# KevinMathewT/multimodal-propaganda-meme-classification

Measured on AMD Instinct MI355X. Metric: memes/sec (fine-tune step) ViT-B/16+BERT-base bs=32, 1/2/4/8 MI355X, higher is better.
Workload: dtype fp16

## Files before the change

### include/memehip.h

```cpp
#ifndef MEMEHIP_H
#define MEMEHIP_H

#include <stdint.h>

#ifdef __cplusplus
extern "C" {
#endif

typedef enum MhStatus {
    MH_OK = 0,
    MH_EINVAL = 1,
    MH_ESHAPE = 2,
    MH_ELAUNCH = 3
} MhStatus;

typedef void* mh_stream_t;

const char* mh_version(void);
const char* mh_status_str(int status);

#define MH_GEMM_MAX_GROUP 8
#define MH_GEMM_GELU 1
#define MH_GEMM_OUT_F32 2
#define MH_GEMM_ACCUM 4
#define MH_GEMM_QUICK_GELU 8
#define MH_GEMM_DERIV_AUX 16

typedef struct MhGemmProblem {
    const void* A;
    const void* B;
    void* C;
    const float* bias;
    const void* residual;
    void* aux;
    const void* mul;
    float* rowsum;
    int32_t M, N, K;
    int32_t lda, ldb, ldc;
    int32_t flags;
    float alpha;
    const uint32_t* drop_rng;
    float drop_p;
    uint32_t drop_stream;
    const int32_t* rows_dev;
    const int32_t* drop_rows;
    int32_t ksplit;
    int32_t reserved_;
} MhGemmProblem;

int mh_gemm_bf16_grouped(const MhGemmProblem* problems , int n_problems, int a_kmajor,
                         int b_kmajor, mh_stream_t stream);
int mh_gemm_ksplit_for(int K, int want);
int mh_gemm_set_trace(void* device_buffer);

int mh_layernorm_fwd(const void* x , const float* gamma, const float* beta, void* y ,
                     float* y_f32 , float* mean, float* rstd,
                     int rows, int D, float eps, mh_stream_t stream);
int mh_layernorm_bwd(const void* dy , const void* x , const float* gamma,
                     const float* mean, const float* rstd, const void* dx_add ,
                     void* dx , float* part , int n_part, int rows, int D,
                     void* dx_drop ,
                     const uint32_t* rng, float drop_p, uint32_t drop_stream, mh_stream_t stream);
#define MH_LN_MAX_JOBS 4
typedef struct MhLnFwdJob {
    const void* x; const float* gamma; const float* beta; void* y; float* y_f32; float* mean; float* rstd;
    int32_t rows; float eps;
    const int32_t* rows_dev;
} MhLnFwdJob;
typedef struct MhLnBwdJob {
    const void* dy; const void* x; const float* gamma; const float* mean; const float* rstd;
    const void* dx_add; void* dx; float* part; void* dx_drop; const uint32_t* rng;
    int32_t n_part; int32_t rows; float drop_p; uint32_t drop_stream;
    const int32_t* rows_dev;
    const int32_t* drop_rows;
} MhLnBwdJob;
int mh_layernorm_fwd_grouped(const MhLnFwdJob* jobs, int n_jobs, int D, mh_stream_t stream);
int mh_layernorm_bwd_grouped(const MhLnBwdJob* jobs, int n_jobs, int D, mh_stream_t stream);
#define MH_COLSUM_MAX_JOBS 64
typedef struct MhColsumJob {
    const float* part;
    float* out0;
    float* out1;
} MhColsumJob;
int mh_colsum_partials_f32(const MhColsumJob* jobs , int n_jobs, int n_part, int D,
                           float scale, mh_stream_t stream);

int mh_attn_fwd(const void* qkv, const int64_t* key_mask, void* out, float* lse, int B, int S, int H,
                const uint32_t* rng, float drop_p, uint32_t drop_stream, mh_stream_t stream);
int mh_attn_bwd(const void* qkv, const int64_t* key_mask, const void* out, const void* dout,
                const float* lse, float* delta, void* dqkv, int B, int S, int H, const uint32_t* rng,
                float drop_p, uint32_t drop_stream, mh_stream_t stream);
int mh_attn_fwd_packed(const void* qkv, const int64_t* key_mask, void* out, float* lse, const int32_t* cu,
                       const int32_t* row_map, int B, int S, int H, const uint32_t* rng, float drop_p,
                       uint32_t drop_stream, mh_stream_t stream);
int mh_attn_bwd_packed(const void* qkv, const int64_t* key_mask, const void* out, const void* dout,
                       const float* lse, float* delta, void* dqkv, const int32_t* cu, const int32_t* row_map, int B,
                       int S, int H, const uint32_t* rng, float drop_p, uint32_t drop_stream, mh_stream_t stream);

#define MH_ATTN_MAX_GROUP 2
typedef struct MhAttnProblem {
    const void* qkv; const int64_t* key_mask; void* out; float* lse;
    const void* dout; float* delta; void* dqkv;
    const int32_t* cu; const int32_t* row_map;
    const uint32_t* rng; float drop_p; uint32_t drop_stream;
    int32_t B, S, H; int32_t reserved;
} MhAttnProblem;
int mh_attn_fwd_grouped(const MhAttnProblem* problems , int n, mh_stream_t stream);
int mh_attn_bwd_grouped(const MhAttnProblem* problems , int n, mh_stream_t stream);
int mh_attn_set_onepass(int on);

int mh_pack_plan(const int64_t* mask , int B, int S, int pool_index, int32_t* cu, int32_t* row_map,
                 int32_t* inv_map, int64_t* pmask, int32_t* pool_rows, int32_t* n_rows, mh_stream_t stream);
int mh_pack_rows(const void* src , const int32_t* row_map, const int32_t* n_rows, void* dst,
                 int max_rows, int D, mh_stream_t stream);
int mh_unpack_rows(const void* src , const int32_t* inv_map, void* dst ,
                   int max_rows, int D, mh_stream_t stream);

#define MH_ROWS_MAX_JOBS 8
typedef struct {
    const void* src;
    void* dst;
    const int32_t* idx;
    const int32_t* rows_dev;
    int32_t n, rows, D, stride, offset; int32_t reserved_;
} MhRowsJob;
int mh_rows_gather(const MhRowsJob* jobs , int n_jobs, mh_stream_t stream);
int mh_rows_scatter_zero(const MhRowsJob* jobs , int n_jobs, mh_stream_t stream);

int mh_bert_embed_fwd(const int64_t* ids, const float* word, const float* pos, const float* type0,
                      const float* gamma, const float* beta, void* pre ,
                      void* y , float* mean, float* rstd, int B, int S, int D, int vocab,
                      float eps, const uint32_t* rng, float drop_p, uint32_t drop_stream ,
                      mh_stream_t stream);
int mh_bert_embed_bwd(const int64_t* ids, const void* d_pre , float* dword ,
                      float* dpos , float* dtype0 , int B, int S, int D,
                      int vocab, int64_t pad_id, float scale,
                      uint8_t* row_live ,
                      int32_t* first_pos , int32_t* id_count
                      ,
                      mh_stream_t stream);
int mh_position_ids_from_input_ids(const int64_t* ids , int32_t* pos_ids, int32_t* pos_inv, int B, int S, int pad_id,
                                   int max_position, mh_stream_t stream);
int mh_bert_embed_fwd_pos(const int64_t* ids, const float* word, const float* pos , const float* type0,
                          const float* gamma, const float* beta, void* pre, void* y, float* mean, float* rstd, int B, int S,
                          int D, int vocab, float eps, const uint32_t* rng, float drop_p, uint32_t drop_stream,
                          const int32_t* pos_ids , int max_position, mh_stream_t stream);
int mh_embed_pos_bwd(const void* d_pre , const int32_t* pos_inv ,
                     float* dpos , float* dtype0 , float* scratch ,
                     int B, int S, int D, int max_position, float scale, mh_stream_t stream);
int mh_image_normalize_u8(const uint8_t* src, float* dst, int B, int H, int W, const float* mean3 ,
                          const float* std3 , mh_stream_t stream);
int mh_image_resample_u8(const uint8_t* arena, const int64_t* src_off, const int32_t* hw, const int32_t* xbounds,
                         const int32_t* xcoef, int KX, const int32_t* ybounds, const int32_t* ycoef, int KY, const uint8_t* flip,
                         const uint8_t* vfirst, uint8_t* tmp, uint8_t* out, int B, int max_h, int max_w, int OH, int OW,
                         mh_stream_t stream);
int mh_image_luma_sum_u8(const uint8_t* img, unsigned long long* sums, int B, int HW, mh_stream_t stream);
int mh_image_jitter_rotate_u8(const uint8_t* in, uint8_t* scratch, uint8_t* out, const void* params, unsigned long long* lsum,
                              int B, int H, int W, mh_stream_t stream);
int mh_dropout_apply(void* x, int64_t n, const uint32_t* rng, float p, uint32_t stream_id, mh_stream_t stream);
int mh_dropout_mask_u8(uint8_t* out, int64_t n, const uint32_t* rng, float p, uint32_t stream_id,
                       mh_stream_t stream);
int mh_zero_rows_f32(const int64_t* ids, float* table, int n_ids, int D, int vocab, mh_stream_t stream);

int mh_patchify(const float* image, void* patches, int B, int C, int H, int W, int P, mh_stream_t stream);
int mh_patchify_ld(const float* image, void* patches , int B, int C, int H, int W, int P, int ld,
                   mh_stream_t stream);
int mh_copy2d_u32(const void* src, int ld_src, void* dst, int ld_dst, int rows, int cols, int pad_to, mh_stream_t stream);
int mh_vit_assemble_fwd(const void* proj , const float* cls, const float* pos,
                        void* x , int B, int Np, int D, mh_stream_t stream);
int mh_vit_assemble_bwd(const void* dx , void* dproj ,
                        float* dcls, float* dpos, int B, int Np, int D, float scale, mh_stream_t stream);

typedef struct MhHeadParams {
    const float *Wt, *bt;
    const float *Wi, *bi;
    const float *Wf, *bf_;
    const float *Wo, *bo;
} MhHeadParams;
typedef struct MhHeadGrads {
    float *Wt, *bt, *Wi, *bi, *Wf, *bf_, *Wo, *bo;
} MhHeadGrads;

int mh_head_fwd(const MhHeadParams* p , const float* text_hidden ,
                const float* image_hidden , int text_pool_index, float* pooled
                , float* feat , float* fused ,
                float* logits , int B, int S, int Nt, int Dt, int Di, int P, int C,
                const uint32_t* rng, float drop_p, uint32_t drop_stream ,
                const int32_t* text_rows , mh_stream_t stream);
int mh_head_bwd(const MhHeadParams* p , const MhHeadGrads* g , const float* dlogits,
                const float* pooled, const float* feat, const float* fused, float* dfeat ,
                float* dfused , void* d_text_hidden ,
                void* d_image_hidden , int text_pool_index, int B, int S, int Nt,
                int Dt, int Di, int P, int C, float out_scale, const uint32_t* rng, float drop_p,
                uint32_t drop_stream, const int32_t* text_rows , mh_stream_t stream);
int mh_pool_fwd(const float* text_hidden, const float* image_hidden, int text_pool_index, float* pooled, int B, int S,
                int Nt, int Dt, int Di, const int32_t* text_rows, mh_stream_t stream);
int mh_pool_bwd(const float* d_pooled, void* d_text_hidden, void* d_image_hidden, int text_pool_index, int B, int S,
                int Nt, int Dt, int Di, float out_scale, const int32_t* text_rows, mh_stream_t stream);
#define MH_BN_RELU 1
#define MH_BN_FROZEN_STATS 2
int mh_bn1d_fwd(const float* x, int ldx, const float* gamma, const float* beta, float* running_mean, float* running_var,
                float* y, int ldy, float* save_mean, float* save_rstd, int B, int F, float eps, float momentum,
                int training, int relu, mh_stream_t stream);
int mh_bn1d_bwd(const float* dy, int lddy, const float* x, int ldx, const float* y, int ldy, const float* gamma,
                const float* save_mean, const float* save_rstd, float* dx, int lddx, float* dgamma, float* dbeta, int B,
                int F, int relu, mh_stream_t stream);
int mh_ce_fwd_bwd(const float* logits, const int64_t* labels, float* loss, float* dlogits,
                  int32_t* n_correct, int B, int C, float grad_scale,
                  const float* grad_scale_dev ,
                  mh_stream_t stream);
int mh_focal_fwd_bwd(const float* logits, int ld, const float* targets , float* loss,
                     float* dlogits, int32_t* n_correct, int B, float alpha, float gamma, float grad_scale,
                     const float* grad_scale_dev , mh_stream_t stream);

#define MH_F32_ACCUM 1
#define MH_F32_TANH 2
#define MH_F32_RELU 4
#define MH_F32_BN 8
typedef struct MhGemmF32 {
    const float* A; const float* B; float* C; const float* bias ;
    int32_t M, N, K, lda, ldb, ldc, flags;
    const float* bn_gamma; const float* bn_beta; float* bn_running_mean; float* bn_running_var;
    float* bn_save_mean; float* bn_save_rstd; float* bn_z ;
    int32_t bn_ldz; float bn_eps; float bn_momentum; int32_t bn_training;
} MhGemmF32;
int mh_gemm_f32(const MhGemmF32* p , int a_kmajor, int b_kmajor, mh_stream_t stream);
int mh_colsum_f32(const float* x, int ld, float* out, int rows, int D, float scale, mh_stream_t stream);
int mh_pool_max_fwd(const float* h, float* out, int32_t* arg, int B, int S, int D, mh_stream_t stream);
int mh_pool_max_bwd(const float* dout, const int32_t* arg, float* dh, int B, int S, int D, mh_stream_t stream);
int mh_pool_mean_fwd(const float* h, const int64_t* mask, float* out, int B, int S, int D, mh_stream_t stream);
int mh_pool_mean_bwd(const float* dout, const int64_t* mask, float* dh, int B, int S, int D, mh_stream_t stream);
int mh_pool_attn_fwd(const float* h, const float* u, const float* w2, const float* b2, const int64_t* mask, float* p,
                     float* out, int B, int S, int D, int A, mh_stream_t stream);
int mh_pool_attn_bwd(const float* h, const float* u, const float* w2, const float* p, const float* dout, float* du, float* dh,
                     float* dw2_part, float* db2_part, int B, int S, int D, int A, mh_stream_t stream);
int mh_pad_seq_f32(const float* h, float* hp, int B, int S, int D, int pad, int Sp, mh_stream_t stream);
int mh_relu_max_fwd(const float* z, float* out, int32_t* arg, int B, int S, int Sp, int D, mh_stream_t stream);
int mh_relu_max_bwd(const float* dout, const int32_t* arg, float* dz, int rows, int Sp, int D, mh_stream_t stream);
int mh_conv_fold_f32(const float* da, float* dh, int B, int S, int D, int taps, int pad, int Sp, int rows, mh_stream_t stream);
int mh_softmax_gate_fwd(const float* g, const float* c, float* y, int B, int F, mh_stream_t stream);
int mh_softmax_gate_bwd(const float* g, const float* c, const float* dy, float* dg, float* dc, int B, int F, mh_stream_t stream);

int mh_mca3_fwd(const float* pa, const float* pc, const float* pi, const float* Vw, const float* bv, const float* text,
                const float* caption, float* w, float* ctx, int B, int U, mh_stream_t stream);
int mh_mca3_bwd(const float* pa, const float* pc, const float* pi, const float* Vw, const float* text, const float* caption,
                const float* w, const float* dctx, float* de_ws, float* dpa, float* dpi, float* dtext, float* dcaption,
                float* dV_part, float* dbv_part, int B, int U, mh_stream_t stream);

int mh_nchw_to_nhwc(const float* x, void* y, int B, int C, int H, int W, int Cp, mh_stream_t stream);
int mh_im2col_nhwc(const void* x, void* col, int B, int H, int W, int C, int KH, int KW, int stride, int pad, int ldc,
                   mh_stream_t stream);
int mh_col2im_nhwc(const void* dcol, void* dx, int B, int H, int W, int C, int KH, int KW, int stride, int pad, int ldc,
                   mh_stream_t stream);
int mh_conv_weight_pack(const float* w , void* out , int Cout, int Cin, int KH, int KW,
                        int Cp, int ldk, mh_stream_t stream);
int mh_conv_weight_unpack(const float* gk , float* g , int Cout, int Cin, int KH, int KW, int Cp,
                          int ldk, float scale, mh_stream_t stream);
#define MH_CONV_MAX_JOBS 64
typedef struct MhConvPackJob {
    const float* w;
    void* out;
    int32_t Cout, Cin, KH, KW, Cp, ldk;
// ... 124 lines not shown
```

### multimodal_propaganda_meme_classification_amd/_lib.py

```python
from __future__ import annotations

import ctypes as C
import os

_HERE = os.path.dirname(os.path.abspath(__file__))
LIB_PATH = os.path.join(_HERE, "libmemehip.so")
LIB_PATH_F16 = os.path.join(_HERE, "libmemehip_f16.so")
LIB_PATHS = {"bf16": LIB_PATH, "fp16": LIB_PATH_F16}

MH_GEMM_MAX_GROUP = 8
MH_GEMM_GELU = 1
MH_GEMM_OUT_F32 = 2
MH_GEMM_ACCUM = 4
MH_GEMM_QUICK_GELU = 8
MH_GEMM_DERIV_AUX = 16
MH_COLSUM_MAX_JOBS = 64
MH_LN_MAX_JOBS = 4
MH_ATTN_MAX_GROUP = 2

c_void_p, c_int, c_int64, c_float = C.c_void_p, C.c_int, C.c_int64, C.c_float


class MhGemmProblem(C.Structure):
    _fields_ = [("A", c_void_p), ("B", c_void_p), ("C", c_void_p), ("bias", c_void_p),
                ("residual", c_void_p), ("aux", c_void_p), ("mul", c_void_p), ("rowsum", c_void_p),
                ("M", C.c_int32), ("N", C.c_int32), ("K", C.c_int32),
                ("lda", C.c_int32), ("ldb", C.c_int32), ("ldc", C.c_int32),
                ("flags", C.c_int32), ("alpha", C.c_float),
                ("drop_rng", c_void_p), ("drop_p", C.c_float), ("drop_stream", C.c_uint32),
                ("rows_dev", c_void_p), ("drop_rows", c_void_p), ("ksplit", C.c_int32), ("reserved_", C.c_int32)]


class MhColsumJob(C.Structure):
    _fields_ = [("part", c_void_p), ("out0", c_void_p), ("out1", c_void_p)]


class MhConvPackJob(C.Structure):
    _fields_ = [("w", c_void_p), ("out", c_void_p)] + [(n, C.c_int32) for n in ("Cout", "Cin", "KH", "KW", "Cp", "ldk", "block_start", "reserved_")]


class MhConvWgradJob(C.Structure):
    _fields_ = [("slabs", c_void_p), ("g", c_void_p)] + [(n, C.c_int32) for n in ("Cout", "Cin", "KH", "KW", "Cp", "ldk", "nsplit", "accumulate")] + \
               [("scale", C.c_float), ("block_start", C.c_int32)]


class MhConvGeom(C.Structure):
    _fields_ = [(n, C.c_int32) for n in ("B", "H", "W", "C", "KH", "KW", "stride", "pad", "Cout", "ldk")]


class MhConvBnBwd(C.Structure):
    _fields_ = [(n, c_void_p) for n in ("z", "mean", "rstd", "gamma", "beta", "part")] + [("relu", C.c_int32), ("reserved_", C.c_int32),
                                                                                          ("addend", c_void_p), ("y_mask", c_void_p)]


class MhConvWgradProblem(C.Structure):
    _fields_ = [("dy", c_void_p), ("x", c_void_p), ("slabs", c_void_p), ("ksplit", C.c_int32), ("alpha", C.c_float), ("geom", MhConvGeom)]


MH_CONV_MAX_GROUP = 6
MH_CONV_MAX_JOBS = 64
MH_BN_RELU, MH_BN_ACCUM_PARAM_GRADS = 1, 2


MH_ADAM_MAX_GROUPS = 8


class MhAdamSkipGroups(C.Structure):
    _fields_ = [("hyper", c_void_p * MH_ADAM_MAX_GROUPS), ("beta1", C.c_double * MH_ADAM_MAX_GROUPS), ("beta2", C.c_double * MH_ADAM_MAX_GROUPS),
                ("n", C.c_int32), ("reserved_", C.c_int32)]


class MhLossScale(C.Structure):
    _fields_ = [("scale", c_void_p), ("growth", c_void_p), ("overflow", c_void_p), ("growth_factor", C.c_float), ("backoff_factor", C.c_float),
                ("min_scale", C.c_float), ("max_scale", C.c_float), ("growth_interval", C.c_int32), ("base_grad_scale", C.c_float)]


class MhLnFwdJob(C.Structure):
    _fields_ = [(n, c_void_p) for n in ("x", "gamma", "beta", "y", "y_f32", "mean", "rstd")] + \
               [("rows", C.c_int32), ("eps", C.c_float), ("rows_dev", c_void_p)]


class MhLnBwdJob(C.Structure):
    _fields_ = [(n, c_void_p) for n in ("dy", "x", "gamma", "mean", "rstd", "dx_add", "dx", "part", "dx_drop", "rng")] + \
               [("n_part", C.c_int32), ("rows", C.c_int32), ("drop_p", C.c_float), ("drop_stream", C.c_uint32),
                ("rows_dev", c_void_p), ("drop_rows", c_void_p)]


class MhAttnProblem(C.Structure):
    _fields_ = [(n, c_void_p) for n in ("qkv", "key_mask", "out", "lse", "dout", "delta", "dqkv", "cu", "row_map", "rng")] + \
               [("drop_p", C.c_float), ("drop_stream", C.c_uint32), ("B", C.c_int32), ("S", C.c_int32), ("H", C.c_int32),
                ("reserved", C.c_int32)]


MH_ROWS_MAX_JOBS = 8


class MhRowsJob(C.Structure):
    _fields_ = [(n, c_void_p) for n in ("src", "dst", "idx", "rows_dev")] + \
               [(n, C.c_int32) for n in ("n", "rows", "D", "stride", "offset", "reserved_")]


class MhGemmF32(C.Structure):
    _fields_ = [("A", c_void_p), ("B", c_void_p), ("C", c_void_p), ("bias", c_void_p)] + \
               [(n, C.c_int32) for n in ("M", "N", "K", "lda", "ldb", "ldc", "flags")] + \
               [(n, c_void_p) for n in ("bn_gamma", "bn_beta", "bn_running_mean", "bn_running_var", "bn_save_mean",
                                        "bn_save_rstd", "bn_z")] + \
               [("bn_ldz", C.c_int32), ("bn_eps", C.c_float), ("bn_momentum", C.c_float), ("bn_training", C.c_int32)]


MH_F32_ACCUM, MH_F32_TANH, MH_F32_RELU, MH_F32_BN = 1, 2, 4, 8


class MhHeadParams(C.Structure):
    _fields_ = [(n, c_void_p) for n in ("Wt", "bt", "Wi", "bi", "Wf", "bf_", "Wo", "bo")]


class MhHeadGrads(C.Structure):
    _fields_ = [(n, c_void_p) for n in ("Wt", "bt", "Wi", "bi", "Wf", "bf_", "Wo", "bo")]


_PROTOS = {
    "mh_gemm_bf16_grouped": [C.POINTER(MhGemmProblem), c_int, c_int, c_int, c_void_p],
    "mh_gemm_set_trace": [c_void_p],
    "mh_gemm_ksplit_for": [c_int, c_int],
    "mh_layernorm_fwd": [c_void_p] * 7 + [c_int, c_int, c_float, c_void_p],
    "mh_layernorm_bwd": [c_void_p] * 8 + [c_int, c_int, c_int, c_void_p, c_void_p, c_float, C.c_uint32, c_void_p],
    "mh_layernorm_fwd_grouped": [C.POINTER(MhLnFwdJob), c_int, c_int, c_void_p],
    "mh_layernorm_bwd_grouped": [C.POINTER(MhLnBwdJob), c_int, c_int, c_void_p],
    "mh_colsum_partials_f32": [C.POINTER(MhColsumJob), c_int, c_int, c_int, c_float, c_void_p],
    "mh_attn_fwd": [c_void_p] * 4 + [c_int, c_int, c_int, c_void_p, c_float, C.c_uint32, c_void_p],
    "mh_attn_bwd": [c_void_p] * 7 + [c_int, c_int, c_int, c_void_p, c_float, C.c_uint32, c_void_p],
    "mh_attn_fwd_grouped": [C.POINTER(MhAttnProblem), c_int, c_void_p],
    "mh_attn_bwd_grouped": [C.POINTER(MhAttnProblem), c_int, c_void_p],
    "mh_attn_set_onepass": [c_int],
    "mh_attn_fwd_packed": [c_void_p] * 6 + [c_int, c_int, c_int, c_void_p, c_float, C.c_uint32, c_void_p],
    "mh_attn_bwd_packed": [c_void_p] * 9 + [c_int, c_int, c_int, c_void_p, c_float, C.c_uint32, c_void_p],
    "mh_pack_plan": [c_void_p, c_int, c_int, c_int] + [c_void_p] * 6 + [c_void_p],
    "mh_pack_rows": [c_void_p] * 4 + [c_int, c_int, c_void_p],
    "mh_unpack_rows": [c_void_p] * 3 + [c_int, c_int, c_void_p],
    "mh_rows_gather": [C.POINTER(MhRowsJob), c_int, c_void_p],
    "mh_rows_scatter_zero": [C.POINTER(MhRowsJob), c_int, c_void_p],
    "mh_bert_embed_fwd": [c_void_p] * 10 + [c_int, c_int, c_int, c_int, c_float, c_void_p, c_float, C.c_uint32, c_void_p],
    "mh_image_normalize_u8": [c_void_p, c_void_p, c_int, c_int, c_int, C.POINTER(c_float), C.POINTER(c_float), c_void_p],
    "mh_image_resample_u8": [c_void_p] * 5 + [c_int] + [c_void_p] * 2 + [c_int] + [c_void_p] * 4 + [c_int] * 5 + [c_void_p],
    "mh_image_luma_sum_u8": [c_void_p, c_void_p, c_int, c_int, c_void_p],
    "mh_image_jitter_rotate_u8": [c_void_p] * 5 + [c_int] * 3 + [c_void_p],
    "mh_dropout_apply": [c_void_p, c_int64, c_void_p, c_float, C.c_uint32, c_void_p],
    "mh_dropout_mask_u8": [c_void_p, c_int64, c_void_p, c_float, C.c_uint32, c_void_p],
    "mh_bert_embed_bwd": [c_void_p] * 5 + [c_int, c_int, c_int, c_int, c_int64, c_float, c_void_p, c_void_p, c_void_p, c_void_p],
    "mh_position_ids_from_input_ids": [c_void_p] * 3 + [c_int] * 4 + [c_void_p],
    "mh_bert_embed_fwd_pos": [c_void_p] * 10 + [c_int, c_int, c_int, c_int, c_float, c_void_p, c_float, C.c_uint32, c_void_p, c_int,
                              c_void_p],
    "mh_embed_pos_bwd": [c_void_p] * 5 + [c_int] * 4 + [c_float, c_void_p],
    "mh_zero_rows_f32": [c_void_p, c_void_p, c_int, c_int, c_int, c_void_p],
    "mh_patchify": [c_void_p, c_void_p] + [c_int] * 5 + [c_void_p],
    "mh_patchify_ld": [c_void_p, c_void_p] + [c_int] * 6 + [c_void_p],
    "mh_copy2d_u32": [c_void_p, c_int, c_void_p, c_int, c_int, c_int, c_int, c_void_p],
    "mh_vit_assemble_fwd": [c_void_p] * 4 + [c_int] * 3 + [c_void_p],
    "mh_vit_assemble_bwd": [c_void_p] * 4 + [c_int] * 3 + [c_float, c_void_p],
    "mh_head_fwd": [C.POINTER(MhHeadParams), c_void_p, c_void_p, c_int] + [c_void_p] * 4 + [c_int] * 7 + [c_void_p, c_float, C.c_uint32, c_void_p, c_void_p],
    "mh_head_bwd": [C.POINTER(MhHeadParams), C.POINTER(MhHeadGrads)] + [c_void_p] * 8 + [c_int] * 8 + [c_float, c_void_p, c_float, C.c_uint32, c_void_p, c_void_p],
    "mh_pool_fwd": [c_void_p, c_void_p, c_int, c_void_p] + [c_int] * 5 + [c_void_p, c_void_p],
    "mh_pool_bwd": [c_void_p, c_void_p, c_void_p, c_int] + [c_int] * 5 + [c_float, c_void_p, c_void_p],
    "mh_bn1d_fwd": [c_void_p, c_int, c_void_p, c_void_p, c_void_p, c_void_p, c_void_p, c_int, c_void_p, c_void_p, c_int, c_int,
                    c_float, c_float, c_int, c_int, c_void_p],
    "mh_bn1d_bwd": [c_void_p, c_int, c_void_p, c_int, c_void_p, c_int, c_void_p, c_void_p, c_void_p, c_void_p, c_int, c_void_p,
                    c_void_p, c_int, c_int, c_int, c_void_p],
    "mh_gemm_f32": [C.POINTER(MhGemmF32), c_int, c_int, c_void_p],
    "mh_colsum_f32": [c_void_p, c_int, c_void_p, c_int, c_int, c_float, c_void_p],
    "mh_pool_max_fwd": [c_void_p, c_void_p, c_void_p, c_int, c_int, c_int, c_void_p],
    "mh_pool_max_bwd": [c_void_p, c_void_p, c_void_p, c_int, c_int, c_int, c_void_p],
    "mh_pool_mean_fwd": [c_void_p, c_void_p, c_void_p, c_int, c_int, c_int, c_void_p],
    "mh_pool_mean_bwd": [c_void_p, c_void_p, c_void_p, c_int, c_int, c_int, c_void_p],
    "mh_pool_attn_fwd": [c_void_p] * 7 + [c_int] * 4 + [c_void_p],
    "mh_pool_attn_bwd": [c_void_p] * 9 + [c_int] * 4 + [c_void_p],
    "mh_pad_seq_f32": [c_void_p, c_void_p] + [c_int] * 5 + [c_void_p],
    "mh_relu_max_fwd": [c_void_p, c_void_p, c_void_p] + [c_int] * 4 + [c_void_p],
    "mh_relu_max_bwd": [c_void_p, c_void_p, c_void_p] + [c_int] * 3 + [c_void_p],
    "mh_conv_fold_f32": [c_void_p, c_void_p] + [c_int] * 7 + [c_void_p],
    "mh_mca3_fwd": [c_void_p] * 9 + [c_int, c_int, c_void_p],
    "mh_mca3_bwd": [c_void_p] * 15 + [c_int, c_int, c_void_p],
    "mh_softmax_gate_fwd": [c_void_p, c_void_p, c_void_p, c_int, c_int, c_void_p],
    "mh_softmax_gate_bwd": [c_void_p] * 5 + [c_int, c_int, c_void_p],
    "mh_nchw_to_nhwc": [c_void_p, c_void_p] + [c_int] * 5 + [c_void_p],
    "mh_im2col_nhwc": [c_void_p, c_void_p] + [c_int] * 9 + [c_void_p],
    "mh_col2im_nhwc": [c_void_p, c_void_p] + [c_int] * 9 + [c_void_p],
    "mh_conv_weight_pack": [c_void_p, c_void_p] + [c_int] * 6 + [c_void_p],
    "mh_conv_weight_unpack": [c_void_p, c_void_p] + [c_int] * 6 + [c_float, c_void_p],
    "mh_conv_weight_pack_batched": [C.POINTER(MhConvPackJob), c_int, c_void_p],
    "mh_conv_wgrad_finish_batched": [C.POINTER(MhConvWgradJob), c_int, c_void_p],
    "mh_conv_splitk": [C.POINTER(MhConvGeom), c_int],
    "mh_conv_fwd": [c_void_p, c_void_p, c_void_p, c_void_p, c_void_p, C.POINTER(MhConvGeom), c_void_p],
    "mh_conv_dgrad": [c_void_p, c_void_p, c_void_p, c_void_p, C.POINTER(MhConvGeom), C.POINTER(MhConvBnBwd), c_void_p],
    "mh_conv_dgrad_pair": [c_void_p, c_void_p, c_void_p, c_void_p, c_int, c_int, c_void_p, C.POINTER(MhConvGeom), C.POINTER(MhConvBnBwd), c_void_p],
    "mh_bn2d_bwd_parts": [c_void_p, c_void_p, c_void_p, c_int] + [c_void_p] * 7 + [c_int, c_int, c_int, c_float, c_void_p],
    "mh_conv_wgrad": [c_void_p, c_void_p, c_void_p, c_int, c_float, C.POINTER(MhConvGeom), c_void_p],
    "mh_conv_wgrad_grouped": [C.POINTER(MhConvWgradProblem), c_int, c_void_p],
    "mh_bn2d_fwd_parts": [c_void_p, c_void_p, c_int] + [c_void_p] * 8 + [c_int, c_int, c_float, c_float, c_int, c_void_p],
    "mh_bn2d_workspace_elems": [c_int, c_int],
    "mh_bn2d_fwd": [c_void_p] * 10 + [c_int, c_int, c_float, c_float, c_int, c_int, c_void_p],
    "mh_bn2d_apply": [c_void_p] * 7 + [c_int, c_int, c_int, c_void_p],
    "mh_bn2d_bwd": [c_void_p] * 12 + [c_int, c_int, c_int, c_float, c_void_p],
    "mh_maxpool_fwd": [c_void_p, c_void_p, c_void_p] + [c_int] * 7 + [c_void_p],
    "mh_maxpool_bwd": [c_void_p, c_void_p, c_void_p] + [c_int] * 7 + [c_void_p],
    "mh_avgpool_fwd": [c_void_p, c_void_p, c_int, c_int, c_int, c_void_p],
    "mh_avgpool_bwd": [c_void_p, c_void_p, c_int, c_int, c_int, c_float, c_void_p],
    "mh_add_h16": [c_void_p, c_void_p, c_void_p, c_int64, c_void_p],
    "mh_dwconv_weight_pack": [c_void_p, c_void_p, c_int, c_int, c_void_p],
    "mh_dwconv_nhwc": [c_void_p, c_void_p, c_void_p, c_void_p] + [c_int] * 5 + [c_void_p],
    "mh_dwconv_nhwc_dgrad": [c_void_p, c_void_p, c_void_p, c_void_p] + [c_int] * 5 + [c_void_p],
    "mh_dwconv_wgrad_workspace_elems": [c_int] * 5,
    "mh_dwconv_nhwc_wgrad": [c_void_p] * 5 + [c_int] * 5 + [c_float, c_int, c_void_p],
    "mh_layer_scale_bwd": [c_void_p] * 8 + [c_int, c_int, c_int, c_void_p],
    "mh_ce_fwd_bwd": [c_void_p] * 5 + [c_int, c_int, c_float, c_void_p, c_void_p],
    "mh_focal_fwd_bwd": [c_void_p, c_int, c_void_p, c_void_p, c_void_p, c_void_p, c_int, c_float, c_float, c_float, c_void_p, c_void_p],
    "mh_adam_skip_account": [C.POINTER(MhAdamSkipGroups), c_void_p, c_void_p, c_void_p, C.POINTER(MhLossScale), c_void_p],
    "mh_sumsq_f32": [c_void_p, c_int64, c_void_p, c_void_p, c_void_p],
    "mh_adam_step": [c_void_p] * 5 + [c_int64, c_int64, c_void_p, c_int, c_void_p, c_float, c_float, c_void_p, c_int, c_void_p],
    "mh_adam_step_rows": [c_void_p] * 6 + [c_int, c_int, c_void_p, c_int, c_void_p, c_float, c_float, c_void_p, c_int, c_void_p],
    "mh_cast_f32_bf16": [c_void_p, c_void_p, c_int64, c_void_p],
    "mh_cast_bf16_f32": [c_void_p, c_void_p, c_int64, c_void_p],
    "mh_sum_shards_16": [c_void_p, c_void_p, c_int, c_int64, c_void_p],
    "mh_attn_decode": [c_void_p, c_int, c_void_p, c_void_p, c_int64, c_int, c_void_p, c_int, c_void_p, c_int, c_void_p, c_int,
                       c_void_p, c_int, c_int, c_int, c_void_p],
    "mh_decode_embed": [c_void_p] * 7 + [c_int] * 4 + [c_float, c_void_p],
    "mh_greedy_step": [c_void_p, c_int, c_int, c_int, c_void_p, c_int, c_void_p, c_void_p, c_void_p, c_int, c_int64, c_int64, c_void_p],
    "mh_version": [],
    "mh_status_str": [c_int],
}
_RESTYPES = {"mh_version": C.c_char_p, "mh_status_str": C.c_char_p, "mh_bn2d_workspace_elems": c_int64,
             "mh_dwconv_wgrad_workspace_elems": c_int64}
_LAB_PROTOS = {"mh_gemm_set_variant": ([c_int], c_int), "mh_gemm_streamk_workspace_bytes": ([], c_int64),
               "mh_gemm_set_streamk": ([c_void_p, c_int], c_int)}

EXPORTED_SYMBOLS = tuple(_PROTOS)

_libs = {}


class MemehipError(RuntimeError):
    pass


def load(kind: str = "bf16") -> C.CDLL:
    if kind in _libs:
        return _libs[kind]
    if kind not in LIB_PATHS:
        raise ValueError(f"compute dtype must be 'bf16' or 'fp16', got {kind!r}")
    path = LIB_PATHS[kind]
    if kind == "bf16" and os.environ.get("MEMEHIP_LIB"):
        path = os.environ["MEMEHIP_LIB"]
    if kind == "fp16" and os.environ.get("MEMEHIP_LIB_F16"):
        path = os.environ["MEMEHIP_LIB_F16"]
    if not os.path.exists(path):
        raise MemehipError(
            f"{path} is missing: build the HIP extension first "
            "(python -c 'import __graft_entry__ as g; g.build()' or make -C "
            "multimodal_propaganda_meme_classification_amd/csrc). There is no CPU/PyTorch fallback.")
    lib = C.CDLL(path)
    for name, argtypes in _PROTOS.items():
        fn = getattr(lib, name)
        fn.argtypes = argtypes
        fn.restype = _RESTYPES.get(name, c_int)
    for name, (argtypes, restype) in _LAB_PROTOS.items():
        if hasattr(lib, name):
            fn = getattr(lib, name)
            fn.argtypes, fn.restype = argtypes, restype
    _libs[kind] = lib
    return lib


def check(status: int, what: str):
    if status != 0:
        msg = load().mh_status_str(status).decode()
        raise MemehipError(f"{what} failed: status {status} ({msg})")
```

### multimodal_propaganda_meme_classification_amd/csrc/attention.hip

```cpp
#include "common.h"
#include <stdlib.h>

namespace {

constexpr int HD = 64;
constexpr int TILE = 64;
constexpr int IMG = TILE * HD * 2;
constexpr float NEG_BIG = -1.0e30f;
constexpr float LOG2E = 1.4426950408889634f;
constexpr float LN2 = 0.6931471805599453f;

MH_DEV int row_img_off(int row, int chunk) { return row * 128 + ((chunk ^ ((row ^ (row >> 3)) & 7)) << 4); }
MH_DEV int tr_img_off(int row, int unit) { return row * 128 + ((unit ^ (((row >> 1) & 1) << 1)) << 5); }

template <int NT>
struct TileRegs {
    static constexpr int CH = (TILE * 8 + NT - 1) / NT;
    i32x4 v[CH];
};
template <int NT>
MH_DEV void tile_load(const h16* __restrict__ base, size_t pitch, int row0, int nrows, int tid, TileRegs<NT>& R) {
#pragma unroll
    for (int i = 0; i < TileRegs<NT>::CH; ++i) {
        const int q = tid + i * NT;
        const int r = q >> 3, c = q & 7;
        R.v[i] = i32x4{0, 0, 0, 0};
        if (q < TILE * 8 && row0 + r < nrows) R.v[i] = *(const i32x4*)(base + (size_t)(row0 + r) * pitch + c * 8);
    }
}
template <int NT>
MH_DEV void tile_store(const TileRegs<NT>& R, int tid, char* row_img, char* tr_img) {
#pragma unroll
    for (int i = 0; i < TileRegs<NT>::CH; ++i) {
        const int q = tid + i * NT;
        if (q >= TILE * 8) continue;
        const int r = q >> 3, c = q & 7;
        if (row_img) *(i32x4*)(row_img + row_img_off(r, c)) = R.v[i];
        if (tr_img) *(i32x4*)(tr_img + tr_img_off(r, c >> 1) + ((c & 1) << 4)) = R.v[i];
    }
}

template <int NW, int NTL>
MH_DEV void dma_resident(const h16* __restrict__ base, size_t pitch, int nrows, int ntiles, int wave_u, int lane, char* row_img,
                         char* tr_img) {
    const __amdgpu_buffer_rsrc_t rs = mh_rsrc(base, (uint32_t)(((size_t)(nrows - 1) * pitch + HD) * 2));
    const int npieces = ntiles * 8;
#pragma unroll
    for (int i = 0; i < (NTL * 8 + NW - 1) / NW; ++i) {
        const int p = wave_u + i * NW;
        if (p < npieces) {
            const int r = p * 8 + (lane >> 3), rl = r & (TILE - 1), cp = lane & 7;
            const uint32_t rowoff = (uint32_t)r * (uint32_t)pitch * 2u;
            if (row_img) {
                const int ck = cp ^ ((rl ^ (rl >> 3)) & 7);
                __builtin_amdgcn_raw_ptr_buffer_load_lds(rs, LDS_PTR(void, row_img + p * 1024), 16, rowoff + ck * 16, 0, 0, 0);
            }
            if (tr_img) {
                const int cv = ((((cp >> 1) ^ (((rl >> 1) & 1) << 1)) << 1) | (cp & 1));
                __builtin_amdgcn_raw_ptr_buffer_load_lds(rs, LDS_PTR(void, tr_img + p * 1024), 16, rowoff + cv * 16, 0, 0, 0);
            }
        }
    }
}

MH_DEV h16x8 frag_rows(const char* img, int rb, int s, int lane) {
    Pack8 u;
    u.v = *(const i32x4*)(img + row_img_off(rb + (lane & 31), 2 * s + (lane >> 5)));
    return u.h;
}
MH_DEV h16x8 frag_tr(const char* img, int rb, int s, int dbase, int lane) {
    const int i = lane & 15, q = i >> 2, p = i & 3;
    const int chalf = (lane >> 4) & 1, h = lane >> 5;
    const int unit = (dbase >> 4) + chalf;
    const int r0 = rb + 16 * s + 4 * h + q;
    const int r1 = r0 + 8;
    s16x4 lo = __builtin_amdgcn_ds_read_tr16_b64_v4i16(LDS_PTR(s16x4, img + tr_img_off(r0, unit) + 8 * p));
    s16x4 hi = __builtin_amdgcn_ds_read_tr16_b64_v4i16(LDS_PTR(s16x4, img + tr_img_off(r1, unit) + 8 * p));
    union {
        struct { s16x4 lo, hi; } s;
        h16x8 h8;
    } cv;
    cv.s.lo = lo;
    cv.s.hi = hi;
    return cv.h8;
}
MH_DEV h16x8 acc_frag(const f32x16& x, int s) {
    h16x8 f;
#pragma unroll
    for (int j = 0; j < 8; ++j) f[j] = (h16)x[8 * s + j];
    return f;
}
MH_DEV int acc_row(int g, int h) { return (g & 3) + 8 * (g >> 2) + 4 * h; }

MH_DEV void load_rows_frag(const h16* __restrict__ base, size_t pitch, int row0, int nrows, int lane,
                           h16x8 (&f)[4]) {
    const int r = row0 + (lane & 31);
#pragma unroll
    for (int s = 0; s < 4; ++s) {
        Pack8 u;
        u.v = i32x4{0, 0, 0, 0};
        if (r < nrows) u.v = *(const i32x4*)(base + (size_t)r * pitch + 16 * s + 8 * (lane >> 5));
        f[s] = u.h;
    }
}

MH_DEV void store_rows_from_T(h16* __restrict__ base, size_t pitch, int row0, int nrows, int lane,
                              const f32x16 (&acc)[2], float scale) {
    const int r = row0 + (lane & 31), h = lane >> 5;
    if (r >= nrows) return;
#pragma unroll
    for (int dt = 0; dt < 2; ++dt)
#pragma unroll
        for (int g4 = 0; g4 < 4; ++g4) {
            Pack4 u;
#pragma unroll
            for (int e = 0; e < 4; ++e) u.e[e] = (h16)(acc[dt][4 * g4 + e] * scale);
            *(i32x2*)(base + (size_t)r * pitch + dt * 32 + 8 * g4 + 4 * h) = u.v;
        }
}

struct AttnArgs {
    const h16* qkv;
    const int64_t* key_mask;
    h16* out;
    float* lse;
    const h16* dout;
    float* delta;
    h16* dqkv;
    int B, S, H;
    const uint32_t* rng;
    float drop_p;
    uint32_t drop_stream;
    const int32_t* cu;
    const int32_t* row_map;
};

template <int NW, int NT_RES, bool DROP>
MH_DEV void attn_fwd_body(const AttnArgs& A, const int bx, const int gx, const int bh, char* smem) {
    const h16* __restrict__ qkv = A.qkv;
    const int64_t* __restrict__ key_mask = A.key_mask;
    h16* __restrict__ out = A.out;
    float* __restrict__ lse = A.lse;
    const int S = A.S, H = A.H;
    const uint32_t* __restrict__ rng = A.rng;
    const float drop_p = A.drop_p;
    const uint32_t drop_stream = A.drop_stream;
    const int32_t* __restrict__ cu = A.cu;
    const int32_t* __restrict__ row_map = A.row_map;
    constexpr int NT = NW * 64;
    constexpr int NTL = NT_RES > 0 ? NT_RES : 1;
    const DropCtx drop = mh_drop_ctx(DROP ? rng : nullptr, drop_p, drop_stream);
    char* k_img = smem;
    char* v_img = smem + NTL * IMG;
    float* kbias = (float*)(smem + 2 * NTL * IMG);
    int* kany = (int*)(kbias + NTL * TILE);
    int* pos_t = kany + 16;

    const int b = bh / H, hh = bh % H;
    const int tid = threadIdx.x, lane = tid & 63, wave = tid >> 6, h = lane >> 5;
    const size_t pitch = (size_t)3 * H * HD;
    const size_t r0 = cu ? (size_t)cu[b] : (size_t)b * S;
    const int Sb = cu ? cu[b + 1] - cu[b] : S;
    auto pos = [&](int i) -> uint64_t { return (row_map && i < Sb) ? (uint64_t)(row_map[r0 + i] - b * S) : (uint64_t)i; };
    auto posl = [&](int i) -> uint64_t { return NT_RES > 0 ? (uint64_t)pos_t[i] : pos(i); };
    const h16* qb = qkv + r0 * pitch + hh * HD;
    const h16* kb = qb + (size_t)H * HD;
    const h16* vb = qb + (size_t)2 * H * HD;
    const float c = 0.125f * LOG2E;
    constexpr float LAZY_LOG2 = 6.0f;
    const int ntiles = (Sb + TILE - 1) / TILE;

    const int qt_first = bx * NW + wave;
    h16x8 qf[4];
    if (NT_RES > 0) {
        const int uw = __builtin_amdgcn_readfirstlane(wave);
        dma_resident<NW, NTL>(kb, pitch, Sb, ntiles, uw, lane, k_img, nullptr);
        dma_resident<NW, NTL>(vb, pitch, Sb, ntiles, uw, lane, nullptr, v_img);
        if (qt_first * 32 < Sb) load_rows_frag(qb, pitch, qt_first * 32, Sb, lane, qf);
        if (DROP)
            for (int i = tid; i < NTL * TILE; i += NT) pos_t[i] = (int)pos(i);
        if (tid < TILE) {
            int64_t km[NTL];
#pragma unroll
            for (int t = 0; t < NTL; ++t) km[t] = 1;
            if (key_mask && Sb > 0) {
#pragma unroll
                for (int t = 0; t < NTL; ++t) km[t] = key_mask[r0 + max(min(t * TILE + tid, Sb - 1), 0)];
            }
#pragma unroll
            for (int t = 0; t < NTL; ++t)
                if (t * TILE + tid >= Sb) km[t] = 0;
#pragma unroll
            for (int t = 0; t < NTL; ++t) {
                const float bias = km[t] != 0 ? 0.f : NEG_BIG;
                kbias[t * TILE + tid] = bias;
                const unsigned long long bal = __ballot(bias == 0.f);
                if (tid == 0) {
                    kany[t * 2] = (bal & 0xffffffffull) != 0;
                    kany[t * 2 + 1] = (bal >> 32) != 0;
                }
            }
        }
        __syncthreads();
    }

    for (int qt = qt_first; (NT_RES > 0) ? (qt * 32 < Sb) : (qt == bx * NW + wave); qt += NW * gx) {
        const int wq0 = qt * 32;
        const bool active = wq0 < Sb;
        if (NT_RES == 0 || qt != qt_first) load_rows_frag(qb, pitch, wq0, Sb, lane, qf);
        f32x16 o[2];
#pragma unroll
        for (int i = 0; i < 2; ++i)
#pragma unroll
            for (int g = 0; g < 16; ++g) o[i][g] = 0.f;
        float m = NEG_BIG, l = 0.f;
        TileRegs<NT> Rk, Rv;
        int64_t Rm = 0;
        auto pre_load = [&](int t) {
            tile_load<NT>(kb, pitch, t * TILE, Sb, tid, Rk);
            tile_load<NT>(vb, pitch, t * TILE, Sb, tid, Rv);
            if (tid < TILE) {
                const int key = t * TILE + tid;
                Rm = (key < Sb && (!key_mask || key_mask[r0 + key] != 0)) ? 1 : 0;
            }
        };
        auto pre_store = [&]() {
            tile_store<NT>(Rk, tid, k_img, nullptr);
            tile_store<NT>(Rv, tid, nullptr, v_img);
            if (tid < TILE) {
                const float bias = Rm ? 0.f : NEG_BIG;
                kbias[tid] = bias;
                const unsigned long long bal = __ballot(bias == 0.f);
                if (tid == 0) {
                    kany[0] = (bal & 0xffffffffull) != 0;
                    kany[1] = (bal >> 32) != 0;
                }
            }
        };
        if (NT_RES == 0 && ntiles > 0) pre_load(0);

        for (int t = 0; t < ntiles; ++t) {
            const int slot = NT_RES > 0 ? t : 0;
            if (NT_RES == 0) {
                __syncthreads();
                pre_store();
                __syncthreads();
                if (t + 1 < ntiles) pre_load(t + 1);
                if (!active) continue;
            }
            const char* ki = k_img + slot * IMG;
            const char* vi = v_img + slot * IMG;
            const float* kbt = kbias + slot * TILE;
#pragma unroll
            for (int sub = 0; sub < 2; ++sub) {
                if (!__builtin_amdgcn_readfirstlane(kany[slot * 2 + sub])) continue;
                f32x16 st;
#pragma unroll
                for (int g = 0; g < 16; ++g) st[g] = 0.f;
#pragma unroll
                for (int s = 0; s < 4; ++s)
                    st = MH_MFMA_32x32x16(frag_rows(ki, sub * 32, s, lane), qf[s], st, 0, 0, 0);
                float mx = NEG_BIG;
#pragma unroll
                for (int g4 = 0; g4 < 4; ++g4) {
                    const f32x4 kb4 = *(const f32x4*)(kbt + sub * 32 + 8 * g4 + 4 * h);
#pragma unroll
                    for (int e = 0; e < 4; ++e) {
                        const float v = st[4 * g4 + e] * c + kb4[e];
                        st[4 * g4 + e] = v;
                        mx = fmaxf(mx, v);
                    }
                }
                mx = fmaxf(mx, mh_xor_partner<32>(mx, (unsigned)lane));
                const bool move = mx > m + LAZY_LOG2;
                if (__ballot(move) != 0ull) {
                    const float mn = move ? mx : m;
                    const float alpha = __builtin_amdgcn_exp2f(m - mn);
                    m = mn;
                    l *= alpha;
#pragma unroll
                    for (int i = 0; i < 2; ++i)
#pragma unroll
                        for (int g = 0; g < 16; ++g) o[i][g] *= alpha;
                }
                float ps = 0.f;
#pragma unroll
                for (int g = 0; g < 16; ++g) {
                    const float p = __builtin_amdgcn_exp2f(st[g] - m);
                    st[g] = p;
                    ps += p;
                }
                l += ps;
                if (DROP && drop.on) {
                    const uint64_t rowbase = (((uint64_t)bh * S) + posl(wq0 + (lane & 31))) * (uint64_t)S;
#pragma unroll
                    for (int g = 0; g < 16; ++g)
                        st[g] *= mh_drop_mul(drop, rowbase + posl(t * TILE + sub * 32 + acc_row(g, h)));
                }
#pragma unroll
                for (int s = 0; s < 2; ++s) {
                    const h16x8 pf = acc_frag(st, s);
#pragma unroll
                    for (int dt = 0; dt < 2; ++dt)
                        o[dt] = MH_MFMA_32x32x16(frag_tr(vi, sub * 32, s, dt * 32, lane), pf, o[dt], 0, 0, 0);
                }
            }
        }
        if (!active) continue;
        l += mh_xor_partner<32>(l, (unsigned)lane);
        const float inv = l > 0.f ? 1.0f / l : 0.f;
        store_rows_from_T(out + r0 * H * HD + hh * HD, (size_t)H * HD, wq0, Sb, lane, o, inv);
        const int q = wq0 + (lane & 31);
        if (h == 0 && q < Sb) lse[((size_t)b * H + hh) * S + q] = (m + __builtin_amdgcn_logf(l)) * LN2;
    }
}

template <int NW, int NT_RES, bool DROP>
MH_DEV void attn_bwd_dq_body(const AttnArgs& A, const int bx, const int gx, const int bh, char* smem) {
    const h16* __restrict__ qkv = A.qkv;
    const int64_t* __restrict__ key_mask = A.key_mask;
    const h16* __restrict__ out = A.out;
    const h16* __restrict__ dout = A.dout;
    const float* __restrict__ lse = A.lse;
    float* __restrict__ delta = A.delta;
    h16* __restrict__ dqkv = A.dqkv;
    const int S = A.S, H = A.H;
    const uint32_t* __restrict__ rng = A.rng;
    const float drop_p = A.drop_p;
    const uint32_t drop_stream = A.drop_stream;
    const int32_t* __restrict__ cu = A.cu;
    const int32_t* __restrict__ row_map = A.row_map;
    constexpr int NT = NW * 64;
    constexpr int NTL = NT_RES > 0 ? NT_RES : 1;
    const DropCtx drop = mh_drop_ctx(DROP ? rng : nullptr, drop_p, drop_stream);
    char* k_img = smem;
    char* kt_img = smem + NTL * IMG;
    char* v_img = smem + 2 * NTL * IMG;
    float* kbias = (float*)(smem + 3 * NTL * IMG);
    int* kany = (int*)(kbias + NTL * TILE);
    int* pos_t = kany + 16;

    const int b = bh / H, hh = bh % H;
    const int tid = threadIdx.x, lane = tid & 63, wave = tid >> 6, h = lane >> 5;
    const size_t pitch = (size_t)3 * H * HD;
    const size_t r0 = cu ? (size_t)cu[b] : (size_t)b * S;
    const int Sb = cu ? cu[b + 1] - cu[b] : S;
    auto pos = [&](int i) -> uint64_t { return (row_map && i < Sb) ? (uint64_t)(row_map[r0 + i] - b * S) : (uint64_t)i; };
    auto posl = [&](int i) -> uint64_t { return NT_RES > 0 ? (uint64_t)pos_t[i] : pos(i); };
    const h16* qb = qkv + r0 * pitch + hh * HD;
    const h16* kb = qb + (size_t)H * HD;
    const h16* vb = qb + (size_t)2 * H * HD;
    const h16* dob = dout + r0 * H * HD + hh * HD;
    const float c = 0.125f * LOG2E;
    const int ntiles = (Sb + TILE - 1) / TILE;

    auto stage = [&](int t, int slot) {
        if (tid < TILE) {
            const int key = t * TILE + tid;
            float bias = NEG_BIG;
            if (key < Sb && (!key_mask || key_mask[r0 + key] != 0)) bias = 0.f;
            kbias[slot * TILE + tid] = bias;
            const unsigned long long bal = __ballot(bias == 0.f);
            if (tid == 0) {
                kany[slot * 2] = (bal & 0xffffffffull) != 0;
                kany[slot * 2 + 1] = (bal >> 32) != 0;
            }
        }
    };
    if (NT_RES > 0) {
        const int uw = __builtin_amdgcn_readfirstlane(wave);
        dma_resident<NW, NTL>(kb, pitch, Sb, ntiles, uw, lane, k_img, kt_img);
        dma_resident<NW, NTL>(vb, pitch, Sb, ntiles, uw, lane, v_img, nullptr);
        if (DROP)
            for (int i = tid; i < NTL * TILE; i += NT) pos_t[i] = (int)pos(i);
        for (int t = 0; t < ntiles; ++t) stage(t, t);
        __syncthreads();
    }

    for (int qt = bx * NW + wave; (NT_RES > 0) ? (qt * 32 < Sb) : (qt == bx * NW + wave); qt += NW * gx) {
        const int wq0 = qt * 32;
        const bool active = wq0 < Sb;
        const int q = wq0 + (lane & 31);
        h16x8 qf[4], dof[4];
        load_rows_frag(qb, pitch, wq0, Sb, lane, qf);
        load_rows_frag(dob, (size_t)H * HD, wq0, Sb, lane, dof);
        float dl = 0.f;
        {
            h16x8 of[4];
            load_rows_frag(out + r0 * H * HD + hh * HD, (size_t)H * HD, wq0, Sb, lane, of);
#pragma unroll
            for (int s4 = 0; s4 < 4; ++s4)
#pragma unroll
                for (int j = 0; j < 8; ++j) dl += (float)dof[s4][j] * (float)of[s4][j];
            dl += mh_xor_partner<32>(dl, (unsigned)lane);
        }
        float lse2 = 0.f;
        if (q < Sb) {
            lse2 = lse[((size_t)b * H + hh) * S + q] * LOG2E;
            if (h == 0) delta[((size_t)b * H + hh) * S + q] = dl;
        }
        f32x16 dq[2];
#pragma unroll
        for (int i = 0; i < 2; ++i)
#pragma unroll
            for (int g = 0; g < 16; ++g) dq[i][g] = 0.f;
        TileRegs<NT> Rk, Rv;
        int64_t Rm = 0;
        auto pre_load = [&](int t) {
            tile_load<NT>(kb, pitch, t * TILE, Sb, tid, Rk);
            tile_load<NT>(vb, pitch, t * TILE, Sb, tid, Rv);
            if (tid < TILE) {
                const int key = t * TILE + tid;
                Rm = (key < Sb && (!key_mask || key_mask[r0 + key] != 0)) ? 1 : 0;
            }
        };
        auto pre_store = [&]() {
            tile_store<NT>(Rk, tid, k_img, kt_img);
            tile_store<NT>(Rv, tid, v_img, nullptr);
            if (tid < TILE) {
                const float bias = Rm ? 0.f : NEG_BIG;
                kbias[tid] = bias;
                const unsigned long long bal = __ballot(bias == 0.f);
                if (tid == 0) {
                    kany[0] = (bal & 0xffffffffull) != 0;
                    kany[1] = (bal >> 32) != 0;
                }
            }
        };
        if (NT_RES == 0 && ntiles > 0) pre_load(0);

        for (int t = 0; t < ntiles; ++t) {
            const int slot = NT_RES > 0 ? t : 0;
            if (NT_RES == 0) {
                __syncthreads();
                pre_store();
                __syncthreads();
                if (t + 1 < ntiles) pre_load(t + 1);
                if (!active) continue;
            }
            const char* ki = k_img + slot * IMG;
            const char* kti = kt_img + slot * IMG;
            const char* vi = v_img + slot * IMG;
            const float* kbt = kbias + slot * TILE;
#pragma unroll
            for (int sub = 0; sub < 2; ++sub) {
                if (!__builtin_amdgcn_readfirstlane(kany[slot * 2 + sub])) continue;
                f32x16 st, dp;
#pragma unroll
                for (int g = 0; g < 16; ++g) { st[g] = 0.f; dp[g] = 0.f; }
#pragma unroll
                for (int s = 0; s < 4; ++s) {
                    st = MH_MFMA_32x32x16(frag_rows(ki, sub * 32, s, lane), qf[s], st, 0, 0, 0);
                    dp = MH_MFMA_32x32x16(frag_rows(vi, sub * 32, s, lane), dof[s], dp, 0, 0, 0);
                }
#pragma unroll
                for (int g4 = 0; g4 < 4; ++g4) {
                    const f32x4 kb4 = *(const f32x4*)(kbt + sub * 32 + 8 * g4 + 4 * h);
#pragma unroll
                    for (int e = 0; e < 4; ++e) {
                        const int g = 4 * g4 + e;
                        const float p = __builtin_amdgcn_exp2f(st[g] * c + kb4[e] - lse2);
                        float dpg = dp[g];
                        if (DROP && drop.on)
                            dpg *= mh_drop_mul(drop, ((uint64_t)bh * S + posl(q)) * (uint64_t)S +
                                                         posl(t * TILE + sub * 32 + acc_row(g, h)));
                        st[g] = p * (dpg - dl);
                    }
                }
#pragma unroll
                for (int s = 0; s < 2; ++s) {
                    const h16x8 df = acc_frag(st, s);
#pragma unroll
                    for (int dt = 0; dt < 2; ++dt)
                        dq[dt] = MH_MFMA_32x32x16(frag_tr(kti, sub * 32, s, dt * 32, lane), df, dq[dt], 0, 0, 0);
                }
            }
        }
        if (!active) continue;
        store_rows_from_T(dqkv + r0 * pitch + hh * HD, pitch, wq0, Sb, lane, dq, 0.125f);
    }
}

template <int NW, int NT_RES, bool DROP, bool OWN_DELTA = false>
MH_DEV void attn_bwd_dkv_body(const AttnArgs& A, const int bx, const int gx, const int bh, char* smem) {
    const h16* __restrict__ qkv = A.qkv;
    const int64_t* __restrict__ key_mask = A.key_mask;
    const h16* __restrict__ outp = A.out;
    const h16* __restrict__ dout = A.dout;
    const float* __restrict__ lse = A.lse;
    const float* __restrict__ delta = A.delta;
    h16* __restrict__ dqkv = A.dqkv;
    const int S = A.S, H = A.H;
    const uint32_t* __restrict__ rng = A.rng;
    const float drop_p = A.drop_p;
    const uint32_t drop_stream = A.drop_stream;
    const int32_t* __restrict__ cu = A.cu;
    const int32_t* __restrict__ row_map = A.row_map;
    constexpr int NT = NW * 64;
    constexpr int NTL = NT_RES > 0 ? NT_RES : 1;
    const DropCtx drop = mh_drop_ctx(DROP ? rng : nullptr, drop_p, drop_stream);
    char* q_img = smem;
    char* qt_img = smem + NTL * IMG;
    char* do_img = smem + 2 * NTL * IMG;
    char* dot_img = smem + 3 * NTL * IMG;
    float* lse_t = (float*)(smem + 4 * NTL * IMG);
    float* dl_t = lse_t + NTL * TILE;
    int* pos_t = (int*)(dl_t + NTL * TILE);

    const int b = bh / H, hh = bh % H;
    const int tid = threadIdx.x, lane = tid & 63, wave = tid >> 6, h = lane >> 5;
    const size_t pitch = (size_t)3 * H * HD;
    const size_t r0 = cu ? (size_t)cu[b] : (size_t)b * S;
    const int Sb = cu ? cu[b + 1] - cu[b] : S;
    auto pos = [&](int i) -> uint64_t { return (row_map && i < Sb) ? (uint64_t)(row_map[r0 + i] - b * S) : (uint64_t)i; };
    auto posl = [&](int i) -> uint64_t { return NT_RES > 0 ? (uint64_t)pos_t[i] : pos(i); };
    const h16* qb = qkv + r0 * pitch + hh * HD;
    const h16* kb = qb + (size_t)H * HD;
    const h16* vb = qb + (size_t)2 * H * HD;
    const h16* dob = dout + r0 * H * HD + hh * HD;
    const float c = 0.125f * LOG2E;
    const int ntiles = (Sb + TILE - 1) / TILE;

    auto stage = [&](int t, int slot) {
        for (int i = tid; i < TILE; i += NT) {
            const int qq = t * TILE + i;
            lse_t[slot * TILE + i] = qq < Sb ? lse[((size_t)b * H + hh) * S + qq] * LOG2E : 1.0e30f;
            if (!OWN_DELTA) dl_t[slot * TILE + i] = qq < Sb ? delta[((size_t)b * H + hh) * S + qq] : 0.f;
        }
        if (OWN_DELTA && tid < 2 * TILE) {
            const int i = tid >> 1, hf = tid & 1;
            const int qq = t * TILE + i;
            float dl = 0.f;
            if (qq < Sb) {
                const h16* dr = dob + (size_t)qq * H * HD + 8 * hf;
                const h16* orow = outp + (r0 + qq) * (size_t)H * HD + hh * HD + 8 * hf;
#pragma unroll
                for (int s4 = 0; s4 < 4; ++s4) {
                    Pack8 a, o;
                    a.v = *(const i32x4*)(dr + 16 * s4);
                    o.v = *(const i32x4*)(orow + 16 * s4);
#pragma unroll
                    for (int j = 0; j < 8; ++j) dl += (float)a.h[j] * (float)o.h[j];
                }
            }
            dl += mh_xor_partner<1>(dl, 0u);
            if (hf == 0) dl_t[slot * TILE + i] = dl;
        }
    };
    if (NT_RES > 0) {
        const int uw = __builtin_amdgcn_readfirstlane(wave);
        dma_resident<NW, NTL>(qb, pitch, Sb, ntiles, uw, lane, q_img, qt_img);
        dma_resident<NW, NTL>(dob, (size_t)H * HD, Sb, ntiles, uw, lane, do_img, dot_img);
        if (DROP)
            for (int i = tid; i < NTL * TILE; i += NT) pos_t[i] = (int)pos(i);
        for (int t = 0; t < ntiles; ++t) stage(t, t);
        __syncthreads();
    }

    for (int kt = bx * NW + wave; (NT_RES > 0) ? (kt * 32 < Sb) : (kt == bx * NW + wave); kt += NW * gx) {
        const int wk0 = kt * 32;
        const bool active = wk0 < Sb;
        const int key = wk0 + (lane & 31);
        h16x8 kf[4], vf[4];
        load_rows_frag(kb, pitch, wk0, Sb, lane, kf);
        load_rows_frag(vb, pitch, wk0, Sb, lane, vf);
        float kbias = NEG_BIG;
        if (key < Sb && (!key_mask || key_mask[r0 + key] != 0)) kbias = 0.f;
        f32x16 dk[2], dv[2];
#pragma unroll
        for (int i = 0; i < 2; ++i)
#pragma unroll
            for (int g = 0; g < 16; ++g) { dk[i][g] = 0.f; dv[i][g] = 0.f; }
        const bool any_key = __ballot(kbias == 0.f) != 0ull;
        TileRegs<NT> Rq, Rdo;
        float Rl = 0.f, Rd = 0.f;
        i32x4 Ra[4], Ro[4];
        auto pre_load = [&](int t) {
            tile_load<NT>(qb, pitch, t * TILE, Sb, tid, Rq);
            tile_load<NT>(dob, (size_t)H * HD, t * TILE, Sb, tid, Rdo);
            if (tid < TILE) {
                const int qq = t * TILE + tid;
                Rl = qq < Sb ? lse[((size_t)b * H + hh) * S + qq] * LOG2E : 1.0e30f;
                if (!OWN_DELTA) Rd = qq < Sb ? delta[((size_t)b * H + hh) * S + qq] : 0.f;
            }
            if (OWN_DELTA && tid < 2 * TILE) {
                const int i = tid >> 1, hf = tid & 1;
                const int qq = t * TILE + i;
#pragma unroll
                for (int s4 = 0; s4 < 4; ++s4) { Ra[s4] = i32x4{0, 0, 0, 0}; Ro[s4] = i32x4{0, 0, 0, 0}; }
                if (qq < Sb) {
                    const h16* dr = dob + (size_t)qq * H * HD + 8 * hf;
                    const h16* orow = outp + (r0 + qq) * (size_t)H * HD + hh * HD + 8 * hf;
#pragma unroll
                    for (int s4 = 0; s4 < 4; ++s4) {
                        Ra[s4] = *(const i32x4*)(dr + 16 * s4);
                        Ro[s4] = *(const i32x4*)(orow + 16 * s4);
                    }
                }
            }
        };
        auto pre_store = [&]() {
            tile_store<NT>(Rq, tid, q_img, qt_img);
            tile_store<NT>(Rdo, tid, do_img, dot_img);
            if (tid < TILE) {
                lse_t[tid] = Rl;
                if (!OWN_DELTA) dl_t[tid] = Rd;
            }
            if (OWN_DELTA && tid < 2 * TILE) {
                float dl = 0.f;
#pragma unroll
                for (int s4 = 0; s4 < 4; ++s4) {
                    Pack8 a, o;
                    a.v = Ra[s4];
                    o.v = Ro[s4];
#pragma unroll
                    for (int j = 0; j < 8; ++j) dl += (float)a.h[j] * (float)o.h[j];
                }
                dl += mh_xor_partner<1>(dl, 0u);
                if ((tid & 1) == 0) dl_t[tid >> 1] = dl;
            }
        };
        if (NT_RES == 0 && ntiles > 0) pre_load(0);

        for (int t = 0; t < ntiles; ++t) {
            const int slot = NT_RES > 0 ? t : 0;
            if (NT_RES == 0) {
                __syncthreads();
                pre_store();
                __syncthreads();
                if (t + 1 < ntiles) pre_load(t + 1);
                if (!active) continue;
            }
            if (!any_key) continue;
            const char* qi = q_img + slot * IMG;
            const char* qti = qt_img + slot * IMG;
            const char* doi = do_img + slot * IMG;
            const char* doti = dot_img + slot * IMG;
            const float* lt = lse_t + slot * TILE;
            const float* dt_ = dl_t + slot * TILE;
#pragma unroll
            for (int sub = 0; sub < 2; ++sub) {
                if (t * TILE + sub * 32 >= Sb) continue;
                f32x16 st, dp;
#pragma unroll
                for (int g = 0; g < 16; ++g) { st[g] = 0.f; dp[g] = 0.f; }
#pragma unroll
                for (int s = 0; s < 4; ++s) {
                    st = MH_MFMA_32x32x16(frag_rows(qi, sub * 32, s, lane), kf[s], st, 0, 0, 0);
                    dp = MH_MFMA_32x32x16(frag_rows(doi, sub * 32, s, lane), vf[s], dp, 0, 0, 0);
                }
                f32x16 pp;
#pragma unroll
                for (int g4 = 0; g4 < 4; ++g4) {
                    const f32x4 l4 = *(const f32x4*)(lt + sub * 32 + 8 * g4 + 4 * h);
                    const f32x4 d4 = *(const f32x4*)(dt_ + sub * 32 + 8 * g4 + 4 * h);
#pragma unroll
                    for (int e = 0; e < 4; ++e) {
                        const int g = 4 * g4 + e;
                        const float p = __builtin_amdgcn_exp2f(st[g] * c + kbias - l4[e]);
                        float mul = 1.f;
                        if (DROP && drop.on)
                            mul = mh_drop_mul(drop, ((uint64_t)bh * S + posl(t * TILE + sub * 32 + 8 * g4 + 4 * h + e)) *
                                                            (uint64_t)S + posl(key));
                        pp[g] = p * mul;
                        st[g] = p * (dp[g] * mul - d4[e]);
                    }
                }
#pragma unroll
                for (int s = 0; s < 2; ++s) {
                    const h16x8 pf = acc_frag(pp, s);
                    const h16x8 df = acc_frag(st, s);
#pragma unroll
                    for (int dt = 0; dt < 2; ++dt) {
                        dv[dt] = MH_MFMA_32x32x16(frag_tr(doti, sub * 32, s, dt * 32, lane), pf, dv[dt], 0, 0, 0);
                        dk[dt] = MH_MFMA_32x32x16(frag_tr(qti, sub * 32, s, dt * 32, lane), df, dk[dt], 0, 0, 0);
                    }
                }
            }
        }
        if (!active) continue;
        h16* dkb = dqkv + r0 * pitch + (size_t)H * HD + hh * HD;
        h16* dvb = dqkv + r0 * pitch + (size_t)2 * H * HD + hh * HD;
        store_rows_from_T(dkb, pitch, wk0, Sb, lane, dk, 0.125f);
        store_rows_from_T(dvb, pitch, wk0, Sb, lane, dv, 1.0f);
    }
}


template <int NW, int NT_RES, bool DROP>
__global__ __launch_bounds__(NW * 64) void attn_fwd_kernel(const AttnArgs A) {
    extern __shared__ __attribute__((aligned(16))) char smem[];
    attn_fwd_body<NW, NT_RES, DROP>(A, blockIdx.x, gridDim.x, blockIdx.y, smem);
}
template <int NW, int NT_RES, bool DROP>
__global__ __launch_bounds__(NW * 64) void attn_bwd_dq_kernel(const AttnArgs A) {
    extern __shared__ __attribute__((aligned(16))) char smem[];
    attn_bwd_dq_body<NW, NT_RES, DROP>(A, blockIdx.x, gridDim.x, blockIdx.y, smem);
}
template <int NW, int NT_RES, bool DROP>
__global__ __launch_bounds__(NW * 64) void attn_bwd_dkv_kernel(const AttnArgs A) {
    extern __shared__ __attribute__((aligned(16))) char smem[];
    attn_bwd_dkv_body<NW, NT_RES, DROP>(A, blockIdx.x, gridDim.x, blockIdx.y, smem);
}
template <int RES_A, bool DROP_B>
__global__ __launch_bounds__(448) void attn_fwd_dual_kernel(const AttnArgs A, const AttnArgs Bp, const int nA) {
    extern __shared__ __attribute__((aligned(16))) char smem[];
    if ((int)blockIdx.y < nA) {
        attn_fwd_body<7, RES_A, false>(A, 0, 1, blockIdx.y, smem);
    } else {
        if (threadIdx.x >= 256) return;
        attn_fwd_body<4, 2, DROP_B>(Bp, 0, 1, blockIdx.y - nA, smem);
    }
}

template <int RES_B, bool DROP_B>
__global__ __launch_bounds__(448) void attn_bwd_merged_dual_kernel(const AttnArgs A, const AttnArgs Bp, const int nA,
                                                                   const int nB) {
    extern __shared__ __attribute__((aligned(16))) char smem[];
    const int y = blockIdx.y;
    if (y < nA) {
        attn_bwd_dq_body<7, 0, false>(A, 0, 1, y, smem);
    } else if (y < 2 * nA) {
        attn_bwd_dkv_body<7, 0, false, true>(A, 0, 1, y - nA, smem);
    } else {
        if (threadIdx.x >= 256) return;
        if (y < 2 * nA + nB) attn_bwd_dq_body<4, RES_B, DROP_B>(Bp, 0, 1, y - 2 * nA, smem);
        else attn_bwd_dkv_body<4, RES_B, DROP_B, true>(Bp, 0, 1, y - 2 * nA - nB, smem);
    }
}


constexpr int OP_NB = 7, OP_ROWS = OP_NB * 32, OP_IMG = OP_ROWS * 128;
constexpr int OP_MB_PITCH = 72, OP_MB = 32 * OP_MB_PITCH;
constexpr int OP_LDS = 5 * OP_IMG + OP_NB * OP_MB + 2 * OP_ROWS * 4;

MH_DEV void attn_bwd_onepass_body(const AttnArgs& A, const int bh, char* smem) {
    const h16* __restrict__ qkv = A.qkv;
    const h16* __restrict__ outp = A.out;
    const h16* __restrict__ dout = A.dout;
    const float* __restrict__ lse = A.lse;
    float* __restrict__ delta = A.delta;
    h16* __restrict__ dqkv = A.dqkv;
    const int S = A.S, H = A.H;
    const int b = bh / H, hh = bh % H;
    const int tid = threadIdx.x, lane = tid & 63, wave = tid >> 6, h = lane >> 5;
    const size_t pitch = (size_t)3 * H * HD;
    const size_t r0 = (size_t)b * S;
    const int Sb = S;
    const h16* qb = qkv + r0 * pitch + hh * HD;
    const h16* kb = qb + (size_t)H * HD;
    const h16* vb = qb + (size_t)2 * H * HD;
    const h16* dob = dout + r0 * H * HD + hh * HD;
    const float c = 0.125f * LOG2E;

    char* q_img = smem;
    char* qt_img = smem + OP_IMG;
    char* do_img = smem + 2 * OP_IMG;
    char* dot_img = smem + 3 * OP_IMG;
    char* kt_img = smem + 4 * OP_IMG;
    char* mbox = smem + 5 * OP_IMG;
    float* lse_t = (float*)(mbox + OP_NB * OP_MB);
    float* dl_t = lse_t + OP_ROWS;

    {
        const uint32_t qk_bytes = (uint32_t)(((size_t)(Sb - 1) * pitch + HD) * 2);
        const uint32_t do_bytes = (uint32_t)(((size_t)(Sb - 1) * H * HD + HD) * 2);
        const __amdgpu_buffer_rsrc_t rq = mh_rsrc(qb, qk_bytes), rk = mh_rsrc(kb, qk_bytes), rd = mh_rsrc(dob, do_bytes);
        const int uw = __builtin_amdgcn_readfirstlane(wave);
#pragma unroll
        for (int i = 0; i < OP_ROWS / 8 / OP_NB; ++i) {
            const int p = uw + i * OP_NB;
            const int r = p * 8 + (lane >> 3), cp = lane & 7;
            const int c_row = cp ^ ((r ^ (r >> 3)) & 7);
            const int c_tr = ((((cp >> 1) ^ (((r >> 1) & 1) << 1)) << 1) | (cp & 1));
            const uint32_t oq = (uint32_t)r * (uint32_t)pitch * 2u, od = (uint32_t)r * (uint32_t)(H * HD) * 2u;
            char* dst = smem + p * 1024;
            __builtin_amdgcn_raw_ptr_buffer_load_lds(rq, LDS_PTR(void, dst), 16, oq + c_row * 16, 0, 0, 0);
            __builtin_amdgcn_raw_ptr_buffer_load_lds(rq, LDS_PTR(void, dst + OP_IMG), 16, oq + c_tr * 16, 0, 0, 0);
            __builtin_amdgcn_raw_ptr_buffer_load_lds(rd, LDS_PTR(void, dst + 2 * OP_IMG), 16, od + c_row * 16, 0, 0, 0);
            __builtin_amdgcn_raw_ptr_buffer_load_lds(rd, LDS_PTR(void, dst + 3 * OP_IMG), 16, od + c_tr * 16, 0, 0, 0);
            __builtin_amdgcn_raw_ptr_buffer_load_lds(rk, LDS_PTR(void, dst + 4 * OP_IMG), 16, oq + c_tr * 16, 0, 0, 0);
        }
    }
    const int wk0 = wave * 32;
    const bool mine = wk0 < Sb;
    h16x8 kf[4], vf[4];
    load_rows_frag(kb, pitch, wk0, Sb, lane, kf);
    load_rows_frag(vb, pitch, wk0, Sb, lane, vf);
    {
        const int i = tid >> 1, hf = tid & 1;
        float dl = 0.f;
        if (i < Sb) {
            const h16* dr = dob + (size_t)i * H * HD + 8 * hf;
            const h16* orow = outp + (r0 + i) * (size_t)H * HD + hh * HD + 8 * hf;
#pragma unroll
            for (int s4 = 0; s4 < 4; ++s4) {
                Pack8 a, o;
                a.v = *(const i32x4*)(dr + 16 * s4);
                o.v = *(const i32x4*)(orow + 16 * s4);
#pragma unroll
                for (int j = 0; j < 8; ++j) dl += (float)a.h[j] * (float)o.h[j];
            }
        }
        dl += mh_xor_partner<1>(dl, 0u);
        if (hf == 0) {
            dl_t[i] = dl;
            lse_t[i] = i < Sb ? lse[((size_t)b * H + hh) * S + i] * LOG2E : 1.0e30f;
            if (i < Sb) delta[((size_t)b * H + hh) * S + i] = dl;
        }
    }
    __syncthreads();

    const float kbias = (wk0 + (lane & 31)) < Sb ? 0.f : NEG_BIG;
    f32x16 dk[2], dv[2], dq[2];
#pragma unroll
    for (int i = 0; i < 2; ++i)
#pragma unroll
        for (int g = 0; g < 16; ++g) { dk[i][g] = 0.f; dv[i][g] = 0.f; dq[i][g] = 0.f; }

    for (int j = 0; j < OP_NB; ++j) {
        int qblk = wave + j;
        if (qblk >= OP_NB) qblk -= OP_NB;
        const int q0 = qblk * 32;
        if (mine && q0 < Sb) {
            f32x16 st, dp;
#pragma unroll
            for (int g = 0; g < 16; ++g) { st[g] = 0.f; dp[g] = 0.f; }
#pragma unroll
            for (int s = 0; s < 4; ++s) {
                st = MH_MFMA_32x32x16(frag_rows(q_img, q0, s, lane), kf[s], st, 0, 0, 0);
                dp = MH_MFMA_32x32x16(frag_rows(do_img, q0, s, lane), vf[s], dp, 0, 0, 0);
            }
            f32x16 pp;
#pragma unroll
            for (int g4 = 0; g4 < 4; ++g4) {
                const f32x4 l4 = *(const f32x4*)(lse_t + q0 + 8 * g4 + 4 * h);
                const f32x4 d4 = *(const f32x4*)(dl_t + q0 + 8 * g4 + 4 * h);
#pragma unroll
                for (int e = 0; e < 4; ++e) {
                    const int g = 4 * g4 + e;
                    const float pr = __builtin_amdgcn_exp2f(st[g] * c + kbias - l4[e]);
                    pp[g] = pr;
                    st[g] = pr * (dp[g] - d4[e]);
                }
            }
#pragma unroll
            for (int s = 0; s < 2; ++s) {
                const h16x8 pf = acc_frag(pp, s);
                const h16x8 df = acc_frag(st, s);
#pragma unroll
                for (int dt = 0; dt < 2; ++dt) {
                    dv[dt] = MH_MFMA_32x32x16(frag_tr(dot_img, q0, s, dt * 32, lane), pf, dv[dt], 0, 0, 0);
                    dk[dt] = MH_MFMA_32x32x16(frag_tr(qt_img, q0, s, dt * 32, lane), df, dk[dt], 0, 0, 0);
                }
            }
            char* mb = mbox + qblk * OP_MB + (lane & 31) * 2;
#pragma unroll
            for (int g4 = 0; g4 < 4; ++g4)
#pragma unroll
                for (int e = 0; e < 4; ++e) *(h16*)(mb + (8 * g4 + 4 * h + e) * OP_MB_PITCH) = (h16)st[4 * g4 + e];
        }
        __syncthreads();
        int src = wave - j;
        if (src < 0) src += OP_NB;
        if (mine && src * 32 < Sb) {
            const char* mb = mbox + wave * OP_MB + (lane & 31) * OP_MB_PITCH;
#pragma unroll
            for (int s = 0; s < 2; ++s) {
                union {
                    struct { i32x2 lo, hi; } v;
                    h16x8 f;
                } u;
                u.v.lo = *(const i32x2*)(mb + (16 * s + 4 * h) * 2);
                u.v.hi = *(const i32x2*)(mb + (16 * s + 8 + 4 * h) * 2);
#pragma unroll
                for (int dt = 0; dt < 2; ++dt)
                    dq[dt] = MH_MFMA_32x32x16(frag_tr(kt_img, src * 32, s, dt * 32, lane), u.f, dq[dt], 0, 0, 0);
            }
        }
        __syncthreads();
    }
    if (!mine) return;
    store_rows_from_T(dqkv + r0 * pitch + hh * HD, pitch, wk0, Sb, lane, dq, 0.125f);
    store_rows_from_T(dqkv + r0 * pitch + (size_t)H * HD + hh * HD, pitch, wk0, Sb, lane, dk, 0.125f);
    store_rows_from_T(dqkv + r0 * pitch + (size_t)2 * H * HD + hh * HD, pitch, wk0, Sb, lane, dv, 1.0f);
}

__global__ __launch_bounds__(448) void attn_bwd_onepass_kernel(const AttnArgs A) {
    extern __shared__ __attribute__((aligned(16))) char smem[];
    attn_bwd_onepass_body(A, blockIdx.x, smem);
}
template <int RES_B, bool DROP_B>
__global__ __launch_bounds__(448) void attn_bwd_onepass_dual_kernel(const AttnArgs A, const AttnArgs Bp, const int nA, const int nB) {
    extern __shared__ __attribute__((aligned(16))) char smem[];
    const int y = blockIdx.y;
    if (y < nA) {
        attn_bwd_onepass_body(A, y, smem);
    } else {
        if (threadIdx.x >= 256) return;
        if (y < nA + nB) attn_bwd_dq_body<4, RES_B, DROP_B>(Bp, 0, 1, y - nA, smem);
        else attn_bwd_dkv_body<4, RES_B, DROP_B, true>(Bp, 0, 1, y - nA - nB, smem);
    }
}
template <int RES_B, bool DROP_B>
__global__ __launch_bounds__(256) void attn_bwd_merged_single_kernel(const AttnArgs Bp, const int nB) {
    extern __shared__ __attribute__((aligned(16))) char smem[];
    const int y = blockIdx.y;
    if (y < nB) attn_bwd_dq_body<4, RES_B, DROP_B>(Bp, 0, 1, y, smem);
    else attn_bwd_dkv_body<4, RES_B, DROP_B, true>(Bp, 0, 1, y - nB, smem);
}

template <auto KERN, int THREADS, int LDS, typename... Args>
void launch(dim3 grid, hipStream_t s, const Args&... args) {
    static const hipError_t raised = hipFuncSetAttribute((const void*)KERN, hipFuncAttributeMaxDynamicSharedMemorySize, LDS);
    (void)raised;
    hipLaunchKernelGGL(KERN, grid, dim3(THREADS), LDS, s, args...);
}

int check_problem(const MhAttnProblem& p, bool bwd) {
    if (!p.qkv || !p.out || !p.lse) return MH_EINVAL;
    if (bwd && (!p.dout || !p.delta || !p.dqkv)) return MH_EINVAL;
    if (p.B < 1 || p.S < 1 || p.H < 1 || p.drop_p < 0.f || p.drop_p >= 1.f) return MH_ESHAPE;
    return MH_OK;
}
AttnArgs to_args(const MhAttnProblem& p) {
    AttnArgs a;
    a.qkv = (const h16*)p.qkv;
    a.key_mask = p.key_mask;
    a.out = (h16*)p.out;
    a.lse = p.lse;
    a.dout = (const h16*)p.dout;
    a.delta = p.delta;
    a.dqkv = (h16*)p.dqkv;
    a.B = p.B; a.S = p.S; a.H = p.H;
    a.rng = p.rng; a.drop_p = p.drop_p; a.drop_stream = p.drop_stream;
    a.cu = p.cu; a.row_map = p.row_map;
    return a;
}
bool has_drop(const MhAttnProblem& p) { return p.rng && p.drop_p > 0.f; }

constexpr int lds_fwd(int nt) { return 2 * (nt > 0 ? nt : 1) * IMG + 2 * (nt > 0 ? nt : 1) * TILE * 4 + 64; }
constexpr int lds_dq(int nt) { return 3 * (nt > 0 ? nt : 1) * IMG + 2 * (nt > 0 ? nt : 1) * TILE * 4 + 64; }
constexpr int lds_dkv(int nt) { return 4 * (nt > 0 ? nt : 1) * IMG + 3 * (nt > 0 ? nt : 1) * TILE * 4; }
constexpr int cmax(int a, int b) { return a > b ? a : b; }
constexpr int LDS_FWD_DUAL = cmax(lds_fwd(4), lds_fwd(2));
constexpr int LDS_BWD_TEXT = cmax(lds_dq(2), lds_dkv(2));
constexpr int LDS_BWD_DUAL = cmax(cmax(lds_dq(0), lds_dkv(0)), LDS_BWD_TEXT);

template <int NW, int NT_RES>
void fwd_one(bool dr, dim3 grid, hipStream_t s, const AttnArgs& a) {
    dr ? launch<attn_fwd_kernel<NW, NT_RES, true>, NW * 64, lds_fwd(NT_RES)>(grid, s, a)
       : launch<attn_fwd_kernel<NW, NT_RES, false>, NW * 64, lds_fwd(NT_RES)>(grid, s, a);
}
template <int NW, int NT_RES>
void bwd_sweeps(bool dr, dim3 grid, hipStream_t s, const AttnArgs& a) {
    dr ? launch<attn_bwd_dq_kernel<NW, NT_RES, true>, NW * 64, lds_dq(NT_RES)>(grid, s, a)
       : launch<attn_bwd_dq_kernel<NW, NT_RES, false>, NW * 64, lds_dq(NT_RES)>(grid, s, a);
    dr ? launch<attn_bwd_dkv_kernel<NW, NT_RES, true>, NW * 64, lds_dkv(NT_RES)>(grid, s, a)
       : launch<attn_bwd_dkv_kernel<NW, NT_RES, false>, NW * 64, lds_dkv(NT_RES)>(grid, s, a);
}

void launch_fwd(const MhAttnProblem& p, hipStream_t s) {
    const AttnArgs a = to_args(p);
    const bool dr = has_drop(p);
    const int S = p.S, BH = p.B * p.H;
    if (S <= 128) fwd_one<4, 2>(dr, dim3(1, BH), s, a);
    else if (S <= 224) fwd_one<7, 4>(dr, dim3(1, BH), s, a);
    else if (S <= 256) fwd_one<4, 4>(dr, dim3(2, BH), s, a);
    else fwd_one<4, 0>(dr, dim3((S + 127) / 128, BH), s, a);
}

int g_onepass = 2;
bool onepass_fits(const MhAttnProblem& p) {
    return g_onepass != 0 && p.S > 128 && p.S <= OP_ROWS && !p.key_mask && !p.cu && !has_drop(p);
}
void launch_onepass(const AttnArgs& a, int BH, hipStream_t s) { launch<attn_bwd_onepass_kernel, 448, OP_LDS>(dim3(BH), s, a); }

void launch_bwd(const MhAttnProblem& p, hipStream_t s) {
    const AttnArgs a = to_args(p);
    const bool dr = has_drop(p);
    const int S = p.S, BH = p.B * p.H;
    if (onepass_fits(p)) launch_onepass(a, BH, s);
    else if (S <= 128) bwd_sweeps<4, 2>(dr, dim3(1, BH), s, a);
    else if (S <= 224) bwd_sweeps<7, 0>(dr, dim3(1, BH), s, a);
    else bwd_sweeps<4, 0>(dr, dim3((S + 127) / 128, BH), s, a);
}

bool dual_pair(const MhAttnProblem* p, int n, int& ia, int& ib) {
    if (n != 2) return false;
    for (int k = 0; k < 2; ++k) {
        const MhAttnProblem &a = p[k], &b = p[1 - k];
        if (a.S > 128 && a.S <= 224 && !has_drop(a) && b.S <= 128) {
            ia = k;
            ib = 1 - k;
            return true;
        }
    }
    return false;
}

}

extern "C" int mh_attn_fwd_grouped(const MhAttnProblem* p, int n, mh_stream_t stream) {
    if (!p || n < 1 || n > MH_ATTN_MAX_GROUP) return MH_EINVAL;
    for (int i = 0; i < n; ++i)
        if (int st = check_problem(p[i], false)) return st;
    hipStream_t s = (hipStream_t)stream;
    int ia, ib;
    if (dual_pair(p, n, ia, ib)) {
        const AttnArgs A = to_args(p[ia]), Bp = to_args(p[ib]);
        const int nA = p[ia].B * p[ia].H, nB = p[ib].B * p[ib].H;
        const dim3 grid(1, nA + nB);
        has_drop(p[ib]) ? launch<attn_fwd_dual_kernel<4, true>, 448, LDS_FWD_DUAL>(grid, s, A, Bp, nA)
                        : launch<attn_fwd_dual_kernel<4, false>, 448, LDS_FWD_DUAL>(grid, s, A, Bp, nA);
    } else {
        for (int i = 0; i < n; ++i) launch_fwd(p[i], s);
    }
    return mh_launch_status();
}

extern "C" int mh_attn_bwd_grouped(const MhAttnProblem* p, int n, mh_stream_t stream) {
    if (!p || n < 1 || n > MH_ATTN_MAX_GROUP) return MH_EINVAL;
    for (int i = 0; i < n; ++i)
        if (int st = check_problem(p[i], true)) return st;
    hipStream_t s = (hipStream_t)stream;
    int ia, ib;
    if (dual_pair(p, n, ia, ib)) {
        const AttnArgs A = to_args(p[ia]), Bp = to_args(p[ib]);
        const int nA = p[ia].B * p[ia].H, nB = p[ib].B * p[ib].H;
        const bool dr = has_drop(p[ib]);
        if (!onepass_fits(p[ia])) {
            const dim3 grid(1, 2 * (nA + nB));
            dr ? launch<attn_bwd_merged_dual_kernel<2, true>, 448, LDS_BWD_DUAL>(grid, s, A, Bp, nA, nB)
               : launch<attn_bwd_merged_dual_kernel<2, false>, 448, LDS_BWD_DUAL>(grid, s, A, Bp, nA, nB);
        } else if (g_onepass == 2) {
            const dim3 grid(1, nA + 2 * nB);
            dr ? launch<attn_bwd_onepass_dual_kernel<2, true>, 448, OP_LDS>(grid, s, A, Bp, nA, nB)
               : launch<attn_bwd_onepass_dual_kernel<2, false>, 448, OP_LDS>(grid, s, A, Bp, nA, nB);
        } else {
            launch_onepass(A, nA, s);
            const dim3 grid(1, 2 * nB);
            dr ? launch<attn_bwd_merged_single_kernel<2, true>, 256, LDS_BWD_TEXT>(grid, s, Bp, nB)
               : launch<attn_bwd_merged_single_kernel<2, false>, 256, LDS_BWD_TEXT>(grid, s, Bp, nB);
        }
    } else {
        for (int i = 0; i < n; ++i) launch_bwd(p[i], s);
    }
    return mh_launch_status();
}

extern "C" int mh_attn_set_onepass(int on) {
    g_onepass = on < 0 ? 2 : on;
    return MH_OK;
}

static MhAttnProblem one_problem(const void* qkv, const int64_t* key_mask, const void* out, float* lse, const void* dout,
                                 float* delta, void* dqkv, const int32_t* cu, const int32_t* row_map, int B, int S, int H,
                                 const uint32_t* rng, float drop_p, uint32_t drop_stream) {
    MhAttnProblem p;
    p.qkv = qkv; p.key_mask = key_mask; p.out = (void*)out; p.lse = lse;
    p.dout = dout; p.delta = delta; p.dqkv = dqkv;
    p.cu = cu; p.row_map = row_map;
    p.rng = rng; p.drop_p = drop_p; p.drop_stream = drop_stream;
    p.B = B; p.S = S; p.H = H; p.reserved = 0;
    return p;
}

extern "C" int mh_attn_fwd(const void* qkv, const int64_t* key_mask, void* out, float* lse, int B, int S,
                           int H, const uint32_t* rng, float drop_p, uint32_t drop_stream, mh_stream_t stream) {
    const MhAttnProblem p = one_problem(qkv, key_mask, out, lse, nullptr, nullptr, nullptr, nullptr, nullptr, B, S, H, rng,
                                        drop_p, drop_stream);
    return mh_attn_fwd_grouped(&p, 1, stream);
}
extern "C" int mh_attn_fwd_packed(const void* qkv, const int64_t* key_mask, void* out, float* lse, const int32_t* cu,
                                  const int32_t* row_map, int B, int S, int H, const uint32_t* rng, float drop_p,
                                  uint32_t drop_stream, mh_stream_t stream) {
    if (!cu) return MH_EINVAL;
    const MhAttnProblem p = one_problem(qkv, key_mask, out, lse, nullptr, nullptr, nullptr, cu, row_map, B, S, H, rng,
                                        drop_p, drop_stream);
    return mh_attn_fwd_grouped(&p, 1, stream);
}
extern "C" int mh_attn_bwd(const void* qkv, const int64_t* key_mask, const void* out, const void* dout,
                           const float* lse, float* delta, void* dqkv, int B, int S, int H, const uint32_t* rng,
                           float drop_p, uint32_t drop_stream, mh_stream_t stream) {
    const MhAttnProblem p = one_problem(qkv, key_mask, out, (float*)lse, dout, delta, dqkv, nullptr, nullptr, B, S, H, rng,
                                        drop_p, drop_stream);
    return mh_attn_bwd_grouped(&p, 1, stream);
}
extern "C" int mh_attn_bwd_packed(const void* qkv, const int64_t* key_mask, const void* out, const void* dout,
                                  const float* lse, float* delta, void* dqkv, const int32_t* cu, const int32_t* row_map,
                                  int B, int S, int H, const uint32_t* rng, float drop_p, uint32_t drop_stream,
                                  mh_stream_t stream) {
    if (!cu) return MH_EINVAL;
    const MhAttnProblem p = one_problem(qkv, key_mask, out, (float*)lse, dout, delta, dqkv, cu, row_map, B, S, H, rng,
                                        drop_p, drop_stream);
    return mh_attn_bwd_grouped(&p, 1, stream);
}
```

### multimodal_propaganda_meme_classification_amd/engine.py

```python
from __future__ import annotations

import ctypes as C
from collections import namedtuple
from typing import Callable, Dict, List, NamedTuple, Optional, Tuple

import torch

from . import _lib
from ._lib import (MH_GEMM_DERIV_AUX, MH_GEMM_GELU, MH_GEMM_OUT_F32, MH_GEMM_QUICK_GELU, MhAttnProblem, MhColsumJob, MhGemmProblem, MhHeadGrads,
                   MhHeadParams, MhLnBwdJob, MhLnFwdJob, MhRowsJob)
from .config import Layout, ModelConfig, check_sequence_length

BF16, F32, I64 = torch.bfloat16, torch.float32, torch.int64
LN_PARTS = 512

LAUNCH, PY, WAIT = "launch", "py", "wait"


class Call(NamedTuple):
    fn: Optional[Callable]
    args: object
    name: str
    tag: str
    work: object
    lane: int
    kind: str = LAUNCH


class Segment:

    def __init__(self, name: str, lib=None):
        self.name = name
        self.lib = lib if lib is not None else _lib.load()
        self.calls: List[Call] = []

    def c(self, fn_name: str, *args, tag: Optional[str] = None, work: float = 0.0, lane: int = 0):
        self.calls.append(Call(getattr(self.lib, fn_name), args, fn_name, tag or fn_name, work, lane))

    def py(self, fn: Callable[[], None]):
        self.calls.append(Call(None, fn, PY, PY, 0.0, 0, PY))

    def wait(self, key: str):
        self.calls.append(Call(None, key, WAIT, WAIT, 0.0, 0, WAIT))

    def run(self, stream: int):
        for fn, args, name, _, _, _, kind in self.calls:
            if fn is None:
                if kind == PY:
                    args()
            else:
                st = fn(*args, stream)
                if st != 0:
                    _lib.check(st, name)

    def run2(self, main: "torch.cuda.Stream", side: Optional["torch.cuda.Stream"], events: Dict[str, "torch.cuda.Event"]):
        mp = main.cuda_stream
        sp = side.cuda_stream if side is not None else mp
        forked1 = False
        for fn, args, name, _, _, lane, kind in self.calls:
            if fn is None:
                if kind == PY:
                    args()
                elif kind == WAIT:
                    if args in events:
                        main.wait_event(events.pop(args))
                continue
            if lane == 1 and side is not None:
                if not forked1:
                    e = torch.cuda.Event()
                    e.record(main)
                    side.wait_event(e)
                    forked1 = True
                st = fn(*args, sp)
            else:
                st = fn(*args, mp)
            if st != 0:
                _lib.check(st, name)
        if forked1:
            d = torch.cuda.Event()
            d.record(side)
            events[self.name] = d

    def run_timed(self, stream: int, tag: str, out: list, dyn_scale: float = 1.0):
        for fn, args, name, t, work, _, kind in self.calls:
            if isinstance(work, tuple):
                work = work[0] + work[1] * dyn_scale
            if fn is None:
                if kind == PY:
                    args()
                continue
            if t == tag:
                e0, e1 = torch.cuda.Event(enable_timing=True), torch.cuda.Event(enable_timing=True)
                e0.record()
                st = fn(*args, stream)
                e1.record()
                out.append((e0, e1, work))
            else:
                st = fn(*args, stream)
            if st != 0:
                _lib.check(st, name)

    def __len__(self):
        return len(self.calls)


def _ptr(t: Optional[torch.Tensor]):
    return None if t is None else t.data_ptr()


class Plan:
    def __init__(self, B: int, S: int, lib=None):
        self.B, self.S = B, S
        self.lib = lib
        self.buf: Dict[str, torch.Tensor] = {}
        self.keep: list = []
        self.fwd = Segment("fwd", lib)
        self.loss = Segment("loss", lib)
        self.bwd: List[Segment] = []
        self.bucket_after: Dict[str, Tuple[int, int]] = {}
        self.n_launches = 0
        self.gemm_flops = 0.0
        self.gemm_flops_dyn = 0.0
        self.packed = False
        self.dropout_on = False
        self.features = False
        self.last_rows = "all"
        self.gather = None
        self._ln_jobs: Dict[int, list] = {}


class Engine:
    def __init__(self, cfg: ModelConfig, layout: Layout, P: torch.Tensor, G: torch.Tensor, SH: torch.Tensor):
        self.cfg, self.layout = cfg, layout
        self.P, self.G, self.SH = P, G, SH
        self.dev = P.device
        assert P.is_cuda and G.is_cuda and SH.is_cuda, "memehip needs HIP device buffers (no CPU fallback)"
        self.kind = cfg.compute_dtype
        self.T16 = torch.float16 if self.kind == "fp16" else torch.bfloat16
        assert SH.dtype == self.T16
        self.lib = _lib.load(self.kind)
        self.gscale = cfg.stream_scale
        self.pack_text = cfg.pack_text
        self.plans: Dict[Tuple[int, int], Plan] = {}
        self.word_row_live = torch.zeros(cfg.text.vocab_size, dtype=torch.uint8, device=self.dev)
        self.word_first = torch.full((cfg.text.vocab_size,), 0x7fffffff, dtype=torch.int32, device=self.dev)
        self.word_count = torch.zeros(cfg.text.vocab_size, dtype=torch.int32, device=self.dev)
        self.loss_scale = torch.ones(1, dtype=F32, device=self.dev)

    def _slice(self, flat: torch.Tensor, name: str, count: int = 1) -> torch.Tensor:
        s = self.layout.spec[name]
        return flat[s.offset:s.offset + s.numel * count]

    def p(self, name, count=1):
        return self._slice(self.P, name, count)

    def g(self, name, count=1):
        return self._slice(self.G, name, count)

    def w(self, name, count=1):
        s = self.layout.spec[name]
        assert s.offset + s.numel * count <= self.layout.n_shadow, name
        return self.SH[s.offset:s.offset + s.numel * count]

    def before_backward(self, plan: Plan):
        last = getattr(self, "_last_bwd_plan", None)
        if last is not None and last is not plan:
            gword = self.g("bert.embeddings.word_embeddings.weight")
            for key in ("prev_ids_all", "prev_ids"):
                prev = last.buf.get(key)
                if prev is not None:
                    st = self.lib.mh_zero_rows_f32(prev.data_ptr(), gword.data_ptr(), prev.numel(), self.cfg.text.hidden,
                                                   self.cfg.text.vocab_size, torch.cuda.current_stream().cuda_stream)
                    _lib.check(st, "mh_zero_rows_f32")
                    prev.zero_()
        self._last_bwd_plan = plan

    def plan(self, B: int, S: int, training: bool = True, gather_world: int = 0, features=False,
             last_rows: str = "pooled") -> Plan:
        if last_rows not in ("pooled", "all"):
            raise ValueError(f"last_rows must be 'pooled' or 'all', got {last_rows!r}")
        cfg = self.cfg
        has_drop = (cfg.text.hidden_dropout > 0 or cfg.text.attention_dropout > 0 or cfg.head_dropout > 0)
        features = features if features == "sequence" else bool(features)
        pack = self.pack_text and features != "sequence"
        key = (B, S, bool(training and has_drop), int(gather_world), pack, features) + (() if last_rows == "pooled" else (last_rows,))
        if key not in self.plans:
            self.plans[key] = self._build(B, S, key[2], key[3], key[4], key[5], last_rows=last_rows)
        return self.plans[key]

    def _build(self, B: int, S: int, dropout_on: bool = False, gather_world: int = 0, pack: bool = False,
               features=False, last_rows: str = "pooled") -> Plan:
        b = _PlanBuilder(self, B, S, dropout_on, gather_world, pack, features, last_rows)
        nl = max(b.text.L, b.image.L)
        b.text_embed()
        b.image_embed()
        b.last_layer_form()
        b.layer_buffers()
        for l in range(nl):
            b.fwd_layer(l)
        b.head_and_loss()
        b.bwd_head()
        for l in range(nl - 1, -1, -1):
            b.bwd_layer(l)
        b.bwd_embed()
        pl = b.pl
        pl.n_launches = sum(1 for sg in [pl.fwd, pl.loss] + pl.bwd for c in sg.calls if c[0] is not None)
        return pl



Site = namedtuple("Site", "rng p sid", defaults=(None, 0.0, 0))
NO_DROP = Site()

Gemm = namedtuple("Gemm", "A B C M N K lda ldb ldc bias residual aux mul rowsum gelu quick deriv_aux alpha drop rows_dev drop_rows",
                  defaults=(None, None, None, None, None, False, False, False, 1.0, NO_DROP, None, None))
LnFwd = namedtuple("LnFwd", "x gamma beta y mean rstd rows D eps y32 rows_dev", defaults=(None, None))
LnBwd = namedtuple("LnBwd", "dy x gamma mean rstd dx part rows D dx_add dx_drop drop rows_dev drop_rows",
                   defaults=(None, None, NO_DROP, None, None))
Attn = namedtuple("Attn", "qkv out lse B S H key_mask cu row_map drop dout delta dqkv", defaults=(None, None, None, NO_DROP, None, None, None))
RowsJob = namedtuple("RowsJob", "n rows D idx stride offset src dst rows_dev", defaults=(None, 0, 0, None, None, None))

TextActs = namedtuple("TextActs", "qkv ctx lse a y m1 r1 h g f m2 r2 pctx x rows")
ImageActs = namedtuple("ImageActs", "u m1 r1 qkv ctx lse xp w m2 r2 h g pctx x rows")

Roles = namedtuple("Roles", "attn_in proj_out ffn_in ffn_res ffn_out")

Grads = namedtuple("Grads", "d_out dh d_mid d_proj res dctx res_full dctx_full dqkv d_in df", defaults=(None,))


class Tower:

    def __init__(self, pre, c, T, S, attn, ln_mid, post_ln, quick=False, p_h=0.0, p_a=0.0):
        self.pre, self.T, self.S = pre, T, S
        self.D, self.I, self.H, self.L, self.eps = c.hidden, c.intermediate, c.heads, c.layers, c.ln_eps
        self.attn, self.ln_mid = attn, ln_mid
        self.post_ln, self.quick = post_ln, quick
        self.p_h, self.p_a = p_h, p_a
        self.rows_dev = self.row_map = self.key_mask = self.cu = None
        self.pool, self.compact = None, 0
        self.x, self.acts = [], []
        self.dX, self.d_last = [], None
        self.grads, self.delta = [], None

    def rows(self, l: int) -> int:
        return self.compact if (self.compact and l == self.L - 1) else self.T

    @property
    def out_rows(self) -> int:
        return self.compact or self.T

    def live(self, M: int, drop: bool = False) -> dict:
        if self.rows_dev is None or M != self.T:
            return {}
        return dict(rows_dev=self.rows_dev, drop_rows=self.row_map) if drop else dict(rows_dev=self.rows_dev)

    def name(self, l: int, stem: str) -> str:
        return f"{self.pre}encoder.layer.{l}.{stem}"

    def roles(self, l: int) -> Roles:
        a = self.acts[l]
        return Roles(self.x[l], a.a, a.y, a.y, a.f) if self.post_ln else Roles(a.u, a.xp, a.w, a.xp, self.x[l + 1])

    def d_x(self, l: int) -> torch.Tensor:
        return self.d_last if l == self.L - 1 else self.dX[(self.L - 1 - l) % 3]


def _fill_ln_fwd(e: MhLnFwdJob, j: LnFwd):
    assert j.x.numel() >= j.rows * j.D and j.y.numel() >= j.rows * j.D
    e.x, e.gamma, e.beta, e.y, e.y_f32 = _ptr(j.x), _ptr(j.gamma), _ptr(j.beta), _ptr(j.y), _ptr(j.y32)
    e.mean, e.rstd, e.rows, e.eps = _ptr(j.mean), _ptr(j.rstd), j.rows, j.eps
    e.rows_dev = _ptr(j.rows_dev)


def _fill_ln_bwd(e: MhLnBwdJob, j: LnBwd):
    n = j.rows * j.D
    assert j.dy.numel() >= n and j.x.numel() >= n and j.dx.numel() >= n
    assert j.dx_add is None or j.dx_add.numel() >= n
    e.dy, e.x, e.gamma, e.mean, e.rstd = _ptr(j.dy), _ptr(j.x), _ptr(j.gamma), _ptr(j.mean), _ptr(j.rstd)
    e.dx_add, e.dx, e.part, e.dx_drop, e.rng = _ptr(j.dx_add), _ptr(j.dx), _ptr(j.part), _ptr(j.dx_drop), j.drop.rng
    e.n_part, e.rows, e.drop_p, e.drop_stream = LN_PARTS, j.rows, j.drop.p, j.drop.sid
    e.rows_dev, e.drop_rows = _ptr(j.rows_dev), _ptr(j.drop_rows)


TXT, IMG = "bert.", "image_model."


class _PlanBuilder:

    def __init__(self, eng: Engine, B: int, S: int, dropout_on: bool, gather_world: int, pack: bool, features, last_rows: str):
        cfg, t, v = eng.cfg, eng.cfg.text, eng.cfg.image
        check_sequence_length(t, S)
        if B > 1024:
            raise ValueError("batch > 1024 not supported by the loss kernel")
        self.eng, self.cfg, self.B, self.S = eng, cfg, B, S
        self.T16 = eng.T16
        self.pl = pl = Plan(B, S, eng.lib)
        self.gather_world, self.last_rows = gather_world, last_rows
        pl.dropout_on, pl.packed, pl.features = dropout_on, pack, features
        self.rng = self.alloc("rng", (4,), torch.int32, zero=True)
        self.p_head = cfg.head_dropout if dropout_on else 0.0
        self.pool_index = 0 if cfg.pool == "cls" else S - 1
        self.text = Tower(TXT, t, B * S, S, "attention.self.", "attention.output.LayerNorm", post_ln=True,
                          p_h=t.hidden_dropout if dropout_on else 0.0, p_a=t.attention_dropout if dropout_on else 0.0)
        self.image = Tower(IMG, v, B * v.n_tokens, v.n_tokens, "attention.attention.", "layernorm_after", post_ln=False,
                           quick=v.act == "quick_gelu")
        self.towers = (self.text, self.image)

    def alloc(self, name, shape, dtype=None, zero=False):
        tns = (torch.zeros if zero else torch.empty)(shape, dtype=dtype or self.T16, device=self.eng.dev)
        self.pl.buf[name] = tns
        return tns

    def site(self, p_, sid) -> Site:
        return Site(self.rng.data_ptr(), float(p_), int(sid)) if p_ > 0 else NO_DROP

    def seg(self, name) -> Segment:
        s = Segment(name, self.eng.lib)
        self.pl.bwd.append(s)
        return s

    def _gemm(self, seg: Segment, probs: List[Gemm], a_k: bool, b_k: bool, lane: int = 0):
        n, pl, T16 = len(probs), self.pl, self.T16
        assert 1 <= n <= _lib.MH_GEMM_MAX_GROUP
        arr = (MhGemmProblem * n)()
        for e, d in zip(arr, probs):
            A, Bm, Cm, M, N, K, lda, ldb, ldc = d[:9]
            assert A.dtype == T16 and Bm.dtype == T16 and Cm.dtype in (T16, F32)
            a_need = (K - 1) * lda + M if a_k else (M - 1) * lda + K
            b_need = (K - 1) * ldb + N if b_k else (N - 1) * ldb + K
            assert A.numel() >= a_need and Bm.numel() >= b_need and Cm.numel() >= (M - 1) * ldc + N, (M, N, K)
            for key, t, dt, need in (("bias", d.bias, F32, N), ("residual", d.residual, T16, (M - 1) * ldc + N),
                                     ("aux", d.aux, T16, (M - 1) * ldc + N), ("mul", d.mul, T16, (M - 1) * ldc + N),
                                     ("rowsum", d.rowsum, F32, M)):
                assert t is None or (t.dtype == dt and t.numel() >= need), key
            e.A, e.B, e.C = _ptr(A), _ptr(Bm), _ptr(Cm)
            e.bias, e.residual, e.aux = _ptr(d.bias), _ptr(d.residual), _ptr(d.aux)
            e.mul, e.rowsum = _ptr(d.mul), _ptr(d.rowsum)
            e.M, e.N, e.K, e.lda, e.ldb, e.ldc = M, N, K, lda, ldb, ldc
            e.flags = (MH_GEMM_GELU if d.gelu else 0) | (MH_GEMM_OUT_F32 if Cm.dtype == F32 else 0) | \
                      (MH_GEMM_QUICK_GELU if d.quick else 0) | (MH_GEMM_DERIV_AUX if d.deriv_aux else 0)
            e.alpha = float(d.alpha)
            if d.drop.rng is not None:
                e.drop_rng, e.drop_p, e.drop_stream = d.drop
                e.drop_rows = _ptr(d.drop_rows)
            e.rows_dev = _ptr(d.rows_dev)
        pl.keep.append(arr)
        fl = [2.0 * d.M * d.N * d.K for d in probs]
        dyn = float(sum(x for x, d in zip(fl, probs) if d.rows_dev is not None))
        fixed = float(sum(fl)) - dyn
        pl.gemm_flops += fixed + dyn
        pl.gemm_flops_dyn += dyn
        seg.c("mh_gemm_bf16_grouped", arr, n, int(a_k), int(b_k), tag=f"gemm<{int(a_k)},{int(b_k)}>", work=(fixed, dyn),
              lane=lane)

    @staticmethod
    def _fwd_prob(x, w, out, T, N, K, **kw) -> Gemm:
        return Gemm(x, w, out, T, N, K, lda=K, ldb=K, ldc=N, **kw)

    @staticmethod
    def _dgrad_prob(dy, w, out, T, N_out, K_in, **kw) -> Gemm:
        return Gemm(dy, w, out, T, K_in, N_out, lda=N_out, ldb=K_in, ldc=K_in, **kw)

    def _wgrad_prob(self, dy, x, dw, db, T, N_out, K_in, **kw) -> Gemm:
        return Gemm(dy, x, dw, N_out, K_in, T, lda=N_out, ldb=K_in, ldc=K_in, rowsum=db, alpha=1.0 / self.eng.gscale, **kw)

    def _linear(self, tw: Tower, l, stem, x, out, M, N, K, count=1, **kw) -> Gemm:
        nm = tw.name(l, stem)
        return self._fwd_prob(x, self.eng.w(nm + ".weight", count), out, M, N, K, bias=self.eng.p(nm + ".bias", count), **kw)

    def _linear_dgrad(self, tw: Tower, l, stem, dy, out, M, N_out, K_in, count=1, **kw) -> Gemm:
        return self._dgrad_prob(dy, self.eng.w(tw.name(l, stem) + ".weight", count), out, M, N_out, K_in, **kw)

    def _linear_wgrad(self, tw: Tower, l, stem, dy, x, M, N_out, K_in, count=1, **kw) -> Gemm:
        nm = tw.name(l, stem)
        return self._wgrad_prob(dy, x, self.eng.g(nm + ".weight", count), self.eng.g(nm + ".bias", count), M, N_out, K_in, **kw)

    def _ln_fwd_job(self, x, name, y, mean, rstd, rows, D, eps, y32=None, rows_dev=None) -> LnFwd:
        return LnFwd(x, self.eng.p(name + ".weight"), self.eng.p(name + ".bias"), y, mean, rstd, rows, D, float(eps), y32, rows_dev)

    def _ln_bwd_job(self, dy, x, name, mean, rstd, dx, rows, D, dx_add=None, dx_drop=None, drop=NO_DROP, rows_dev=None,
                    drop_rows=None) -> LnBwd:
        part = self.alloc(f"lnpart.{name}.weight", (2, LN_PARTS, D), F32)
        self.pl._ln_jobs.setdefault(D, []).append((part, self.eng.g(name + ".weight"), self.eng.g(name + ".bias")))
        on = drop.rng is not None and dx_drop is not None
        return LnBwd(dy, x, self.eng.p(name + ".weight"), mean, rstd, dx, part, rows, D, dx_add, dx_drop if on else None,
                     drop if on else NO_DROP, rows_dev, drop_rows if on else None)

    def _ln(self, seg: Segment, jobs: list, fn_name: str, struct, fill):
        by_d: Dict[int, list] = {}
        for j in jobs:
            if j is not None:
                by_d.setdefault(j.D, []).append(j)
        for D, js in by_d.items():
            assert len(js) <= _lib.MH_LN_MAX_JOBS
            arr = (struct * len(js))()
            for e, j in zip(arr, js):
                fill(e, j)
            self.pl.keep.append(arr)
            seg.c(fn_name, arr, len(js), D)

    def _ln_fwd(self, seg: Segment, jobs: List[Optional[LnFwd]]):
        self._ln(seg, jobs, "mh_layernorm_fwd_grouped", MhLnFwdJob, _fill_ln_fwd)

    def _ln_bwd(self, seg: Segment, jobs: List[Optional[LnBwd]]):
        self._ln(seg, jobs, "mh_layernorm_bwd_grouped", MhLnBwdJob, _fill_ln_bwd)

    def _attn(self, seg: Segment, probs: List[Attn], backward: bool):
        arr = (MhAttnProblem * len(probs))()
        for e, d in zip(arr, probs):
            for k in ("qkv", "key_mask", "out", "lse", "dout", "delta", "dqkv", "cu", "row_map"):
                setattr(e, k, _ptr(getattr(d, k)))
            e.rng, e.drop_p, e.drop_stream = d.drop
            e.B, e.S, e.H = d.B, d.S, d.H
            n = d.B * d.S * d.H * 64
            assert d.qkv.numel() >= 3 * n and d.out.numel() >= n and d.lse.numel() >= d.B * d.H * d.S
            if backward:
                assert d.dout.numel() >= n and d.dqkv.numel() >= 3 * n and d.delta.numel() >= d.B * d.H * d.S
        self.pl.keep.append(arr)
        seg.c("mh_attn_bwd_grouped" if backward else "mh_attn_fwd_grouped", arr, len(probs))

    def _attn_prob(self, tw: Tower, l: int, **bw) -> Attn:
        a = tw.acts[l]
        return Attn(a.qkv, a.ctx, a.lse, self.B, tw.S, tw.H, tw.key_mask, tw.cu, tw.row_map,
                    self.site(tw.p_a, 16 * (l + 1) + 1), **bw)

    def _rows(self, seg: Segment, jobs: List[RowsJob], scatter: bool):
        if not jobs:
            return
        assert len(jobs) <= _lib.MH_ROWS_MAX_JOBS
        arr = (MhRowsJob * len(jobs))()
        for e, j in zip(arr, jobs):
            full, compact = (j.dst, j.src) if scatter else (j.src, j.dst)
            assert j.src.dtype == self.T16 and j.dst.dtype == self.T16 and full.numel() >= j.rows * j.D and compact.numel() >= j.n * j.D
            assert j.idx is None or (j.idx.dtype == torch.int32 and j.idx.numel() >= j.n)
            e.src, e.dst, e.idx, e.rows_dev = _ptr(j.src), _ptr(j.dst), _ptr(j.idx), _ptr(j.rows_dev if scatter else None)
            e.n, e.rows, e.D, e.stride, e.offset = j.n, j.rows, j.D, j.stride, j.offset
        self.pl.keep.append(arr)
        seg.c("mh_rows_scatter_zero" if scatter else "mh_rows_gather", arr, len(jobs))

    def text_embed(self):
        eng, f, tw, t, B, S, alloc = self.eng, self.pl.fwd, self.text, self.cfg.text, self.B, self.S, self.alloc
        Tt, Dt = tw.T, tw.D
        self.ids, self.mask = alloc("ids", (B, S), I64, zero=True), alloc("mask", (B, S), I64, zero=True)
        self.prev_ids = alloc("prev_ids", (B, S), I64, zero=True)
        self.pre0 = alloc("t.pre0", (Tt, Dt))
        x0d = alloc("t.x0", (Tt, Dt))
        self.m0, self.r0 = alloc("t.m0", (Tt,), F32), alloc("t.r0", (Tt,), F32)
        type0 = eng.p(TXT + "embeddings.token_type_embeddings.weight")[:Dt] if t.type_vocab > 0 else None
        embed = (_ptr(self.ids), _ptr(eng.p(TXT + "embeddings.word_embeddings.weight")),
                 _ptr(eng.p(TXT + "embeddings.position_embeddings.weight")), _ptr(type0),
                 _ptr(eng.p(TXT + "embeddings.LayerNorm.weight")), _ptr(eng.p(TXT + "embeddings.LayerNorm.bias")),
                 _ptr(self.pre0), _ptr(x0d), _ptr(self.m0), _ptr(self.r0), B, S, Dt, t.vocab_size, float(t.ln_eps), *self.site(tw.p_h, 1))
        if t.position_scheme == "roberta":
            pos_ids = alloc("t.pos_ids", (B, S), torch.int32, zero=True)
            self.pos_inv = alloc("t.pos_inv", (B, t.max_position), torch.int32, zero=True)
            f.c("mh_position_ids_from_input_ids", _ptr(self.ids), _ptr(pos_ids), _ptr(self.pos_inv), B, S, int(t.pad_token_id),
                t.max_position)
            f.c("mh_bert_embed_fwd_pos", *embed, _ptr(pos_ids), t.max_position)
        else:
            f.c("mh_bert_embed_fwd", *embed)
        if self.pl.packed:
            I32 = torch.int32
            cu, row_map = alloc("pk.cu", (B + 1,), I32, zero=True), alloc("pk.row_map", (Tt,), I32, zero=True)
            self.inv_map, pmask = alloc("pk.inv_map", (Tt,), I32, zero=True), alloc("pk.pmask", (Tt,), I64, zero=True)
            self.pool_rows, n_rows = alloc("pk.pool_rows", (B,), I32, zero=True), alloc("pk.n_rows", (1,), I32, zero=True)
            f.c("mh_pack_plan", _ptr(self.mask), B, S, self.pool_index, _ptr(cu), _ptr(row_map), _ptr(self.inv_map), _ptr(pmask),
                _ptr(self.pool_rows), _ptr(n_rows))
            tw.x.append(alloc("t.x0p", (Tt, Dt)))
            f.c("mh_pack_rows", _ptr(x0d), _ptr(row_map), _ptr(n_rows), _ptr(tw.x[0]), Tt, Dt)
            tw.rows_dev, tw.row_map, tw.key_mask, tw.cu = n_rows, row_map, pmask, cu
            tw.pool = RowsJob(B, Tt, Dt, idx=self.pool_rows)
        else:
            self.inv_map = self.pool_rows = None
            tw.x.append(x0d)
            tw.key_mask = self.mask
            tw.pool = RowsJob(B, Tt, Dt, stride=S, offset=self.pool_index)

    def image_embed(self):
        eng, f, tw, v, B, alloc = self.eng, self.pl.fwd, self.image, self.cfg.image, self.B, self.alloc
        Np, Ti, Di = v.n_patches, tw.T, tw.D
        Kp, Kpp = v.patch_dim, v.patch_dim_padded
        image = alloc("image", (B, v.channels, v.image_size, v.image_size), F32, zero=True)
        self.patches = alloc("i.patches", (B * Np, Kpp))
        proj = alloc("i.proj", (B * Np, Di))
        tw.x.append(alloc("i.x0", (Ti, Di)))
        tw.pool = RowsJob(B, Ti, Di, stride=tw.S, offset=0)
        wp = eng.w(IMG + "embeddings.patch_embeddings.projection.weight")
        if Kpp == Kp and v.patch % 8 == 0:
            f.c("mh_patchify", _ptr(image), _ptr(self.patches), B, v.channels, v.image_size, v.image_size, v.patch)
        else:
            f.c("mh_patchify_ld", _ptr(image), _ptr(self.patches), B, v.channels, v.image_size, v.image_size, v.patch, Kpp)
        if Kpp != Kp:
            wpad = alloc("i.wp_pad", (Di, Kpp))
            f.c("mh_copy2d_u32", _ptr(wp), Kp // 2, _ptr(wpad), Kpp // 2, Di, Kp // 2, Kpp // 2)
            wp = wpad
        pbias = eng.p(IMG + "embeddings.patch_embeddings.projection.bias") if v.patch_bias else None
        self._gemm(f, [self._fwd_prob(self.patches, wp, proj, B * Np, Di, Kpp, bias=pbias)], False, False)
        x0 = alloc("i.x0pre", (Ti, Di)) if v.pre_ln else tw.x[0]
        f.c("mh_vit_assemble_fwd", _ptr(proj), _ptr(eng.p(IMG + "embeddings.cls_token")),
            _ptr(eng.p(IMG + "embeddings.position_embeddings")), _ptr(x0), B, Np, Di)
        if v.pre_ln:
            self._ln_fwd(f, [self._ln_fwd_job(x0, IMG + "pre_layernorm", tw.x[0], alloc("i.mpre", (Ti,), F32),
                                              alloc("i.rpre", (Ti,), F32), Ti, Di, v.ln_eps)])

    def last_layer_form(self):
        pl, B, t, v = self.pl, self.B, self.text, self.image
        cmp = self.last_rows == "pooled" and pl.features != "sequence" and not pl.dropout_on and t.L >= 1 and v.L >= 1
        pl.last_rows = "pooled" if cmp else "all"
        self.head_rows = (1, 1, 0, None) if cmp else (t.S, v.S, self.pool_index, self.pool_rows)
        for tw, n in ((t, "t"), (v, "i")):
            tw.compact = B if cmp else 0
            tw.dX = [self.alloc(f"{n}.dX{i}", (tw.T, tw.D)) for i in range(3)]
            tw.d_last = self.alloc(f"{n}.dXrows", (B, tw.D)) if cmp else tw.dX[0]
        self.zero_fill = not cmp

    def layer_buffers(self):
        B, t, v, alloc = self.B, self.text, self.image, self.alloc
        self.xt_last32 = alloc("t.xlast32", (t.out_rows, t.D), F32)
        self.xf32 = alloc("i.xf32", (v.out_rows, v.D), F32)
        for l in range(t.L):
            R, n = t.rows(l), f"t{l}."
            ctx = alloc(n + "ctx", (t.T, t.D))
            t.acts.append(TextActs(
                qkv=alloc(n + "qkv", (t.T, 3 * t.D)), ctx=ctx, lse=alloc(n + "lse", (B, t.H, t.S), F32), a=alloc(n + "a", (R, t.D)),
                y=alloc(n + "y", (R, t.D)), m1=alloc(n + "m1", (R,), F32), r1=alloc(n + "r1", (R,), F32),
                h=alloc(n + "h", (R, t.I)), g=alloc(n + "g", (R, t.I)), f=alloc(n + "f", (R, t.D)),
                m2=alloc(n + "m2", (R,), F32), r2=alloc(n + "r2", (R,), F32),
                pctx=alloc(n + "pctx", (B, t.D)) if R != t.T else ctx, x=alloc(n + "xrows", (B, t.D)) if R != t.T else t.x[l], rows=R))
            t.x.append(alloc(f"t.x{l + 1}", (R, t.D)))
        for l in range(v.L):
            R, n = v.rows(l), f"i{l}."
            ctx = alloc(n + "ctx", (v.T, v.D))
            v.acts.append(ImageActs(
                u=alloc(n + "u", (v.T, v.D)), m1=alloc(n + "m1", (v.T,), F32), r1=alloc(n + "r1", (v.T,), F32),
                qkv=alloc(n + "qkv", (v.T, 3 * v.D)), ctx=ctx, lse=alloc(n + "lse", (B, v.H, v.S), F32),
                xp=alloc(n + "xp", (R, v.D)), w=alloc(n + "w", (R, v.D)), m2=alloc(n + "m2", (R,), F32), r2=alloc(n + "r2", (R,), F32),
                h=alloc(n + "h", (R, v.I)), g=alloc(n + "g", (R, v.I)),
                pctx=alloc(n + "pctx", (B, v.D)) if R != v.T else ctx, x=alloc(n + "xrows", (B, v.D)) if R != v.T else v.x[l], rows=R))
            v.x.append(alloc(f"i.x{l + 1}", (R, v.D)))
        self.xf = alloc("i.xf", (v.out_rows, v.D))
        self.mf, self.rf = alloc("i.mf", (v.out_rows,), F32), alloc("i.rf", (v.out_rows,), F32)
        self._ln_fwd(self.pl.fwd, [self._img_ln1(0)])

    def _img_ln1(self, l) -> Optional[LnFwd]:
        v = self.image
        if l < v.L:
            b = v.acts[l]
            return self._ln_fwd_job(v.x[l], v.name(l, "layernorm_before"), b.u, b.m1, b.r1, v.T, v.D, v.eps)
        if l == v.L:
            return self._ln_fwd_job(v.x[l], IMG + "layernorm", self.xf, self.mf, self.rf, v.out_rows, v.D, v.eps, y32=self.xf32)
        return None

    def fwd_layer(self, l):
        f, t, v = self.pl.fwd, self.text, self.image
        lay = [(tw, tw.acts[l], tw.roles(l), tw.rows(l)) for tw in self.towers if l < tw.L]
        a, b = (t.acts[l] if l < t.L else None), (v.acts[l] if l < v.L else None)
        self._gemm(f, [self._linear(tw, l, tw.attn + "query", r.attn_in, a_.qkv, tw.T, 3 * tw.D, tw.D, 3, **tw.live(tw.T))
                       for tw, a_, r, M in lay], False, False)
        self._attn(f, [self._attn_prob(tw, l) for tw, _, _, _ in reversed(lay)], backward=False)
        self._rows(f, [j for tw, a_, r, M in lay if M != tw.T
                       for j in (tw.pool._replace(src=a_.ctx, dst=a_.pctx), tw.pool._replace(src=tw.x[l], dst=a_.x))], scatter=False)
        self._gemm(f, [self._linear(tw, l, "attention.output.dense", a_.pctx, r.proj_out, M, tw.D, tw.D, residual=a_.x,
                                    drop=self.site(tw.p_h, 16 * (l + 1) + 2), **tw.live(M, drop=True)) for tw, a_, r, M in lay], False, False)
        self._ln_fwd(f, [
            self._ln_fwd_job(a.a, t.name(l, t.ln_mid), a.y, a.m1, a.r1, a.rows, t.D, t.eps, **t.live(a.rows)) if a else None,
            self._ln_fwd_job(b.xp, v.name(l, v.ln_mid), b.w, b.m2, b.r2, b.rows, v.D, v.eps) if b else None])
        self._gemm(f, [self._linear(tw, l, "intermediate.dense", r.ffn_in, a_.g, M, tw.I, tw.D, aux=a_.h, gelu=True, deriv_aux=True,
                                    quick=tw.quick, **tw.live(M)) for tw, a_, r, M in lay], False, False)
        self._gemm(f, [self._linear(tw, l, "output.dense", a_.g, r.ffn_out, M, tw.D, tw.I, residual=r.ffn_res,
                                    drop=self.site(tw.p_h, 16 * (l + 1) + 3), **tw.live(M, drop=True)) for tw, a_, r, M in lay], False, False)
        self._ln_fwd(f, [
            self._ln_fwd_job(a.f, t.name(l, "output.LayerNorm"), t.x[l + 1], a.m2, a.r2, a.rows, t.D, t.eps,
                             y32=self.xt_last32 if l == t.L - 1 else None, **t.live(a.rows)) if a else None,
            self._img_ln1(l + 1) if b else None])

    def head_and_loss(self):
        eng, pl, f, B, alloc, t, v = self.eng, self.pl, self.pl.fwd, self.B, self.alloc, self.text, self.image
        P_, Cn = self.cfg.proj, self.cfg.num_classes
        self.hp, self.hg = MhHeadParams(), MhHeadGrads()
        for fld, nm in (("Wt", "bert_fc.weight"), ("bt", "bert_fc.bias"), ("Wi", "image_fc.weight"),
                        ("bi", "image_fc.bias"), ("Wf", "fusion_fc.weight"), ("bf_", "fusion_fc.bias"),
                        ("Wo", "output_fc.weight"), ("bo", "output_fc.bias")):
            setattr(self.hp, fld, _ptr(eng.p(nm)))
            setattr(self.hg, fld, _ptr(eng.g(nm)))
        pl.keep += [self.hp, self.hg]
        self.pooled = alloc("h.pooled", (B, t.D + v.D), F32)
        self.feat, self.fused = alloc("h.feat", (B, 2 * P_), F32), alloc("h.fused", (B, P_), F32)
        logits = alloc("logits", (B, Cn), F32)
        S_h, Nt_h, pool_h, rows_h = self.head_rows
        if pl.features == "sequence":
            assert not pl.packed
            self.d_seq_t, self.d_seq_i = alloc("h.d_seq_t", (t.T, t.D), F32, zero=True), alloc("h.d_seq_i", (v.T, v.D), F32, zero=True)
        elif pl.features:
            self.d_pooled = alloc("h.d_pooled", (B, t.D + v.D), F32, zero=True)
            f.c("mh_pool_fwd", _ptr(self.xt_last32), _ptr(self.xf32), pool_h, _ptr(self.pooled), B, S_h, Nt_h, t.D, v.D, _ptr(rows_h))
        else:
            f.c("mh_head_fwd", C.byref(self.hp), _ptr(self.xt_last32), _ptr(self.xf32), pool_h, _ptr(self.pooled), _ptr(self.feat),
                _ptr(self.fused), _ptr(logits), B, S_h, Nt_h, t.D, v.D, P_, Cn, *self.site(self.p_head, 7), _ptr(rows_h))
        labels, loss = alloc("labels", (B,), I64, zero=True), alloc("loss", (1,), F32, zero=True)
        self.dlogits = alloc("dlogits", (B, Cn), F32, zero=True)
        ncorrect = alloc("ncorrect", (1,), torch.int32, zero=True)
        pl.loss.c("mh_ce_fwd_bwd", _ptr(logits), _ptr(labels), _ptr(loss), _ptr(self.dlogits), _ptr(ncorrect), B, Cn,
                  1.0, _ptr(eng.loss_scale))

    def bwd_head(self):
        eng, pl, B, alloc, t, v = self.eng, self.pl, self.B, self.alloc, self.text, self.image
        P_, Cn = self.cfg.proj, self.cfg.num_classes
        s = self.seg("bwd_head")
        dXf = alloc("i.dXf", (v.out_rows, v.D))
        dfeat, dfused = alloc("h.dfeat", (B, 2 * P_), F32), alloc("h.dfused", (B, P_), F32)
        S_h, Nt_h, pool_h, rows_h = self.head_rows
        if self.zero_fill:
            s.py(t.d_last.zero_)
            s.py(dXf.zero_)
        if pl.features:
            h0 = eng.layout.spec["bert_fc.weight"].offset
            h1 = eng.layout.spec["output_fc.bias"].offset + eng.layout.spec["output_fc.bias"].numel
            head_grads = eng.G[h0:h1]
            s.py(head_grads.zero_)
            if pl.features == "sequence":
                s.c("mh_cast_f32_bf16", _ptr(self.d_seq_t), _ptr(t.d_last), t.T * t.D)
                s.c("mh_cast_f32_bf16", _ptr(self.d_seq_i), _ptr(dXf), v.T * v.D)
            else:
                s.c("mh_pool_bwd", _ptr(self.d_pooled), _ptr(t.d_last), _ptr(dXf), pool_h, B, S_h, Nt_h, t.D, v.D, float(eng.gscale),
                    _ptr(rows_h))
        else:
            s.c("mh_head_bwd", C.byref(self.hp), C.byref(self.hg), _ptr(self.dlogits), _ptr(self.pooled), _ptr(self.feat),
                _ptr(self.fused), _ptr(dfeat), _ptr(dfused), _ptr(t.d_last), _ptr(dXf), pool_h, B, S_h, Nt_h, t.D, v.D, P_, Cn,
                float(eng.gscale), *self.site(self.p_head, 7), _ptr(rows_h))
        t.grads, v.grads = self._text_grads(), self._image_grads()
        self.t_dpre = alloc("t.dpre", (t.T, t.D))
        self._ln_bwd(s, [
            self._ln_bwd_job(dXf, v.x[v.L], IMG + "layernorm", self.mf, self.rf, v.d_last, v.out_rows, v.D),
            self._text_ln2_bwd(t.L - 1) if t.L >= v.L else None])

    def _text_grads(self) -> List[Grads]:
        t, B, alloc = self.text, self.B, self.alloc
        dh = [alloc(f"t.dh{i}", (t.T, t.I)) for i in range(2)]
        da = [alloc(f"t.da{i}", (t.T, t.D)) for i in range(2)]
        dqkv = [alloc(f"t.dqkv{i}", (t.T, 3 * t.D)) for i in range(2)]
        dam = [alloc(f"t.dam{i}", (t.T, t.D)) for i in range(2)] if t.p_h > 0 else da
        df = [alloc(f"t.df{i}", (t.T, t.D)) for i in range(3)]
        dfm = [alloc(f"t.dfm{i}", (t.T, t.D)) for i in range(3)] if t.p_h > 0 else df
        dy, dctx = alloc("t.dy", (t.T, t.D)), alloc("t.dctx", (t.T, t.D))
        t.delta = alloc("t.delta", (B, t.H, t.S), F32)
        out = [Grads(d_out=dfm[l % 3], dh=dh[l & 1], d_mid=dy, d_proj=dam[l & 1], res=da[l & 1], dctx=dctx, res_full=da[l & 1],
                     dctx_full=dctx, dqkv=dqkv[l & 1], d_in=t.d_x(l - 1), df=df[l % 3]) for l in range(t.L)]
        if t.compact:
            c_df, c_dh, c_dy = alloc("t.dfrows", (B, t.D)), alloc("t.dhrows", (B, t.I)), alloc("t.dyrows", (B, t.D))
            c_da, c_dctx = alloc("t.darows", (B, t.D)), alloc("t.dctxrows", (B, t.D))
            if t.rows(t.L - 1) != t.T:
                out[-1] = out[-1]._replace(d_out=c_df, dh=c_dh, d_mid=c_dy, d_proj=c_da, res=c_da, dctx=c_dctx, df=c_df)
        return out

    def _image_grads(self) -> List[Grads]:
        v, B, alloc = self.image, self.B, self.alloc
        dh = [alloc(f"i.dh{i}", (v.T, v.I)) for i in range(2)]
        dxp = [alloc(f"i.dxp{i}", (v.T, v.D)) for i in range(2)]
        dqkv = [alloc(f"i.dqkv{i}", (v.T, 3 * v.D)) for i in range(2)]
        dw, dctx, du = alloc("i.dw", (v.T, v.D)), alloc("i.dctx", (v.T, v.D)), alloc("i.du", (v.T, v.D))
        v.delta = alloc("i.delta", (B, v.H, v.S), F32)
        out = [Grads(d_out=v.d_x(l), dh=dh[l & 1], d_mid=dw, d_proj=dxp[l & 1], res=dxp[l & 1], dctx=dctx, res_full=dxp[l & 1],
                     dctx_full=dctx, dqkv=dqkv[l & 1], d_in=du) for l in range(v.L)]
        if v.compact:
            c_dh, c_dw = alloc("i.dhrows", (B, v.I)), alloc("i.dwrows", (B, v.D))
            c_dxp, c_dctx = alloc("i.dxprows", (B, v.D)), alloc("i.dctxrows", (B, v.D))
            if v.rows(v.L - 1) != v.T:
                out[-1] = out[-1]._replace(dh=c_dh, d_mid=c_dw, d_proj=c_dxp, res=c_dxp, dctx=c_dctx)
        return out

    def _text_ln2_bwd(self, l) -> Optional[LnBwd]:
        t = self.text
        if not (0 <= l < t.L):
            return None
        a, g = t.acts[l], t.grads[l]
        return self._ln_bwd_job(t.d_x(l), a.f, t.name(l, "output.LayerNorm"), a.m2, a.r2, g.df, a.rows, t.D, dx_drop=g.d_out,
                                drop=self.site(t.p_h, 16 * (l + 1) + 3), **t.live(a.rows, drop=True))

    def _text_embed_ln_bwd(self, s: Segment) -> LnBwd:
        t = self.text
        d_emb = t.d_x(-1)
        if self.pl.packed:
            d_emb = self.alloc("t.dX_dense", (t.T, t.D))
            s.c("mh_unpack_rows", _ptr(t.d_x(-1)), _ptr(self.inv_map), _ptr(d_emb), t.T, t.D)
        if t.p_h > 0:
            s.c("mh_dropout_apply", _ptr(d_emb), t.T * t.D, self.rng.data_ptr(), float(t.p_h), 1)
        return self._ln_bwd_job(d_emb, self.pre0, TXT + "embeddings.LayerNorm", self.m0, self.r0, self.t_dpre, t.T, t.D)

    def bwd_layer(self, l):
        t, v = self.text, self.image
        s = self.seg(f"bwd_layer_{l}")
        s.wait(f"bwd_layer_{l + 2}")
        lay = [(tw, tw.acts[l], tw.roles(l), tw.grads[l], tw.rows(l)) for tw in self.towers if l < tw.L]
        a, ga = (t.acts[l], t.grads[l]) if l < t.L else (None, None)
        b, gb = (v.acts[l], v.grads[l]) if l < v.L else (None, None)
        self._gemm(s, [self._linear_dgrad(tw, l, "output.dense", g.d_out, g.dh, M, tw.D, tw.I, mul=a_.h, deriv_aux=True, quick=tw.quick,
                                          **tw.live(M)) for tw, a_, r, g, M in lay], False, True)
        self._gemm(s, [self._linear_dgrad(tw, l, "intermediate.dense", g.dh, g.d_mid, M, tw.I, tw.D, residual=g.df, **tw.live(M))
                       for tw, a_, r, g, M in lay], False, True)
        self._ln_bwd(s, [
            self._ln_bwd_job(ga.d_mid, a.a, t.name(l, t.ln_mid), a.m1, a.r1, ga.res, a.rows, t.D, dx_drop=ga.d_proj,
                             drop=self.site(t.p_h, 16 * (l + 1) + 2), **t.live(a.rows, drop=True)) if a else None,
            self._ln_bwd_job(gb.d_mid, b.xp, v.name(l, v.ln_mid), b.m2, b.r2, gb.res, b.rows, v.D, dx_add=gb.d_out) if b else None])
        self._gemm(s, [self._linear_dgrad(tw, l, "attention.output.dense", g.d_proj, g.dctx, M, tw.D, tw.D, **tw.live(M))
                       for tw, a_, r, g, M in lay], False, True)
        self._rows(s, [j for tw, a_, r, g, M in lay if M != tw.T
                       for j in (tw.pool._replace(src=g.dctx, dst=g.dctx_full, rows_dev=tw.rows_dev),
                                 tw.pool._replace(src=g.res, dst=g.res_full, rows_dev=tw.rows_dev))], scatter=True)
        self._attn(s, [self._attn_prob(tw, l, dout=g.dctx_full, delta=tw.delta, dqkv=g.dqkv) for tw, a_, r, g, M in reversed(lay)],
                   backward=True)
        self._gemm(s, [self._linear_dgrad(tw, l, tw.attn + "query", g.dqkv, g.d_in, tw.T, 3 * tw.D, tw.D, 3,
                                          residual=g.res_full if tw.post_ln else None, **tw.live(tw.T)) for tw, a_, r, g, M in lay], False, True)
        t_job = self._text_ln2_bwd(l - 1) if l >= 1 else self._text_embed_ln_bwd(s)
        self._ln_bwd(s, [
            t_job,
            self._ln_bwd_job(gb.d_in, v.x[l], v.name(l, "layernorm_before"), b.m1, b.r1, v.d_x(l - 1), v.T, v.D,
                             dx_add=gb.res_full) if b else None])
        for tw, a_, r, g, M in lay:
            self._gemm(s, [
                self._linear_wgrad(tw, l, "output.dense", g.d_out, a_.g, M, tw.D, tw.I, **tw.live(M)),
                self._linear_wgrad(tw, l, "intermediate.dense", g.dh, r.ffn_in, M, tw.I, tw.D, **tw.live(M)),
                self._linear_wgrad(tw, l, "attention.output.dense", g.d_proj, a_.pctx, M, tw.D, tw.D, **tw.live(M)),
                self._linear_wgrad(tw, l, tw.attn + "query", g.dqkv, r.attn_in, tw.T, 3 * tw.D, tw.D, 3, **tw.live(tw.T))],
                True, True, lane=1)
        rng = [r for r in self.eng.layout.layer_ranges if r[0] == l][0]
        self.pl.bucket_after[s.name] = (rng[1], rng[2])

    def bwd_embed(self):
        eng, pl, B, alloc, v, tw = self.eng, self.pl, self.B, self.alloc, self.cfg.image, self.image
        Np, Ti, Di = v.n_patches, tw.T, tw.D
        s = self.seg("bwd_embed")
        i_dproj = alloc("i.dproj", (B * Np, Di))
        d_x0 = tw.d_x(-1)
        if v.pre_ln:
            d_x0 = alloc("i.dx0pre", (Ti, Di))
            self._ln_bwd(s, [self._ln_bwd_job(tw.d_x(-1), pl.buf["i.x0pre"], IMG + "pre_layernorm", pl.buf["i.mpre"], pl.buf["i.rpre"],
                                              d_x0, Ti, Di)])
        s.c("mh_vit_assemble_bwd", _ptr(d_x0), _ptr(i_dproj), _ptr(eng.g(IMG + "embeddings.cls_token")),
            _ptr(eng.g(IMG + "embeddings.position_embeddings")), B, Np, Di, 1.0 / eng.gscale)
        self._patch_wgrad(s, i_dproj)
        if self.gather_world <= 0:
            self._table_grads(s, self.ids, self.t_dpre, self.prev_ids, B)
        for D, jobs in pl._ln_jobs.items():
            for i0 in range(0, len(jobs), _lib.MH_COLSUM_MAX_JOBS):
                chunk = jobs[i0:i0 + _lib.MH_COLSUM_MAX_JOBS]
                arr = (MhColsumJob * len(chunk))()
                for j, (part, o0, o1) in enumerate(chunk):
                    arr[j].part, arr[j].out0, arr[j].out1 = _ptr(part), _ptr(o0), _ptr(o1)
                pl.keep.append(arr)
                s.c("mh_colsum_partials_f32", arr, len(chunk), LN_PARTS, D, 1.0 / eng.gscale)
        tail0 = eng.layout.layer_ranges[-1][2]
        if self.gather_world <= 0:
            pl.bucket_after[s.name] = (tail0, eng.layout.n_total)
        else:
            self._bwd_embed_tables(s, tail0)

    def _patch_wgrad(self, s: Segment, i_dproj):
        eng, pl, alloc, v, Di = self.eng, self.pl, self.alloc, self.cfg.image, self.image.D
        Kp, Kpp, Tp = v.patch_dim, v.patch_dim_padded, self.B * v.n_patches
        gw = gw_out = eng.g(IMG + "embeddings.patch_embeddings.projection.weight")
        gb = eng.g(IMG + "embeddings.patch_embeddings.projection.bias") if v.patch_bias else None
        if Kpp != Kp:
            gw = alloc("i.dwp_pad", (Di * Kpp,), F32)
        nsplit = min(_lib.MH_GEMM_MAX_GROUP, max(1, Tp // 512))
        if nsplit > 1:
            chunk = -(-Tp // nsplit)
            chunk = -(-chunk // 8) * 8
            part_w = alloc("i.dwp_part", (2, nsplit, Di * Kpp), F32)
            part_b = alloc("i.dbp_part", (2, nsplit, Di), F32)
            probs = []
            for i in range(nsplit):
                k0 = i * chunk
                kk = min(chunk, Tp - k0)
                if kk <= 0:
                    part_w[0, i].zero_(), part_b[0, i].zero_()
                    continue
                probs.append(self._wgrad_prob(i_dproj[k0:], self.patches[k0:], part_w[0, i], part_b[0, i], kk, Di, Kpp))
            self._gemm(s, probs, True, True)
            for part, out, D_ in ((part_w, gw, Di * Kpp), (part_b, gb, Di)):
                if out is None:
                    continue
                arr = (MhColsumJob * 1)()
                arr[0].part, arr[0].out0, arr[0].out1 = _ptr(part), _ptr(out), None
                pl.keep.append(arr)
                s.c("mh_colsum_partials_f32", arr, 1, nsplit, D_, 1.0)
        else:
            self._gemm(s, [self._wgrad_prob(i_dproj, self.patches, gw, gb, Tp, Di, Kpp)], True, True)
        if Kpp != Kp:
            s.c("mh_copy2d_u32", _ptr(gw), Kpp, _ptr(gw_out), Kp, Di, Kp, Kp)

    def _table_grads(self, sg: Segment, ids_, dpre_, prev_, nb):
        eng, t, S, Dt = self.eng, self.cfg.text, self.S, self.text.D
        gword = eng.g(TXT + "embeddings.word_embeddings.weight")
        gtype0 = eng.g(TXT + "embeddings.token_type_embeddings.weight")[:Dt] if t.type_vocab > 0 else None
        gpos = eng.g(TXT + "embeddings.position_embeddings.weight")
        sg.c("mh_zero_rows_f32", _ptr(prev_), _ptr(gword), nb * S, Dt, t.vocab_size)
        roberta = t.position_scheme == "roberta"
        dpos = self.alloc("t.dpos_by_s", (S, Dt), F32) if roberta else gpos
        sg.c("mh_bert_embed_bwd", _ptr(ids_), _ptr(dpre_), _ptr(gword), _ptr(dpos), _ptr(gtype0), nb, S, Dt, t.vocab_size,
             int(t.pad_token_id), 1.0 / eng.gscale, eng.word_row_live.data_ptr(), eng.word_first.data_ptr(),
             eng.word_count.data_ptr())
        if roberta:
            pos_inv = self.pos_inv
            if ids_ is not self.ids:
                pos_ids = self.alloc("t.pos_ids_all", (nb, S), torch.int32, zero=True)
                pos_inv = self.alloc("t.pos_inv_all", (nb, t.max_position), torch.int32, zero=True)
                sg.c("mh_position_ids_from_input_ids", _ptr(ids_), _ptr(pos_ids), _ptr(pos_inv), nb, S, int(t.pad_token_id),
                     t.max_position)
            sg.c("mh_embed_pos_bwd", _ptr(dpre_), _ptr(pos_inv), _ptr(gpos), None, None, nb, S, Dt, t.max_position,
                 1.0 / eng.gscale)
        sg.py(lambda: prev_.copy_(ids_))

    def _bwd_embed_tables(self, s: Segment, tail0: int):
        eng, pl, t, B, S, W, alloc = self.eng, self.pl, self.cfg.text, self.B, self.S, self.gather_world, self.alloc
        Tt, Dt = self.text.T, self.text.D
        first_tbl = TXT + ("embeddings.token_type_embeddings.weight" if t.type_vocab > 0
                           else "embeddings.position_embeddings.weight")
        tbl0 = eng.layout.spec[first_tbl].offset
        assert eng.layout.spec[TXT + "embeddings.word_embeddings.weight"].offset + t.vocab_size * Dt + 3 >= eng.layout.n_total - 3
        pl.bucket_after[s.name] = (tail0, tbl0)
        ids_all = alloc("ids_all", (W * B, S), I64, zero=True)
        prev_all = alloc("prev_ids_all", (W * B, S), I64, zero=True)
        dpre_all = alloc("t.dpre_all", (W * Tt, Dt))
        pl.gather = [(self.ids, ids_all), (self.t_dpre, dpre_all)]
        self._table_grads(self.seg("bwd_embed_tables"), ids_all, dpre_all, prev_all, W * B)
```

### multimodal_propaganda_meme_classification_amd/ops.py

```python
from __future__ import annotations

import ctypes as C
from typing import Optional, Sequence

import torch

from . import _lib
from ._lib import (MH_GEMM_ACCUM, MH_GEMM_DERIV_AUX, MH_GEMM_GELU, MH_GEMM_OUT_F32, MH_GEMM_QUICK_GELU, MhColsumJob, MhGemmProblem, MhHeadGrads,
                   MhHeadParams, check)

BF16, F16, F32, I64 = torch.bfloat16, torch.float16, torch.float32, torch.int64
H16 = (BF16, F16)


def _stream() -> int:
    return torch.cuda.current_stream().cuda_stream


def _p(t: Optional[torch.Tensor]) -> Optional[int]:
    return None if t is None else t.data_ptr()


def _kind(t: torch.Tensor) -> str:
    return "fp16" if t.dtype == F16 else "bf16"
# ... 187 lines not shown
    y = torch.empty_like(x) if y is None else _chk(y, BF16, "y")
    mean = torch.empty(rows, dtype=F32, device=x.device) if mean is None else mean
    rstd = torch.empty(rows, dtype=F32, device=x.device) if rstd is None else rstd
    if y_f32 is not None:
        _chk(y_f32, F32, "y_f32")
        assert y_f32.numel() >= rows * D
    check(_L(x).mh_layernorm_fwd(_p(x), _p(gamma), _p(beta), _p(y), _p(y_f32), _p(mean), _p(rstd), rows, D,
                                       float(eps), _stream()), "mh_layernorm_fwd")
    return y, mean, rstd


def layernorm_bwd(dy, x, gamma, mean, rstd, part, dx=None, dx_add=None, dx_drop=None, drop=None):
    _chk(dy, BF16, "dy"), _chk(x, BF16, "x"), _chk(gamma, F32, "gamma"), _chk(part, F32, "part")
    rows, D = x.shape
    n_part = part.shape[1]
    assert part.shape == (2, n_part, D) and mean.numel() >= rows and rstd.numel() >= rows
    dx = torch.empty_like(x) if dx is None else _chk(dx, BF16, "dx")
    r, p, sid = _drop(drop)
    check(_L(x).mh_layernorm_bwd(_p(dy), _p(x), _p(gamma), _p(mean), _p(rstd), _p(dx_add), _p(dx), _p(part),
                                 n_part, rows, D, _p(dx_drop), r, p, sid, _stream()), "mh_layernorm_bwd")
    return dx


def colsum_partials(jobs, n_part: int, D: int, scale: float = 1.0):
    for i in range(0, len(jobs), _lib.MH_COLSUM_MAX_JOBS):
        chunk = jobs[i:i + _lib.MH_COLSUM_MAX_JOBS]
        arr = (MhColsumJob * len(chunk))()
        for j, (part, o0, o1) in enumerate(chunk):
            _chk(part, F32, "part")
            assert part.numel() >= 2 * n_part * D
            for o in (o0, o1):
                if o is not None:
                    _chk(o, F32, "out", False)
                    assert o.numel() >= D
            arr[j].part, arr[j].out0, arr[j].out1 = _p(part), _p(o0), _p(o1)
        check(_lib.load().mh_colsum_partials_f32(arr, len(chunk), n_part, D, float(scale), _stream()), "mh_colsum_partials_f32")



def attn_fwd(qkv, key_mask, B, S, H, out=None, lse=None, drop=None):
    _chk(qkv, BF16, "qkv")
    assert qkv.numel() == B * S * 3 * H * 64
    if key_mask is not None:
        _chk(key_mask, I64, "key_mask")
        assert key_mask.numel() == B * S
    out = torch.empty((B * S, H * 64), dtype=qkv.dtype, device=qkv.device) if out is None else _chk(out, BF16, "out")
    lse = torch.empty((B, H, S), dtype=F32, device=qkv.device) if lse is None else _chk(lse, F32, "lse")
    assert out.numel() == B * S * H * 64 and lse.numel() == B * H * S
    r, p, sid = _drop(drop)
    check(_L(qkv).mh_attn_fwd(_p(qkv), _p(key_mask), _p(out), _p(lse), B, S, H, r, p, sid, _stream()), "mh_attn_fwd")
    return out, lse


def pack_plan(mask, pool_index: int):
    _chk(mask, I64, "mask")
    B, S = mask.shape
    dev = mask.device
    I32 = torch.int32
    out = dict(cu=torch.empty(B + 1, dtype=I32, device=dev), row_map=torch.empty(B * S, dtype=I32, device=dev),
               inv_map=torch.empty(B * S, dtype=I32, device=dev), pmask=torch.empty(B * S, dtype=I64, device=dev),
               pool_rows=torch.empty(B, dtype=I32, device=dev), n_rows=torch.empty(1, dtype=I32, device=dev))
    check(_lib.load().mh_pack_plan(_p(mask), B, S, int(pool_index), _p(out["cu"]), _p(out["row_map"]), _p(out["inv_map"]),
                                   _p(out["pmask"]), _p(out["pool_rows"]), _p(out["n_rows"]), _stream()), "mh_pack_plan")
    return out


def pack_rows(src, plan, D):
    _chk(src, BF16, "src")
    max_rows = plan["row_map"].numel()
    assert src.numel() == max_rows * D
    dst = torch.zeros_like(src)
    check(_L(src).mh_pack_rows(_p(src), _p(plan["row_map"]), _p(plan["n_rows"]), _p(dst), max_rows, D, _stream()),
          "mh_pack_rows")
    return dst


def unpack_rows(src, plan, D):
    _chk(src, BF16, "src")
    max_rows = plan["inv_map"].numel()
    assert src.numel() == max_rows * D
    dst = torch.empty_like(src)
    check(_L(src).mh_unpack_rows(_p(src), _p(plan["inv_map"]), _p(dst), max_rows, D, _stream()), "mh_unpack_rows")
    return dst


def _rows_jobs(jobs, scatter: bool):
    assert 1 <= len(jobs) <= _lib.MH_ROWS_MAX_JOBS
    arr = (_lib.MhRowsJob * len(jobs))()
    for e, j in zip(arr, jobs):
        src, dst, idx = _chk(j["src"], BF16, "src"), _chk(j["dst"], BF16, "dst"), j.get("idx")
        assert src.dim() == 2 and dst.dim() == 2 and src.dtype == dst.dtype and src.shape[1] == dst.shape[1]
        full, compact = (dst, src) if scatter else (src, dst)
        n, D = compact.shape
        if idx is not None:
            _chk(idx, torch.int32, "idx")
            assert idx.numel() == n
        e.src, e.dst, e.idx, e.rows_dev = _p(src), _p(dst), _p(idx), _p(j.get("rows_dev") if scatter else None)
        e.n, e.rows, e.D, e.stride, e.offset = n, full.shape[0], D, int(j.get("stride", 0)), int(j.get("offset", 0))
    return arr


def rows_gather(jobs):
    arr = _rows_jobs(jobs, False)
    check(_L(jobs[0]["src"]).mh_rows_gather(arr, len(jobs), _stream()), "mh_rows_gather")


def rows_scatter_zero(jobs):
    arr = _rows_jobs(jobs, True)
    check(_L(jobs[0]["src"]).mh_rows_scatter_zero(arr, len(jobs), _stream()), "mh_rows_scatter_zero")


def attn_fwd_packed(qkv, plan, B, S, H, drop=None):
    _chk(qkv, BF16, "qkv")
    assert qkv.numel() == B * S * 3 * H * 64
    out = torch.zeros((B * S, H * 64), dtype=qkv.dtype, device=qkv.device)
    lse = torch.zeros((B, H, S), dtype=F32, device=qkv.device)
    r, p, sid = _drop(drop)
    check(_L(qkv).mh_attn_fwd_packed(_p(qkv), _p(plan["pmask"]), _p(out), _p(lse), _p(plan["cu"]), _p(plan["row_map"]),
                                     B, S, H, r, p, sid, _stream()), "mh_attn_fwd_packed")
    return out, lse


def attn_bwd_packed(qkv, plan, out, dout, lse, B, S, H, drop=None):
    _chk(qkv, BF16, "qkv"), _chk(out, BF16, "out"), _chk(dout, BF16, "dout"), _chk(lse, F32, "lse")
    assert qkv.numel() == B * S * 3 * H * 64 and out.numel() == B * S * H * 64 == dout.numel()
    dqkv = torch.zeros_like(qkv)
    delta = torch.empty((B, H, S), dtype=F32, device=qkv.device)
    r, p, sid = _drop(drop)
    check(_L(qkv).mh_attn_bwd_packed(_p(qkv), _p(plan["pmask"]), _p(out), _p(dout), _p(lse), _p(delta), _p(dqkv),
                                     _p(plan["cu"]), _p(plan["row_map"]), B, S, H, r, p, sid, _stream()),
          "mh_attn_bwd_packed")
    return dqkv


def attn_grouped(problems, backward: bool = False):
    from ._lib import MhAttnProblem
    arr = (MhAttnProblem * len(problems))()
    for e, d in zip(arr, problems):
        _chk(d["qkv"], BF16, "qkv"), _chk(d["out"], BF16, "out"), _chk(d["lse"], F32, "lse")
        n = d["B"] * d["S"] * d["H"] * 64
        assert d["qkv"].numel() >= 3 * n and d["out"].numel() >= n and d["lse"].numel() >= d["B"] * d["H"] * d["S"]
        if backward:
            _chk(d["dout"], BF16, "dout"), _chk(d["dqkv"], BF16, "dqkv"), _chk(d["delta"], F32, "delta")
            assert d["dout"].numel() >= n and d["dqkv"].numel() >= 3 * n and d["delta"].numel() >= d["B"] * d["H"] * d["S"]
        for k in ("qkv", "key_mask", "out", "lse", "dout", "delta", "dqkv", "cu", "row_map"):
            setattr(e, k, _p(d.get(k)))
        e.rng, e.drop_p, e.drop_stream = _drop(d.get("drop"))
        e.B, e.S, e.H = d["B"], d["S"], d["H"]
    lib = _L(problems[0]["qkv"])
    fn = lib.mh_attn_bwd_grouped if backward else lib.mh_attn_fwd_grouped
    check(fn(arr, len(problems), _stream()), "mh_attn_bwd_grouped" if backward else "mh_attn_fwd_grouped")


def attn_bwd(qkv, key_mask, out, dout, lse, B, S, H, dqkv=None, delta=None, drop=None):
    _chk(qkv, BF16, "qkv"), _chk(out, BF16, "out"), _chk(dout, BF16, "dout"), _chk(lse, F32, "lse")
    assert qkv.numel() == B * S * 3 * H * 64 and out.numel() == B * S * H * 64 == dout.numel()
    assert lse.numel() == B * H * S
    dqkv = torch.empty_like(qkv) if dqkv is None else _chk(dqkv, BF16, "dqkv")
    delta = torch.empty((B, H, S), dtype=F32, device=qkv.device) if delta is None else _chk(delta, F32, "delta")
    assert dqkv.numel() == qkv.numel() and delta.numel() == B * H * S
    r, p, sid = _drop(drop)
    check(_L(qkv).mh_attn_bwd(_p(qkv), _p(key_mask), _p(out), _p(dout), _p(lse), _p(delta), _p(dqkv), B, S, H,
                              r, p, sid, _stream()), "mh_attn_bwd")
    return dqkv



def bert_embed_fwd(ids, word, pos, type0, gamma, beta, eps, pre, y, mean, rstd, drop=None):
    _chk(ids, I64, "ids"), _chk(word, F32, "word"), _chk(pos, F32, "pos")
    B, S = ids.shape
    V, D = word.shape
    assert pos.shape[0] >= S and pos.shape[1] == D
    assert pre.numel() >= B * S * D and y.numel() >= B * S * D and mean.numel() >= B * S and rstd.numel() >= B * S
    check(_L(pre).mh_bert_embed_fwd(_p(ids), _p(word), _p(pos), _p(type0), _p(gamma), _p(beta),
                                        _p(_chk(pre, BF16, "pre")), _p(_chk(y, BF16, "y")), _p(mean), _p(rstd), B, S,
                                        D, V, float(eps), *_drop(drop), _stream()), "mh_bert_embed_fwd")


def bert_embed_bwd(ids, d_pre, dword, dpos, dtype0, pad_id: int, scale: float = 1.0, row_live=None, index=None):
    _chk(ids, I64, "ids"), _chk(d_pre, BF16, "d_pre"), _chk(dword, F32, "dword"), _chk(dpos, F32, "dpos")
    B, S = ids.shape
    V, D = dword.shape
    assert d_pre.numel() >= B * S * D and dpos.shape[0] >= S
    check(_L(d_pre).mh_bert_embed_bwd(_p(ids), _p(d_pre), _p(dword), _p(dpos), _p(dtype0), B, S, D, V, int(pad_id),
                                      float(scale), _p(row_live), _p(index[0]) if index else None,
                                      _p(index[1]) if index else None, _stream()), "mh_bert_embed_bwd")


def position_ids_from_input_ids(ids, pad_id: int, max_position: int, pos_ids=None, pos_inv=None, kind: str = "bf16"):
    _chk(ids, I64, "ids")
    B, S = ids.shape
    I32 = torch.int32
    pos_ids = torch.empty((B, S), dtype=I32, device=ids.device) if pos_ids is None else _chk(pos_ids, I32, "pos_ids")
    pos_inv = torch.empty((B, max_position), dtype=I32, device=ids.device) if pos_inv is None else _chk(pos_inv, I32, "pos_inv")
    assert pos_ids.numel() >= B * S and pos_inv.numel() >= B * max_position
    check(_lib.load(kind).mh_position_ids_from_input_ids(_p(ids), _p(pos_ids), _p(pos_inv), B, S, int(pad_id), int(max_position),
                                                         _stream()), "mh_position_ids_from_input_ids")
    return pos_ids, pos_inv


def bert_embed_fwd_pos(ids, pos_ids, word, pos, type0, gamma, beta, eps, pre, y, mean, rstd, drop=None):
    _chk(ids, I64, "ids"), _chk(pos_ids, torch.int32, "pos_ids"), _chk(word, F32, "word"), _chk(pos, F32, "pos")
    B, S = ids.shape
    V, D = word.shape
    assert pos_ids.numel() >= B * S and pos.shape[1] == D
    assert pre.numel() >= B * S * D and y.numel() >= B * S * D and mean.numel() >= B * S and rstd.numel() >= B * S
    check(_L(pre).mh_bert_embed_fwd_pos(_p(ids), _p(word), _p(pos), _p(type0), _p(gamma), _p(beta), _p(_chk(pre, BF16, "pre")),
                                        _p(_chk(y, BF16, "y")), _p(mean), _p(rstd), B, S, D, V, float(eps), *_drop(drop),
                                        _p(pos_ids), pos.shape[0], _stream()), "mh_bert_embed_fwd_pos")


def embed_pos_bwd(d_pre, pos_inv, dpos, dtype0=None, scratch=None, scale: float = 1.0):
    _chk(d_pre, BF16, "d_pre"), _chk(pos_inv, torch.int32, "pos_inv"), _chk(dpos, F32, "dpos")
    B, P = pos_inv.shape
    D = dpos.shape[1]
    S = d_pre.numel() // (B * D)
    assert d_pre.numel() == B * S * D and dpos.shape[0] == P
    if dtype0 is not None:
        _chk(dtype0, F32, "dtype0"), _chk(scratch, F32, "scratch")
        assert dtype0.numel() >= D and scratch.numel() >= S * D
    check(_L(d_pre).mh_embed_pos_bwd(_p(d_pre), _p(pos_inv), _p(dpos), _p(dtype0), _p(scratch), B, S, D, P, float(scale),
                                     _stream()), "mh_embed_pos_bwd")


def zero_rows(ids, table):
    _chk(ids, I64, "ids"), _chk(table, F32, "table")
    V, D = table.shape
    check(_lib.load().mh_zero_rows_f32(_p(ids), _p(table), ids.numel(), D, V, _stream()), "mh_zero_rows_f32")


def image_normalize_u8(images_u8, mean, std, out=None):
    if not (images_u8.is_cuda and images_u8.dtype == torch.uint8 and images_u8.dim() == 4 and images_u8.shape[-1] == 3
            and images_u8.is_contiguous()):
        raise _lib.MemehipError("image_normalize_u8: expected a contiguous uint8 [B,H,W,3] tensor on the HIP device")
    B, H, W, _ = images_u8.shape
    out = torch.empty((B, 3, H, W), dtype=F32, device=images_u8.device) if out is None else _chk(out, F32, "out")
    m = (C.c_float * 3)(*[float(x) for x in mean])
    sd = (C.c_float * 3)(*[float(x) for x in std])
    check(_lib.load().mh_image_normalize_u8(_p(images_u8), _p(out), B, H, W, m, sd, _stream()), "mh_image_normalize_u8")
    return out


def patchify(image, patch: int, out=None, dtype=BF16, ld=None):
    _chk(image, F32, "image")
    B, Cc, H, W = image.shape
    rows, K = B * (H // patch) * (W // patch), Cc * patch * patch
    pitch = K if ld is None else int(ld)
    out = torch.empty((rows, pitch), dtype=dtype, device=image.device) if out is None else _chk(out, BF16, "patches")
    assert out.numel() >= rows * pitch
    if ld is None:
        check(_L(out).mh_patchify(_p(image), _p(out), B, Cc, H, W, patch, _stream()), "mh_patchify")
    else:
        check(_L(out).mh_patchify_ld(_p(image), _p(out), B, Cc, H, W, patch, pitch, _stream()), "mh_patchify_ld")
    return out


def copy2d_words(src, ld_src, dst, ld_dst, rows, cols, pad_to):
    for nm, t in (("src", src), ("dst", dst)):
        if not t.is_cuda:
            raise _lib.MemehipError(f"{nm}: memehip kernels need a HIP device tensor; no CPU fallback")
    assert src.element_size() == dst.element_size()
    wpe = 4 // src.element_size()
    assert src.numel() >= ((rows - 1) * ld_src + cols) * wpe and dst.numel() >= ((rows - 1) * ld_dst + pad_to) * wpe
    check(_lib.load().mh_copy2d_u32(_p(src), ld_src, _p(dst), ld_dst, rows, cols, pad_to, _stream()), "mh_copy2d_u32")
    return dst


def dwconv_dgrad(dy, wt, B, H, W, addend=None, dx=None, K: int = 7):
    _chk(dy, BF16, "dy"), _chk(wt, F32, "wt")
    C = dy.shape[-1]
    if dy.numel() != B * H * W * C or wt.numel() != K * K * C:
        raise ValueError("dwconv_dgrad: dy / wt do not have the sizes B, H, W, C, K imply")
    dx = torch.empty_like(dy) if dx is None else _chk(dx, BF16, "dx")
    if addend is not None:
        _chk(addend, BF16, "addend")
    if dx.numel() != dy.numel() or dx.dtype != dy.dtype or (addend is not None and (addend.numel() != dy.numel() or addend.dtype != dy.dtype)):
        raise ValueError("dwconv_dgrad: dx / addend must match dy")
    check(_L(dy).mh_dwconv_nhwc_dgrad(_p(dy), _p(wt), _p(addend), _p(dx), B, H, W, C, K, _stream()), "mh_dwconv_nhwc_dgrad")
    return dx


def dwconv_wgrad_workspace_elems(B, H, W, C, K: int = 7) -> int:
    return int(_lib.load().mh_dwconv_wgrad_workspace_elems(B, H, W, C, K))


def dwconv_wgrad(x, dy, dw, dbias, B, H, W, scale: float = 1.0, accum: bool = False, workspace=None, K: int = 7):
    _chk(x, BF16, "x"), _chk(dy, BF16, "dy"), _chk(dw, F32, "dw")
    C = x.shape[-1]
    if x.dtype != dy.dtype or x.numel() != B * H * W * C or dy.numel() != x.numel() or dw.numel() != C * K * K:
        raise ValueError("dwconv_wgrad: x / dy / dw do not have the sizes B, H, W, C, K imply")
    if dbias is not None and (_chk(dbias, F32, "dbias").numel() != C):
        raise ValueError("dwconv_wgrad: dbias must hold C elements")
    need = dwconv_wgrad_workspace_elems(B, H, W, C, K)
    if need <= 0:
        raise _lib.MemehipError(f"mh_dwconv_nhwc_wgrad: unsupported shape B={B} H={H} W={W} C={C} K={K}")
    if workspace is None:
        workspace = torch.empty(need, dtype=F32, device=x.device)
    elif _chk(workspace, F32, "workspace").numel() < need:
        raise ValueError(f"dwconv_wgrad: workspace holds {workspace.numel()} elements, {need} needed")
    check(_L(x).mh_dwconv_nhwc_wgrad(_p(x), _p(dy), _p(dw), _p(dbias), _p(workspace), B, H, W, C, K, float(scale), int(accum), _stream()),
          "mh_dwconv_nhwc_wgrad")
    return dw


def layer_scale_bwd(W, b, gamma, dWp, dbp, dgamma, dW=None, db=None, accum: bool = False):
    dW, db = dWp if dW is None else dW, dbp if db is None else db
# ... 206 lines not shown
```

Baseline: 3371.

## Compute attention only for pooled query rows in final layers

Adds row-restricted attention kernels (forward and backward) that compute attention for only one query row per sequence, such as the CLS or pooled token, while keeping K/V over the full sequence. The engine now gathers just those query rows, projects Q only for them, and skips the full-sequence dQ/dKV work and the context scatter in layers where only pooled rows remain live. This removes most of the attention and Q-projection cost in the last layers, at the price of new specialised kernels and more complex plumbing.

```diff
diff --git a/include/memehip.h b/include/memehip.h
--- a/include/memehip.h
+++ b/include/memehip.h
@@ -108,6 +108,15 @@
 int mh_attn_fwd_grouped(const MhAttnProblem* problems , int n, mh_stream_t stream);
 int mh_attn_bwd_grouped(const MhAttnProblem* problems , int n, mh_stream_t stream);
 int mh_attn_set_onepass(int on);
+
+typedef struct MhAttnRowsProblem {
+    MhAttnProblem base;
+    const void* q;
+    const int32_t* idx;
+    int32_t stride, offset;
+} MhAttnRowsProblem;
+int mh_attn_fwd_rows_grouped(const MhAttnRowsProblem* problems , int n, mh_stream_t stream);
+int mh_attn_bwd_rows_grouped(const MhAttnRowsProblem* problems , int n, mh_stream_t stream);
 
 int mh_pack_plan(const int64_t* mask , int B, int S, int pool_index, int32_t* cu, int32_t* row_map,
                  int32_t* inv_map, int64_t* pmask, int32_t* pool_rows, int32_t* n_rows, mh_stream_t stream);
diff --git a/multimodal_propaganda_meme_classification_amd/_lib.py b/multimodal_propaganda_meme_classification_amd/_lib.py
--- a/multimodal_propaganda_meme_classification_amd/_lib.py
+++ b/multimodal_propaganda_meme_classification_amd/_lib.py
@@ -90,6 +90,10 @@
     _fields_ = [(n, c_void_p) for n in ("qkv", "key_mask", "out", "lse", "dout", "delta", "dqkv", "cu", "row_map", "rng")] + \
                [("drop_p", C.c_float), ("drop_stream", C.c_uint32), ("B", C.c_int32), ("S", C.c_int32), ("H", C.c_int32),
                 ("reserved", C.c_int32)]
+
+
+class MhAttnRowsProblem(C.Structure):
+    _fields_ = [("base", MhAttnProblem), ("q", c_void_p), ("idx", c_void_p), ("stride", C.c_int32), ("offset", C.c_int32)]
 
 
 MH_ROWS_MAX_JOBS = 8
@@ -132,6 +136,8 @@
     "mh_attn_bwd": [c_void_p] * 7 + [c_int, c_int, c_int, c_void_p, c_float, C.c_uint32, c_void_p],
     "mh_attn_fwd_grouped": [C.POINTER(MhAttnProblem), c_int, c_void_p],
     "mh_attn_bwd_grouped": [C.POINTER(MhAttnProblem), c_int, c_void_p],
+    "mh_attn_fwd_rows_grouped": [C.POINTER(MhAttnRowsProblem), c_int, c_void_p],
+    "mh_attn_bwd_rows_grouped": [C.POINTER(MhAttnRowsProblem), c_int, c_void_p],
     "mh_attn_set_onepass": [c_int],
     "mh_attn_fwd_packed": [c_void_p] * 6 + [c_int, c_int, c_int, c_void_p, c_float, C.c_uint32, c_void_p],
     "mh_attn_bwd_packed": [c_void_p] * 9 + [c_int, c_int, c_int, c_void_p, c_float, C.c_uint32, c_void_p],
diff --git a/multimodal_propaganda_meme_classification_amd/csrc/attention.hip b/multimodal_propaganda_meme_classification_amd/csrc/attention.hip
--- a/multimodal_propaganda_meme_classification_amd/csrc/attention.hip
+++ b/multimodal_propaganda_meme_classification_amd/csrc/attention.hip
@@ -118,6 +118,17 @@
             *(i32x2*)(base + (size_t)r * pitch + dt * 32 + 8 * g4 + 4 * h) = u.v;
         }
 }
+MH_DEV void store_row_from_T(h16* __restrict__ row, int h, const f32x16 (&acc)[2], float scale) {
+#pragma unroll
+    for (int dt = 0; dt < 2; ++dt)
+#pragma unroll
+        for (int g4 = 0; g4 < 4; ++g4) {
+            Pack4 u;
+#pragma unroll
+            for (int e = 0; e < 4; ++e) u.e[e] = (h16)(acc[dt][4 * g4 + e] * scale);
+            *(i32x2*)(row + dt * 32 + 8 * g4 + 4 * h) = u.v;
+        }
+}
 
 struct AttnArgs {
     const h16* qkv;
@@ -135,8 +146,55 @@
     const int32_t* row_map;
 };
 
-template <int NW, int NT_RES, bool DROP>
-MH_DEV void attn_fwd_body(const AttnArgs& A, const int bx, const int gx, const int bh, char* smem) {
+struct RowsArgs {
+    const h16* q;
+    const int32_t* idx;
+    int stride, offset;
+};
+MH_DEV int rows_query_row(const RowsArgs& R, int b) { return R.idx ? R.idx[b] : b * R.stride + R.offset; }
+MH_DEV int rows_query_pos(int row, size_t r0, int Sb) {
+    const long long p = (long long)row - (long long)r0;
+    return (p >= 0 && p < Sb) ? (int)p : -1;
+}
+MH_DEV void load_one_row_frag(const h16* __restrict__ row, bool mine, int lane, h16x8 (&f)[4]) {
+#pragma unroll
+    for (int s = 0; s < 4; ++s) {
+        Pack8 u;
+        u.v = *(const i32x4*)(row + 16 * s + 8 * (lane >> 5));
+        if (!mine) u.v = i32x4{0, 0, 0, 0};
+        f[s] = u.h;
+    }
+}
+template <int NT>
+MH_DEV void stage_one_row(const h16* __restrict__ qrow, const h16* __restrict__ drow, int live, int nrows, int tid, char* q_img,
+                          char* qt_img, char* do_img, char* dot_img) {
+    for (int i = tid; i < nrows * 8; i += NT) {
+        const int r = i >> 3, c = i & 7;
+        i32x4 vq = *(const i32x4*)(qrow + c * 8), vd = *(const i32x4*)(drow + c * 8);
+        if (r != live) vq = vd = i32x4{0, 0, 0, 0};
+        *(i32x4*)(q_img + row_img_off(r, c)) = vq;
+        *(i32x4*)(qt_img + tr_img_off(r, c >> 1) + ((c & 1) << 4)) = vq;
+        *(i32x4*)(do_img + row_img_off(r, c)) = vd;
+        *(i32x4*)(dot_img + tr_img_off(r, c >> 1) + ((c & 1) << 4)) = vd;
+    }
+}
+MH_DEV float row_delta_pair(const h16* __restrict__ drow, const h16* __restrict__ orow, bool live, int hf) {
+    float dl = 0.f;
+#pragma unroll
+    for (int s4 = 0; s4 < 4; ++s4) {
+        Pack8 a, o;
+        a.v = *(const i32x4*)(drow + 8 * hf + 16 * s4);
+        o.v = *(const i32x4*)(orow + 8 * hf + 16 * s4);
+#pragma unroll
+        for (int j = 0; j < 8; ++j) dl += (float)a.h[j] * (float)o.h[j];
+    }
+    if (!live) dl = 0.f;
+    return dl + mh_xor_partner<1>(dl, 0u);
+}
+
+template <int NW, int NT_RES, bool DROP, bool ROWS = false>
+MH_DEV void attn_fwd_body(const AttnArgs& A, const int bx, const int gx, const int bh, char* smem, const RowsArgs* R = nullptr) {
+    static_assert(!ROWS || (NT_RES > 0 && !DROP), "the restricted form: resident K / V, no dropout");
     const h16* __restrict__ qkv = A.qkv;
     const int64_t* __restrict__ key_mask = A.key_mask;
     h16* __restrict__ out = A.out;
@@ -159,6 +217,7 @@
     const int b = bh / H, hh = bh % H;
     const int tid = threadIdx.x, lane = tid & 63, wave = tid >> 6, h = lane >> 5;
     const size_t pitch = (size_t)3 * H * HD;
+    const int qrow = ROWS ? rows_query_row(*R, b) : 0;
     const size_t r0 = cu ? (size_t)cu[b] : (size_t)b * S;
     const int Sb = cu ? cu[b + 1] - cu[b] : S;
     auto pos = [&](int i) -> uint64_t { return (row_map && i < Sb) ? (uint64_t)(row_map[r0 + i] - b * S) : (uint64_t)i; };
@@ -170,13 +229,16 @@
     constexpr float LAZY_LOG2 = 6.0f;
     const int ntiles = (Sb + TILE - 1) / TILE;
 
-    const int qt_first = bx * NW + wave;
+    const int pq = ROWS ? rows_query_pos(qrow, r0, Sb) : 0;
+    const size_t prow = ROWS ? (size_t)b * H * HD + hh * HD : 0;
+    const int qt_first = ROWS ? max(pq, 0) >> 5 : bx * NW + wave;
     h16x8 qf[4];
     if (NT_RES > 0) {
         const int uw = __builtin_amdgcn_readfirstlane(wave);
         dma_resident<NW, NTL>(kb, pitch, Sb, ntiles, uw, lane, k_img, nullptr);
         dma_resident<NW, NTL>(vb, pitch, Sb, ntiles, uw, lane, nullptr, v_img);
-        if (qt_first * 32 < Sb) load_rows_frag(qb, pitch, qt_first * 32, Sb, lane, qf);
+        if constexpr (ROWS) load_one_row_frag(R->q + prow, pq >= 0 && (lane & 31) == (pq & 31), lane, qf);
+        else if (qt_first * 32 < Sb) load_rows_frag(qb, pitch, qt_first * 32, Sb, lane, qf);
         if (DROP)
             for (int i = tid; i < NTL * TILE; i += NT) pos_t[i] = (int)pos(i);
         if (tid < TILE) {
@@ -202,6 +264,10 @@
             }
         }
         __syncthreads();
+    }
+    if constexpr (ROWS) if (wave != 0 || pq < 0) {
+        if (pq < 0 && tid < 8) *(i32x4*)(out + prow + tid * 8) = i32x4{0, 0, 0, 0};
+        return;
     }
 
     for (int qt = qt_first; (NT_RES > 0) ? (qt * 32 < Sb) : (qt == bx * NW + wave); qt += NW * gx) {
@@ -309,14 +375,22 @@
         if (!active) continue;
         l += mh_xor_partner<32>(l, (unsigned)lane);
         const float inv = l > 0.f ? 1.0f / l : 0.f;
+        const int q = wq0 + (lane & 31);
+        if constexpr (ROWS) {
+            if (q == pq) {
+                store_row_from_T(out + prow, h, o, inv);
+                if (h == 0) lse[((size_t)b * H + hh) * S + q] = (m + __builtin_amdgcn_logf(l)) * LN2;
+            }
+            return;
+        }
         store_rows_from_T(out + r0 * H * HD + hh * HD, (size_t)H * HD, wq0, Sb, lane, o, inv);
-        const int q = wq0 + (lane & 31);
         if (h == 0 && q < Sb) lse[((size_t)b * H + hh) * S + q] = (m + __builtin_amdgcn_logf(l)) * LN2;
     }
 }
 
-template <int NW, int NT_RES, bool DROP>
-MH_DEV void attn_bwd_dq_body(const AttnArgs& A, const int bx, const int gx, const int bh, char* smem) {
+template <int NW, int NT_RES, bool DROP, bool ROWS = false>
+MH_DEV void attn_bwd_dq_body(const AttnArgs& A, const int bx, const int gx, const int bh, char* smem, const RowsArgs* R = nullptr) {
+    static_assert(!ROWS || (NT_RES > 0 && !DROP), "the restricted form: resident K / V, no dropout");
     const h16* __restrict__ qkv = A.qkv;
     const int64_t* __restrict__ key_mask = A.key_mask;
     const h16* __restrict__ out = A.out;
@@ -343,6 +417,7 @@
     const int b = bh / H, hh = bh % H;
     const int tid = threadIdx.x, lane = tid & 63, wave = tid >> 6, h = lane >> 5;
     const size_t pitch = (size_t)3 * H * HD;
+    const int qrow = ROWS ? rows_query_row(*R, b) : 0;
     const size_t r0 = cu ? (size_t)cu[b] : (size_t)b * S;
     const int Sb = cu ? cu[b + 1] - cu[b] : S;
     auto pos = [&](int i) -> uint64_t { return (row_map && i < Sb) ? (uint64_t)(row_map[r0 + i] - b * S) : (uint64_t)i; };
@@ -353,6 +428,8 @@
     const h16* dob = dout + r0 * H * HD + hh * HD;
     const float c = 0.125f * LOG2E;
     const int ntiles = (Sb + TILE - 1) / TILE;
+    const int pq = ROWS ? rows_query_pos(qrow, r0, Sb) : 0;
+    const size_t prow = ROWS ? (size_t)b * H * HD + hh * HD : 0;
 
     auto stage = [&](int t, int slot) {
         if (tid < TILE) {
@@ -381,13 +458,21 @@
         const int wq0 = qt * 32;
         const bool active = wq0 < Sb;
         const int q = wq0 + (lane & 31);
+        const bool skip = ROWS && !(pq >= 0 && qt == (pq >> 5));
+        const bool row_lane = ROWS && q == pq;
         h16x8 qf[4], dof[4];
-        load_rows_frag(qb, pitch, wq0, Sb, lane, qf);
-        load_rows_frag(dob, (size_t)H * HD, wq0, Sb, lane, dof);
+        if constexpr (ROWS) {
+            load_one_row_frag(R->q + prow, row_lane, lane, qf);
+            load_one_row_frag(dout + prow, row_lane, lane, dof);
+        } else {
+            load_rows_frag(qb, pitch, wq0, Sb, lane, qf);
+            load_rows_frag(dob, (size_t)H * HD, wq0, Sb, lane, dof);
+        }
         float dl = 0.f;
         {
             h16x8 of[4];
-            load_rows_frag(out + r0 * H * HD + hh * HD, (size_t)H * HD, wq0, Sb, lane, of);
+            if constexpr (ROWS) load_one_row_frag(out + prow, row_lane, lane, of);
+            else load_rows_frag(out + r0 * H * HD + hh * HD, (size_t)H * HD, wq0, Sb, lane, of);
 #pragma unroll
             for (int s4 = 0; s4 < 4; ++s4)
 #pragma unroll
@@ -395,7 +480,13 @@
             dl += mh_xor_partner<32>(dl, (unsigned)lane);
         }
         float lse2 = 0.f;
-        if (q < Sb) {
+        if constexpr (ROWS) {
+            const float lv = lse[((size_t)b * H + hh) * S + max(pq, 0)] * LOG2E;
+            if (row_lane) {
+                lse2 = lv;
+                if (h == 0) delta[((size_t)b * H + hh) * S + q] = dl;
+            }
+        } else if (q < Sb) {
             lse2 = lse[((size_t)b * H + hh) * S + q] * LOG2E;
             if (h == 0) delta[((size_t)b * H + hh) * S + q] = dl;
         }
@@ -429,7 +520,9 @@
         };
         if (NT_RES == 0 && ntiles > 0) pre_load(0);
 
-        for (int t = 0; t < ntiles; ++t) {
+        int t_end = ntiles;
+        if constexpr (ROWS) t_end = skip ? 0 : ntiles;
+        for (int t = 0; t < t_end; ++t) {
             const int slot = NT_RES > 0 ? t : 0;
             if (NT_RES == 0) {
                 __syncthreads();
@@ -481,8 +574,9 @@
     }
 }
 
-template <int NW, int NT_RES, bool DROP, bool OWN_DELTA = false>
-MH_DEV void attn_bwd_dkv_body(const AttnArgs& A, const int bx, const int gx, const int bh, char* smem) {
+template <int NW, int NT_RES, bool DROP, bool OWN_DELTA = false, bool ROWS = false>
+MH_DEV void attn_bwd_dkv_body(const AttnArgs& A, const int bx, const int gx, const int bh, char* smem, const RowsArgs* R = nullptr) {
+    static_assert(!ROWS || (NT_RES == 1 && !DROP && OWN_DELTA), "the restricted form: one staged tile, no dropout, its own delta");
     const h16* __restrict__ qkv = A.qkv;
     const int64_t* __restrict__ key_mask = A.key_mask;
     const h16* __restrict__ outp = A.out;
@@ -510,6 +604,7 @@
     const int b = bh / H, hh = bh % H;
     const int tid = threadIdx.x, lane = tid & 63, wave = tid >> 6, h = lane >> 5;
     const size_t pitch = (size_t)3 * H * HD;
+    const int qrow = ROWS ? rows_query_row(*R, b) : 0;
     const size_t r0 = cu ? (size_t)cu[b] : (size_t)b * S;
     const int Sb = cu ? cu[b + 1] - cu[b] : S;
     auto pos = [&](int i) -> uint64_t { return (row_map && i < Sb) ? (uint64_t)(row_map[r0 + i] - b * S) : (uint64_t)i; };
@@ -520,6 +615,8 @@
     const h16* dob = dout + r0 * H * HD + hh * HD;
     const float c = 0.125f * LOG2E;
     const int ntiles = (Sb + TILE - 1) / TILE;
+    const int pq = ROWS ? rows_query_pos(qrow, r0, Sb) : 0;
+    const size_t prow = ROWS ? (size_t)b * H * HD + hh * HD : 0;
 
     auto stage = [&](int t, int slot) {
         for (int i = tid; i < TILE; i += NT) {
@@ -547,7 +644,17 @@
             if (hf == 0) dl_t[slot * TILE + i] = dl;
         }
     };
-    if (NT_RES > 0) {
+    if constexpr (ROWS) {
+        const int live = pq >= 0 ? (pq & (TILE - 1)) : -1;
+        stage_one_row<NT>(R->q + prow, dout + prow, live, TILE, tid, q_img, qt_img, do_img, dot_img);
+        const float lv = lse[((size_t)b * H + hh) * S + max(pq, 0)] * LOG2E;
+        for (int i = tid; i < TILE; i += NT) lse_t[i] = i == live ? lv : 1.0e30f;
+        if (tid < 2 * TILE) {
+            const float dl = row_delta_pair(dout + prow, outp + prow, (tid >> 1) == live, tid & 1);
+            if ((tid & 1) == 0) dl_t[tid >> 1] = dl;
+        }
+        __syncthreads();
+    } else if (NT_RES > 0) {
         const int uw = __builtin_amdgcn_readfirstlane(wave);
         dma_resident<NW, NTL>(qb, pitch, Sb, ntiles, uw, lane, q_img, qt_img);
         dma_resident<NW, NTL>(dob, (size_t)H * HD, Sb, ntiles, uw, lane, do_img, dot_img);
@@ -622,8 +729,10 @@
         };
         if (NT_RES == 0 && ntiles > 0) pre_load(0);
 
-        for (int t = 0; t < ntiles; ++t) {
-            const int slot = NT_RES > 0 ? t : 0;
+        int t_first = 0, t_end = ntiles;
+        if constexpr (ROWS) { t_first = max(pq, 0) >> 6; t_end = pq >= 0 ? t_first + 1 : 0; }
+        for (int t = t_first; t < t_end; ++t) {
+            const int slot = (NT_RES > 0 && !ROWS) ? t : 0;
             if (NT_RES == 0) {
                 __syncthreads();
                 pre_store();
@@ -641,6 +750,7 @@
 #pragma unroll
             for (int sub = 0; sub < 2; ++sub) {
                 if (t * TILE + sub * 32 >= Sb) continue;
+                if constexpr (ROWS) if (sub != ((pq >> 5) & 1)) continue;
                 f32x16 st, dp;
 #pragma unroll
                 for (int g = 0; g < 16; ++g) { st[g] = 0.f; dp[g] = 0.f; }
@@ -910,6 +1020,175 @@
     else attn_bwd_dkv_body<4, RES_B, DROP_B, true>(Bp, 0, 1, y - nB, smem);
 }
 
+constexpr int OPR_BLK = 32 * 128;
+constexpr int OPR_LDS = OP_IMG + 4 * OPR_BLK + OP_NB * OP_MB + 2 * 32 * 4;
+
+MH_DEV void attn_bwd_onepass_rows_body(const AttnArgs& A, const RowsArgs& R, const int bh, char* smem) {
+    const h16* __restrict__ qkv = A.qkv;
+    const h16* __restrict__ outp = A.out;
+    const h16* __restrict__ dout = A.dout;
+    const float* __restrict__ lse = A.lse;
+    float* __restrict__ delta = A.delta;
+    h16* __restrict__ dqkv = A.dqkv;
+    const int S = A.S, H = A.H;
+    const int b = bh / H, hh = bh % H;
+    const int tid = threadIdx.x, lane = tid & 63, wave = tid >> 6, h = lane >> 5;
+    const size_t pitch = (size_t)3 * H * HD;
+    const size_t r0 = (size_t)b * S;
+    const int Sb = S;
+    const h16* qb = qkv + r0 * pitch + hh * HD;
+    const h16* kb = qb + (size_t)H * HD;
+    const h16* vb = qb + (size_t)2 * H * HD;
+    const float c = 0.125f * LOG2E;
+    const int pq = rows_query_pos(rows_query_row(R, b), r0, Sb);
+    const size_t prow = (size_t)b * H * HD + hh * HD;
+    const int PB = max(pq, 0) >> 5, live = pq >= 0 ? (pq & 31) : -1;
+
+    char* kt_img = smem;
+    char* q_img = smem + OP_IMG;
+    char* qt_img = q_img + OPR_BLK;
+    char* do_img = q_img + 2 * OPR_BLK;
+    char* dot_img = q_img + 3 * OPR_BLK;
+    char* mbox = q_img + 4 * OPR_BLK;
+    float* lse_t = (float*)(mbox + OP_NB * OP_MB);
+    float* dl_t = lse_t + 32;
+
+    {
+        const __amdgpu_buffer_rsrc_t rk = mh_rsrc(kb, (uint32_t)(((size_t)(Sb - 1) * pitch + HD) * 2));
+        const int uw = __builtin_amdgcn_readfirstlane(wave);
+#pragma unroll
+        for (int i = 0; i < OP_ROWS / 8 / OP_NB; ++i) {
+            const int p = uw + i * OP_NB;
+            const int r = p * 8 + (lane >> 3), cp = lane & 7;
+            const int c_tr = ((((cp >> 1) ^ (((r >> 1) & 1) << 1)) << 1) | (cp & 1));
+            __builtin_amdgcn_raw_ptr_buffer_load_lds(rk, LDS_PTR(void, kt_img + p * 1024), 16, (uint32_t)r * (uint32_t)pitch * 2u + c_tr * 16, 0, 0, 0);
+        }
+    }
+    const int wk0 = wave * 32;
+    const bool mine = wk0 < Sb;
+    h16x8 kf[4], vf[4];
+    load_rows_frag(kb, pitch, wk0, Sb, lane, kf);
+    load_rows_frag(vb, pitch, wk0, Sb, lane, vf);
+    stage_one_row<OP_NB * 64>(R.q + prow, dout + prow, live, 32, tid, q_img, qt_img, do_img, dot_img);
+    if (tid < 64) {
+        const int i = tid >> 1;
+        const float dl = row_delta_pair(dout + prow, outp + prow, i == live, tid & 1);
+        const float lv = lse[((size_t)b * H + hh) * S + max(pq, 0)] * LOG2E;
+        if ((tid & 1) == 0) {
+            dl_t[i] = dl;
+            lse_t[i] = i == live ? lv : 1.0e30f;
+            if (i == live) delta[((size_t)b * H + hh) * S + pq] = dl;
+        }
+    }
+    __syncthreads();
+
+    const float kbias = (wk0 + (lane & 31)) < Sb ? 0.f : NEG_BIG;
+    f32x16 dk[2], dv[2], dq[2];
+#pragma unroll
+    for (int i = 0; i < 2; ++i)
+#pragma unroll
+        for (int g = 0; g < 16; ++g) { dk[i][g] = 0.f; dv[i][g] = 0.f; dq[i][g] = 0.f; }
+
+    if (mine && pq >= 0) {
+        f32x16 st, dp;
+#pragma unroll
+        for (int g = 0; g < 16; ++g) { st[g] = 0.f; dp[g] = 0.f; }
+#pragma unroll
+        for (int s = 0; s < 4; ++s) {
+            st = MH_MFMA_32x32x16(frag_rows(q_img, 0, s, lane), kf[s], st, 0, 0, 0);
+            dp = MH_MFMA_32x32x16(frag_rows(do_img, 0, s, lane), vf[s], dp, 0, 0, 0);
+        }
+        f32x16 pp;
+#pragma unroll
+        for (int g4 = 0; g4 < 4; ++g4) {
+            const f32x4 l4 = *(const f32x4*)(lse_t + 8 * g4 + 4 * h);
+            const f32x4 d4 = *(const f32x4*)(dl_t + 8 * g4 + 4 * h);
+#pragma unroll
+            for (int e = 0; e < 4; ++e) {
+                const int g = 4 * g4 + e;
+                const float pr = __builtin_amdgcn_exp2f(st[g] * c + kbias - l4[e]);
+                pp[g] = pr;
+                st[g] = pr * (dp[g] - d4[e]);
+            }
+        }
+#pragma unroll
+        for (int s = 0; s < 2; ++s) {
+            const h16x8 pf = acc_frag(pp, s);
+            const h16x8 df = acc_frag(st, s);
+#pragma unroll
+            for (int dt = 0; dt < 2; ++dt) {
+                dv[dt] = MH_MFMA_32x32x16(frag_tr(dot_img, 0, s, dt * 32, lane), pf, dv[dt], 0, 0, 0);
+                dk[dt] = MH_MFMA_32x32x16(frag_tr(qt_img, 0, s, dt * 32, lane), df, dk[dt], 0, 0, 0);
+            }
+        }
+        char* mb = mbox + wave * OP_MB + (lane & 31) * 2;
+#pragma unroll
+        for (int g4 = 0; g4 < 4; ++g4)
+#pragma unroll
+            for (int e = 0; e < 4; ++e) *(h16*)(mb + (8 * g4 + 4 * h + e) * OP_MB_PITCH) = (h16)st[4 * g4 + e];
+    }
+    __syncthreads();
+    if (pq >= 0 && wave == PB) {
+        for (int j = 0; j < OP_NB; ++j) {
+            int src = PB - j;
+            if (src < 0) src += OP_NB;
+            if (src * 32 >= Sb) continue;
+            const char* mb = mbox + src * OP_MB + (lane & 31) * OP_MB_PITCH;
+#pragma unroll
+            for (int s = 0; s < 2; ++s) {
+                union {
+                    struct { i32x2 lo, hi; } v;
+                    h16x8 f;
+                } u;
+                u.v.lo = *(const i32x2*)(mb + (16 * s + 4 * h) * 2);
+                u.v.hi = *(const i32x2*)(mb + (16 * s + 8 + 4 * h) * 2);
+#pragma unroll
+                for (int dt = 0; dt < 2; ++dt)
+                    dq[dt] = MH_MFMA_32x32x16(frag_tr(kt_img, src * 32, s, dt * 32, lane), u.f, dq[dt], 0, 0, 0);
+            }
+        }
+    }
+    if (!mine) return;
+    store_rows_from_T(dqkv + r0 * pitch + hh * HD, pitch, wk0, Sb, lane, dq, 0.125f);
+    store_rows_from_T(dqkv + r0 * pitch + (size_t)H * HD + hh * HD, pitch, wk0, Sb, lane, dk, 0.125f);
+    store_rows_from_T(dqkv + r0 * pitch + (size_t)2 * H * HD + hh * HD, pitch, wk0, Sb, lane, dv, 1.0f);
+}
+
+template <int NT_RES>
+__global__ __launch_bounds__(256) void attn_fwd_rows_kernel(const AttnArgs A, const RowsArgs R) {
+    extern __shared__ __attribute__((aligned(16))) char smem[];
+    attn_fwd_body<4, NT_RES, false, true>(A, 0, 1, blockIdx.y, smem, &R);
+}
+__global__ __launch_bounds__(256) void attn_fwd_rows_dual_kernel(const AttnArgs A, const RowsArgs RA, const AttnArgs Bp, const RowsArgs RB,
+                                                                 const int nA) {
+    extern __shared__ __attribute__((aligned(16))) char smem[];
+    if ((int)blockIdx.y < nA) attn_fwd_body<4, 4, false, true>(A, 0, 1, blockIdx.y, smem, &RA);
+    else attn_fwd_body<4, 2, false, true>(Bp, 0, 1, blockIdx.y - nA, smem, &RB);
+}
+template <int NT_RES>
+__global__ __launch_bounds__(256) void attn_bwd_rows_kernel(const AttnArgs A, const RowsArgs R, const int n) {
+    extern __shared__ __attribute__((aligned(16))) char smem[];
+    const int y = blockIdx.y;
+    if (y < n) attn_bwd_dq_body<4, NT_RES, false, true>(A, 0, 1, y, smem, &R);
+    else attn_bwd_dkv_body<4, 1, false, true, true>(A, 0, 1, y - n, smem, &R);
+}
+__global__ __launch_bounds__(448) void attn_bwd_onepass_rows_kernel(const AttnArgs A, const RowsArgs R) {
+    extern __shared__ __attribute__((aligned(16))) char smem[];
+    attn_bwd_onepass_rows_body(A, R, blockIdx.y, smem);
+}
+__global__ __launch_bounds__(448) void attn_bwd_onepass_rows_dual_kernel(const AttnArgs A, const RowsArgs RA, const AttnArgs Bp,
+                                                                         const RowsArgs RB, const int nA, const int nB) {
+    extern __shared__ __attribute__((aligned(16))) char smem[];
+    const int y = blockIdx.y;
+    if (y < nA) {
+        attn_bwd_onepass_rows_body(A, RA, y, smem);
+    } else {
+        if (threadIdx.x >= 256) return;
+        if (y < nA + nB) attn_bwd_dq_body<4, 2, false, true>(Bp, 0, 1, y - nA, smem, &RB);
+        else attn_bwd_dkv_body<4, 1, false, true, true>(Bp, 0, 1, y - nA - nB, smem, &RB);
+    }
+}
+
 template <auto KERN, int THREADS, int LDS, typename... Args>
 void launch(dim3 grid, hipStream_t s, const Args&... args) {
     static const hipError_t raised = hipFuncSetAttribute((const void*)KERN, hipFuncAttributeMaxDynamicSharedMemorySize, LDS);
@@ -999,6 +1278,77 @@
     return false;
 }
 
+constexpr int LDS_BWD_ROWS(int nt) { return cmax(lds_dq(nt), lds_dkv(1)); }
+constexpr int LDS_BWD_ROWS_DUAL = cmax(OPR_LDS, LDS_BWD_ROWS(2));
+
+int check_rows_problem(const MhAttnRowsProblem& p, bool bwd) {
+    if (int st = check_problem(p.base, bwd)) return st;
+    if (!p.q) return MH_EINVAL;
+    if (p.base.S > 256 || has_drop(p.base)) return MH_ESHAPE;
+    return MH_OK;
+}
+RowsArgs to_rows(const MhAttnRowsProblem& p) {
+    RowsArgs r;
+    r.q = (const h16*)p.q;
+    r.idx = p.idx;
+    r.stride = p.stride; r.offset = p.offset;
+    return r;
+}
+void launch_fwd_rows(const MhAttnRowsProblem& p, hipStream_t s) {
+    const dim3 grid(1, p.base.B * p.base.H);
+    if (p.base.S <= 128) launch<attn_fwd_rows_kernel<2>, 256, lds_fwd(2)>(grid, s, to_args(p.base), to_rows(p));
+    else launch<attn_fwd_rows_kernel<4>, 256, lds_fwd(4)>(grid, s, to_args(p.base), to_rows(p));
+}
+void launch_bwd_rows(const MhAttnRowsProblem& p, hipStream_t s) {
+    const int BH = p.base.B * p.base.H;
+    const AttnArgs a = to_args(p.base);
+    if (onepass_fits(p.base)) launch<attn_bwd_onepass_rows_kernel, 448, OPR_LDS>(dim3(1, BH), s, a, to_rows(p));
+    else if (p.base.S <= 128) launch<attn_bwd_rows_kernel<2>, 256, LDS_BWD_ROWS(2)>(dim3(1, 2 * BH), s, a, to_rows(p), BH);
+    else launch<attn_bwd_rows_kernel<4>, 256, LDS_BWD_ROWS(4)>(dim3(1, 2 * BH), s, a, to_rows(p), BH);
+}
+bool dual_rows_pair(const MhAttnRowsProblem* p, int n, int s_max, int& ia, int& ib) {
+    if (n != 2) return false;
+    for (int k = 0; k < 2; ++k)
+        if (p[k].base.S > 128 && p[k].base.S <= s_max && p[1 - k].base.S <= 128) {
+            ia = k;
+            ib = 1 - k;
+            return true;
+        }
+    return false;
+}
+
+}
+
+extern "C" int mh_attn_fwd_rows_grouped(const MhAttnRowsProblem* p, int n, mh_stream_t stream) {
+    if (!p || n < 1 || n > MH_ATTN_MAX_GROUP) return MH_EINVAL;
+    for (int i = 0; i < n; ++i)
+        if (int st = check_rows_problem(p[i], false)) return st;
+    hipStream_t s = (hipStream_t)stream;
+    int ia, ib;
+    if (dual_rows_pair(p, n, 256, ia, ib)) {
+        const int nA = p[ia].base.B * p[ia].base.H, nB = p[ib].base.B * p[ib].base.H;
+        launch<attn_fwd_rows_dual_kernel, 256, LDS_FWD_DUAL>(dim3(1, nA + nB), s, to_args(p[ia].base), to_rows(p[ia]), to_args(p[ib].base),
+                                                             to_rows(p[ib]), nA);
+    } else {
+        for (int i = 0; i < n; ++i) launch_fwd_rows(p[i], s);
+    }
+    return mh_launch_status();
+}
+
+extern "C" int mh_attn_bwd_rows_grouped(const MhAttnRowsProblem* p, int n, mh_stream_t stream) {
+    if (!p || n < 1 || n > MH_ATTN_MAX_GROUP) return MH_EINVAL;
+    for (int i = 0; i < n; ++i)
+        if (int st = check_rows_problem(p[i], true)) return st;
+    hipStream_t s = (hipStream_t)stream;
+    int ia, ib;
+    if (g_onepass == 2 && dual_rows_pair(p, n, OP_ROWS, ia, ib) && onepass_fits(p[ia].base)) {
+        const int nA = p[ia].base.B * p[ia].base.H, nB = p[ib].base.B * p[ib].base.H;
+        launch<attn_bwd_onepass_rows_dual_kernel, 448, LDS_BWD_ROWS_DUAL>(dim3(1, nA + 2 * nB), s, to_args(p[ia].base), to_rows(p[ia]),
+                                                                          to_args(p[ib].base), to_rows(p[ib]), nA, nB);
+    } else {
+        for (int i = 0; i < n; ++i) launch_bwd_rows(p[i], s);
+    }
+    return mh_launch_status();
 }
 
 extern "C" int mh_attn_fwd_grouped(const MhAttnProblem* p, int n, mh_stream_t stream) {
diff --git a/multimodal_propaganda_meme_classification_amd/engine.py b/multimodal_propaganda_meme_classification_amd/engine.py
--- a/multimodal_propaganda_meme_classification_amd/engine.py
+++ b/multimodal_propaganda_meme_classification_amd/engine.py
@@ -7,7 +7,7 @@
 import torch
 
 from . import _lib
-from ._lib import (MH_GEMM_DERIV_AUX, MH_GEMM_GELU, MH_GEMM_OUT_F32, MH_GEMM_QUICK_GELU, MhAttnProblem, MhColsumJob, MhGemmProblem, MhHeadGrads,
+from ._lib import (MH_GEMM_DERIV_AUX, MH_GEMM_GELU, MH_GEMM_OUT_F32, MH_GEMM_QUICK_GELU, MhAttnProblem, MhAttnRowsProblem, MhColsumJob, MhGemmProblem, MhHeadGrads,
                    MhHeadParams, MhLnBwdJob, MhLnFwdJob, MhRowsJob)
 from .config import Layout, ModelConfig, check_sequence_length
 
@@ -218,10 +218,11 @@
 LnBwd = namedtuple("LnBwd", "dy x gamma mean rstd dx part rows D dx_add dx_drop drop rows_dev drop_rows",
                    defaults=(None, None, NO_DROP, None, None))
 Attn = namedtuple("Attn", "qkv out lse B S H key_mask cu row_map drop dout delta dqkv", defaults=(None, None, None, NO_DROP, None, None, None))
+AttnRows = namedtuple("AttnRows", "attn q rows")
 RowsJob = namedtuple("RowsJob", "n rows D idx stride offset src dst rows_dev", defaults=(None, 0, 0, None, None, None))
 
-TextActs = namedtuple("TextActs", "qkv ctx lse a y m1 r1 h g f m2 r2 pctx x rows")
-ImageActs = namedtuple("ImageActs", "u m1 r1 qkv ctx lse xp w m2 r2 h g pctx x rows")
+TextActs = namedtuple("TextActs", "qkv ctx lse a y m1 r1 h g f m2 r2 pctx x rows q qin")
+ImageActs = namedtuple("ImageActs", "u m1 r1 qkv ctx lse xp w m2 r2 h g pctx x rows q qin")
 
 Roles = namedtuple("Roles", "attn_in proj_out ffn_in ffn_res ffn_out")
 
@@ -244,6 +245,9 @@
 
     def rows(self, l: int) -> int:
         return self.compact if (self.compact and l == self.L - 1) else self.T
+
+    def query_rows(self, l: int) -> bool:
+        return self.rows(l) != self.T and self.S <= 256
 
     @property
     def out_rows(self) -> int:
@@ -419,10 +423,42 @@
         self.pl.keep.append(arr)
         seg.c("mh_attn_bwd_grouped" if backward else "mh_attn_fwd_grouped", arr, len(probs))
 
-    def _attn_prob(self, tw: Tower, l: int, **bw) -> Attn:
+    def _attn_prob(self, tw: Tower, l: int, out=None, **bw) -> Attn:
         a = tw.acts[l]
-        return Attn(a.qkv, a.ctx, a.lse, self.B, tw.S, tw.H, tw.key_mask, tw.cu, tw.row_map,
+        return Attn(a.qkv, a.ctx if out is None else out, a.lse, self.B, tw.S, tw.H, tw.key_mask, tw.cu, tw.row_map,
                     self.site(tw.p_a, 16 * (l + 1) + 1), **bw)
+
+    def _qkv_fwd(self, tw: Tower, l: int, a_, r: Roles) -> List[Gemm]:
+        stem, D = tw.attn + "query", tw.D
+        if a_.q is None:
+            return [self._linear(tw, l, stem, r.attn_in, a_.qkv, tw.T, 3 * D, D, 3, **tw.live(tw.T))]
+        w, bias = self.eng.w(tw.name(l, stem) + ".weight", 3), self.eng.p(tw.name(l, stem) + ".bias", 3)
+        return [Gemm(r.attn_in, w[D * D:], a_.qkv.view(-1)[D:], tw.T, 2 * D, D, lda=D, ldb=D, ldc=3 * D, bias=bias[D:], **tw.live(tw.T)),
+                self._fwd_prob(a_.qin, w[:D * D], a_.q, self.B, D, D, bias=bias[:D])]
+
+    def _attn_rows(self, seg: Segment, probs: List[AttnRows], backward: bool):
+        arr = (MhAttnRowsProblem * len(probs))()
+        for e, (d, q, rows) in zip(arr, probs):
+            assert d.drop.rng is None and rows.n == d.B and q.dtype == self.T16
+            for k in ("qkv", "key_mask", "out", "lse", "dout", "delta", "dqkv", "cu"):
+                setattr(e.base, k, _ptr(getattr(d, k)))
+            e.base.B, e.base.S, e.base.H = d.B, d.S, d.H
+            e.q, e.idx, e.stride, e.offset = _ptr(q), _ptr(rows.idx), rows.stride, rows.offset
+            n = d.B * d.H * 64
+            assert d.qkv.numel() >= 3 * n * d.S and d.out.numel() >= n and q.numel() >= n and d.lse.numel() >= d.B * d.H * d.S
+            assert rows.idx is None or (rows.idx.dtype == torch.int32 and rows.idx.numel() >= d.B)
+            if backward:
+                assert d.dout.numel() >= n and d.dqkv.numel() >= 3 * n * d.S and d.delta.numel() >= d.B * d.H * d.S
+        self.pl.keep.append(arr)
+        seg.c("mh_attn_bwd_rows_grouped" if backward else "mh_attn_fwd_rows_grouped", arr, len(probs))
+
+    def _attn_layer(self, seg: Segment, probs: List[Tuple[Tower, Attn, Optional[torch.Tensor]]], backward: bool):
+        full = [d for tw, d, q in probs if q is None]
+        rows = [AttnRows(d, q, tw.pool) for tw, d, q in probs if q is not None]
+        if full:
+            self._attn(seg, full, backward)
+        if rows:
+            self._attn_rows(seg, rows, backward)
 
     def _rows(self, seg: Segment, jobs: List[RowsJob], scatter: bool):
         if not jobs:
@@ -526,7 +562,10 @@
                 y=alloc(n + "y", (R, t.D)), m1=alloc(n + "m1", (R,), F32), r1=alloc(n + "r1", (R,), F32),
                 h=alloc(n + "h", (R, t.I)), g=alloc(n + "g", (R, t.I)), f=alloc(n + "f", (R, t.D)),
                 m2=alloc(n + "m2", (R,), F32), r2=alloc(n + "r2", (R,), F32),
-                pctx=alloc(n + "pctx", (B, t.D)) if R != t.T else ctx, x=alloc(n + "xrows", (B, t.D)) if R != t.T else t.x[l], rows=R))
+                pctx=alloc(n + "pctx", (B, t.D)) if R != t.T else ctx, x=alloc(n + "xrows", (B, t.D)) if R != t.T else t.x[l], rows=R,
+                q=alloc(n + "qrows", (B, t.D)) if t.query_rows(l) else None, qin=None))
+            if t.query_rows(l):
+                t.acts[l] = t.acts[l]._replace(qin=t.acts[l].x)
             t.x.append(alloc(f"t.x{l + 1}", (R, t.D)))
         for l in range(v.L):
             R, n = v.rows(l), f"i{l}."
@@ -536,7 +575,8 @@
                 qkv=alloc(n + "qkv", (v.T, 3 * v.D)), ctx=ctx, lse=alloc(n + "lse", (B, v.H, v.S), F32),
                 xp=alloc(n + "xp", (R, v.D)), w=alloc(n + "w", (R, v.D)), m2=alloc(n + "m2", (R,), F32), r2=alloc(n + "r2", (R,), F32),
                 h=alloc(n + "h", (R, v.I)), g=alloc(n + "g", (R, v.I)),
-                pctx=alloc(n + "pctx", (B, v.D)) if R != v.T else ctx, x=alloc(n + "xrows", (B, v.D)) if R != v.T else v.x[l], rows=R))
+                pctx=alloc(n + "pctx", (B, v.D)) if R != v.T else ctx, x=alloc(n + "xrows", (B, v.D)) if R != v.T else v.x[l], rows=R,
+                q=alloc(n + "qrows", (B, v.D)) if v.query_rows(l) else None, qin=alloc(n + "urows", (B, v.D)) if v.query_rows(l) else None))
             v.x.append(alloc(f"i.x{l + 1}", (R, v.D)))
         self.xf = alloc("i.xf", (v.out_rows, v.D))
         self.mf, self.rf = alloc("i.mf", (v.out_rows,), F32), alloc("i.rf", (v.out_rows,), F32)
@@ -555,10 +595,13 @@
         f, t, v = self.pl.fwd, self.text, self.image
         lay = [(tw, tw.acts[l], tw.roles(l), tw.rows(l)) for tw in self.towers if l < tw.L]
         a, b = (t.acts[l] if l < t.L else None), (v.acts[l] if l < v.L else None)
-        self._gemm(f, [self._linear(tw, l, tw.attn + "query", r.attn_in, a_.qkv, tw.T, 3 * tw.D, tw.D, 3, **tw.live(tw.T))
-                       for tw, a_, r, M in lay], False, False)
-        self._attn(f, [self._attn_prob(tw, l) for tw, _, _, _ in reversed(lay)], backward=False)
-        self._rows(f, [j for tw, a_, r, M in lay if M != tw.T
+        self._rows(f, [j for tw, a_, r, M in lay if tw.query_rows(l)
+                       for j in [tw.pool._replace(src=tw.x[l], dst=a_.x)] +
+                                ([tw.pool._replace(src=r.attn_in, dst=a_.qin)] if a_.qin is not a_.x else [])], scatter=False)
+        self._gemm(f, [g for tw, a_, r, M in lay for g in self._qkv_fwd(tw, l, a_, r)], False, False)
+        self._attn_layer(f, [(tw, self._attn_prob(tw, l, out=a_.pctx) if a_.q is not None else self._attn_prob(tw, l), a_.q)
+                             for tw, a_, _, _ in reversed(lay)], backward=False)
+        self._rows(f, [j for tw, a_, r, M in lay if M != tw.T and not tw.query_rows(l)
                        for j in (tw.pool._replace(src=a_.ctx, dst=a_.pctx), tw.pool._replace(src=tw.x[l], dst=a_.x))], scatter=False)
         self._gemm(f, [self._linear(tw, l, "attention.output.dense", a_.pctx, r.proj_out, M, tw.D, tw.D, residual=a_.x,
                                     drop=self.site(tw.p_h, 16 * (l + 1) + 2), **tw.live(M, drop=True)) for tw, a_, r, M in lay], False, False)
@@ -705,10 +748,11 @@
         self._gemm(s, [self._linear_dgrad(tw, l, "attention.output.dense", g.d_proj, g.dctx, M, tw.D, tw.D, **tw.live(M))
                        for tw, a_, r, g, M in lay], False, True)
         self._rows(s, [j for tw, a_, r, g, M in lay if M != tw.T
-                       for j in (tw.pool._replace(src=g.dctx, dst=g.dctx_full, rows_dev=tw.rows_dev),
-                                 tw.pool._replace(src=g.res, dst=g.res_full, rows_dev=tw.rows_dev))], scatter=True)
-        self._attn(s, [self._attn_prob(tw, l, dout=g.dctx_full, delta=tw.delta, dqkv=g.dqkv) for tw, a_, r, g, M in reversed(lay)],
-                   backward=True)
+                       for j in ([] if a_.q is not None else [tw.pool._replace(src=g.dctx, dst=g.dctx_full, rows_dev=tw.rows_dev)]) +
+                                [tw.pool._replace(src=g.res, dst=g.res_full, rows_dev=tw.rows_dev)]], scatter=True)
+        self._attn_layer(s, [(tw, self._attn_prob(tw, l, out=a_.pctx, dout=g.dctx, delta=tw.delta, dqkv=g.dqkv) if a_.q is not None
+                              else self._attn_prob(tw, l, dout=g.dctx_full, delta=tw.delta, dqkv=g.dqkv), a_.q)
+                             for tw, a_, r, g, M in reversed(lay)], backward=True)
         self._gemm(s, [self._linear_dgrad(tw, l, tw.attn + "query", g.dqkv, g.d_in, tw.T, 3 * tw.D, tw.D, 3,
                                           residual=g.res_full if tw.post_ln else None, **tw.live(tw.T)) for tw, a_, r, g, M in lay], False, True)
         t_job = self._text_ln2_bwd(l - 1) if l >= 1 else self._text_embed_ln_bwd(s)
diff --git a/multimodal_propaganda_meme_classification_amd/ops.py b/multimodal_propaganda_meme_classification_amd/ops.py
--- a/multimodal_propaganda_meme_classification_amd/ops.py
+++ b/multimodal_propaganda_meme_classification_amd/ops.py
@@ -363,6 +363,30 @@
     check(fn(arr, len(problems), _stream()), "mh_attn_bwd_grouped" if backward else "mh_attn_fwd_grouped")
 
 
+def attn_rows_grouped(problems, backward: bool = False):
+    from ._lib import MhAttnRowsProblem
+    arr = (MhAttnRowsProblem * len(problems))()
+    for e, d in zip(arr, problems):
+        _chk(d["qkv"], BF16, "qkv"), _chk(d["out"], BF16, "out"), _chk(d["lse"], F32, "lse"), _chk(d["q"], BF16, "q")
+        n = d["B"] * d["H"] * 64
+        assert d["qkv"].numel() >= 3 * n * d["S"] and d["out"].numel() >= n and d["q"].numel() >= n
+        assert d["lse"].numel() >= d["B"] * d["H"] * d["S"]
+        if backward:
+            _chk(d["dout"], BF16, "dout"), _chk(d["dqkv"], BF16, "dqkv"), _chk(d["delta"], F32, "delta")
+            assert d["dout"].numel() >= n and d["dqkv"].numel() >= 3 * n * d["S"] and d["delta"].numel() >= d["B"] * d["H"] * d["S"]
+        idx = d.get("idx")
+        if idx is not None:
+            _chk(idx, torch.int32, "idx")
+            assert idx.numel() >= d["B"]
+        for k in ("qkv", "key_mask", "out", "lse", "dout", "delta", "dqkv", "cu"):
+            setattr(e.base, k, _p(d.get(k)))
+        e.base.B, e.base.S, e.base.H = d["B"], d["S"], d["H"]
+        e.q, e.idx, e.stride, e.offset = _p(d["q"]), _p(idx), int(d.get("stride", 0)), int(d.get("offset", 0))
+    lib = _L(problems[0]["qkv"])
+    fn = lib.mh_attn_bwd_rows_grouped if backward else lib.mh_attn_fwd_rows_grouped
+    check(fn(arr, len(problems), _stream()), "mh_attn_bwd_rows_grouped" if backward else "mh_attn_fwd_rows_grouped")
+
+
 def attn_bwd(qkv, key_mask, out, dout, lse, B, S, H, dqkv=None, delta=None, drop=None):
     _chk(qkv, BF16, "qkv"), _chk(out, BF16, "out"), _chk(dout, BF16, "dout"), _chk(lse, F32, "lse")
     assert qkv.numel() == B * S * 3 * H * 64 and out.numel() == B * S * H * 64 == dout.numel()
```

New measurement: 3387 (median of 5 runs). Within noise of the previous version (+0.5%).
